# xuhaocuhk/TilinGNN

Measured on AMD Instinct MI355X. Metric: scored tile-nodes/sec (GNN forward), higher is better.
Workload: dtype f32; 1 GPU; TilinGNN.forward on a seeded banded super-graph: 100000 nodes / 1000000 adjacency edges / 1250000 collision edges per GPU, tile_count 2, T=13 edge types, width 32, depth 20, train-mode BatchNorm, graph prep included; n_nodes=100000, n_adj_edges=1000000, n_col_edges=1250000, parallelism=single GPU

## Files before the change

### include/tgnn.h

```cpp
#ifndef TGNN_H
#define TGNN_H

#include <stddef.h>
#include <stdint.h>

#ifdef __cplusplus
extern "C" {
#endif

#define TGNN_VERSION 100

#define TGNN_OK 0
#define TGNN_ERR_INVALID_ARG (-1)
#define TGNN_ERR_WORKSPACE (-2)
#define TGNN_ERR_LAUNCH (-3)
#define TGNN_ERR_UNSUPPORTED (-4)
#define TGNN_ERR_BAD_GRAPH (-5)
#define TGNN_ERR_UNVERIFIED (-7)
#define TGNN_ERR_STALE_RESULT (-6)

#define TGNN_ACT_NONE 0
#define TGNN_ACT_LEAKY_RELU 1
#define TGNN_ACT_SIGMOID 2

// ... 72 lines not shown
int tgnn_gin_fwd(const float *a, int64_t lda, const float *in_stat, const int32_t *rowptr,
                 const int32_t *col_src, const float *eps, const float *w1, const float *b1,
                 const float *w2, const float *b2, const float *w3, const float *b3, int64_t n_nodes,
                 int32_t c, int32_t act, float *out, float *z_scratch, double *bn_partial,
                 int32_t *n_partials_host, tgnn_stream_t stream);

int tgnn_dense_act_fwd(const float *a, int64_t lda, int64_t a_kblock_stride, const float *in_stat,
                       const float *w, const float *b, int64_t n_rows, int32_t in_dim, int32_t out_dim,
                       int32_t act, float *out, int64_t ldo, double *bn_partial, int32_t *n_partials_host,
                       tgnn_stream_t stream);
int tgnn_dense_act_slots_fwd(const float *a, int32_t slot_width, int64_t slot_stride, const float *in_stat,
                             const float *w, const float *b, int64_t n_rows, int32_t in_dim, int32_t out_dim,
                             int32_t act, float *out, int64_t ldo, double *bn_partial, int32_t *n_partials_host,
                             tgnn_stream_t stream);
int tgnn_dense_act_slots_f16_fwd(const float *a, int32_t slot_width, int64_t slot_stride, const float *w, const float *b,
                                 int64_t n_rows, int32_t in_dim, int32_t out_dim, int32_t act, float *out, int64_t ldo,
                                 uint32_t *bounds_scratch, void *wimg_scratch, double *bn_partial, int32_t *n_partials_host,
                                 tgnn_stream_t stream);

int tgnn_bn_finalize(int32_t mode, const double *partials, int32_t n_partials, double *sums, int32_t f,
                     int64_t n_rows_total, const float *gamma, const float *beta, float eps, float momentum,
                     float *running_mean, float *running_var, int64_t *num_batches_tracked, float *stat,
                     tgnn_stream_t stream);

int tgnn_bn_apply(const float *v, int64_t ldv, const float *stat, int64_t n_rows, int32_t f, float *out,
                  int64_t ldo, tgnn_stream_t stream);

int tgnn_merge_fwd(const float *a1, const float *stat1, const float *a2, const float *stat2,
                   const float *resid, int64_t n_nodes, int32_t c, float *out, float *h2_out,
                   tgnn_stream_t stream);

typedef struct tgnn_model_dims {
    int32_t node_features_dim;
    int32_t adj_edge_features_dim;
    int32_t network_width;
    int32_t network_depth;
    int32_t output_dim;
} tgnn_model_dims;

int32_t tgnn_param_count(const tgnn_model_dims *dims);
int tgnn_param_name(const tgnn_model_dims *dims, int32_t index, char *buf, size_t buf_len);

typedef struct tgnn_graph {
    int64_t n_nodes;
    int64_t n_adj_edges;
    int64_t n_col_edges;
    int32_t n_types;
    const int32_t *adj_rowptr;
    const int32_t *adj_src;
    const int32_t *adj_type;
    const int32_t *type_rep_edge;
    const int32_t *col_rowptr;
    const int32_t *col_src;
    const int32_t *nn_tile_col_ptr;
    const int32_t *nn_col_meta;
    const int32_t *nn_col_src;
    int32_t nn_max_in_degree;
    const int32_t *nn_mid_tile_nb;
    const uint32_t *nn_mid_ent;
    const int32_t *nn_tile_grp_ptr;
    const int32_t *nn_grp;
    const int32_t *nn_mid_verdict;
} tgnn_graph;

size_t tgnn_forward_workspace_bytes(const tgnn_model_dims *dims, int64_t n_nodes, int32_t n_types);

int tgnn_forward(const tgnn_model_dims *dims, const void *const *params_host, const float *x,
                 const float *adj_edge_attr, const tgnn_graph *graph, int32_t update_running,
                 int32_t use_running_stats, float *probs, void *ws, size_t ws_bytes,
                 tgnn_stream_t stream, tgnn_stream_t stream2);

int tgnn_forward_begin(const tgnn_model_dims *dims, const void *const *params_host, const float *x, int64_t n_nodes,
                       int32_t update_running, void *ws, size_t ws_bytes, tgnn_stream_t stream, tgnn_stream_t stream2);
int tgnn_forward_resume(const tgnn_model_dims *dims, const void *const *params_host, const float *x, const float *adj_edge_attr,
                        const tgnn_graph *graph, int32_t update_running, float *probs, void *ws, size_t ws_bytes,
                        tgnn_stream_t stream, tgnn_stream_t stream2);
int tgnn_forward_small_prepass(const tgnn_model_dims *dims, const void *const *params_host, const float *adj_edge_attr,
                               const int32_t *type_rep_edge, const int32_t *n_types_dev, int64_t n_nodes, void *ws, size_t ws_bytes,
                               tgnn_stream_t stream);

int tgnn_forward_begin_weights(const tgnn_model_dims *dims, const void *const *params_host, const float *adj_edge_attr,
                               const int32_t *type_rep_edge, const int32_t *n_types_dev, int64_t n_nodes, void *ws, size_t ws_bytes,
                               tgnn_stream_t stream);

typedef struct tgnn_train_save {
    float *init_a[2];
    float *init_stat[2];
    float *a1, *a2;
    float *u;
    float *stat1, *stat2;
    float *fin_a[4];
    float *fin_stat[4];
    float *skip;
    float *wtab;
} tgnn_train_save;
int tgnn_forward_train(const tgnn_model_dims *dims, const void *const *params_host, const float *x,
                       const float *adj_edge_attr, const tgnn_graph *graph, const tgnn_train_save *keep, float *probs,
                       void *ws, size_t ws_bytes, tgnn_stream_t stream, tgnn_stream_t stream2);

typedef struct tgnn_train_graph {
    const int32_t *adjT_rowptr, *adjT_src, *adjT_type;
    const int32_t *colT_rowptr, *colT_src;
    const float *deg, *inv_deg;
} tgnn_train_graph;
size_t tgnn_backward_workspace_bytes(const tgnn_model_dims *dims, int64_t n_nodes, int32_t n_types);
int tgnn_backward(const tgnn_model_dims *dims, const void *const *params_host, void *const *grads_host, const float *x,
                  const float *adj_edge_attr, const tgnn_graph *graph, const tgnn_train_graph *tgraph,
                  const tgnn_train_save *keep, const float *probs, const float *dprobs, void *ws, size_t ws_bytes,
                  tgnn_stream_t stream);

typedef struct tgnn_shard {
    int64_t n_own, n_rows, n_total;
    const int32_t *send_idx;
    int64_t n_send;
    double *sum_buf;
    float *send_buf;
    float *recv_buf;
    int (*allreduce_f64)(void *ctx, double *buf, int64_t count, tgnn_stream_t stream);
    int (*alltoall_rows)(void *ctx, const float *send, float *recv, int32_t row_floats, int32_t extra_rows,
                         tgnn_stream_t stream);
    void *ctx;
    int32_t world, rank;
    const int32_t *send_idx_fused;
    const int32_t *recv_idx_fused;
    tgnn_stream_t side_stream;
    void *rccl_comm, *rccl_comm_side;
    const int64_t *send_counts, *recv_counts;
    const int32_t *send_row_ptr, *send_row_slot;
} tgnn_shard;

int32_t tgnn_rccl_available(void);
size_t tgnn_rccl_unique_id_bytes(void);
int tgnn_rccl_unique_id(void *id_out);
int tgnn_rccl_comm_create(const void *unique_id, int32_t rank, int32_t world, void **comm_out);
int tgnn_rccl_comm_destroy(void *comm);
void tgnn_rccl_counters(int64_t *out2);
size_t tgnn_forward_sharded_workspace_bytes(const tgnn_model_dims *dims, int64_t n_own, int64_t n_rows,
                                            int32_t n_types);
int tgnn_forward_sharded(const tgnn_model_dims *dims, const void *const *params_host, const float *x,
                         const float *adj_edge_attr, const tgnn_graph *graph, const tgnn_shard *shard,
                         int32_t update_running, float *probs, void *ws, size_t ws_bytes, tgnn_stream_t stream);

void tgnn_set_small_layout_limit(int64_t n_nodes);
int tgnn_spin_error_poll(tgnn_stream_t stream, uint32_t *code_out);
uint64_t tgnn_set_spin_budget_us(uint64_t us);
void tgnn_persist_fallback(int64_t n_forwards);
uint32_t tgnn_spin_error_peek(void);
int64_t tgnn_get_small_layout_limit(void);

int32_t tgnn_set_split_precision(int32_t mode);
int32_t tgnn_set_gin_fused(int32_t mode);
int32_t tgnn_set_gin_mlp_f16(int32_t on);
int32_t tgnn_set_mid_tail(int32_t on);
int32_t tgnn_set_nnconv_eg(int32_t on);
int32_t tgnn_set_dense_rows_mode(int32_t mode);
int32_t tgnn_set_lean_head(int32_t bits);

int64_t tgnn_graph_prep_small_max_nodes(void);
int64_t tgnn_graph_prep_small_max_edges(void);
size_t tgnn_graph_prep_small_tmp_ints(int64_t n_nodes, int64_t n_adj_edges, int64_t n_col_edges);
int tgnn_graph_prep_small(const int64_t *adj_edge_index, int64_t n_adj_edges, const float *adj_edge_attr, int32_t fe,
                          const int64_t *col_edge_index, int64_t n_col_edges, int64_t n_nodes, int32_t *adj_rowptr,
                          int32_t *adj_src, int32_t *adj_eid, int32_t *adj_type, int32_t *edge_type, int32_t *type_rep_edge,
                          int32_t *col_rowptr, int32_t *col_src, int32_t *col_eid, int32_t *tile_col_ptr, int32_t *col_meta,
                          int32_t *col_slot_src, int32_t *tmp, int32_t *result, uint32_t *counters, int32_t *result_host,
                          tgnn_stream_t stream);

typedef struct tgnn_small_prep_layout {
    const int64_t *adj_edge_index;
    const float *adj_edge_attr;
    const int64_t *col_edge_index;
    int64_t n_adj_edges, n_col_edges, n_nodes;
    int32_t *adj_rowptr, *adj_src, *adj_eid, *adj_type, *edge_type, *type_rep_edge;
    int32_t *col_rowptr, *col_src, *col_eid;
    int32_t *tile_col_ptr, *col_meta, *col_slot_src;
    int32_t *tmp;
    int32_t fe, reserved_;
} tgnn_small_prep_layout;
int tgnn_graph_prep_small_many(const tgnn_small_prep_layout *layouts_host, int32_t k, int32_t *results_dev, int32_t *results_host,
                               tgnn_stream_t stream);
int tgnn_graph_prep_small_many_wait(tgnn_stream_t stream);
int tgnn_graph_prep_small_many_plan(const int64_t *n_adj_edges, const int64_t *n_col_edges, const int64_t *n_nodes, int32_t k,
                                    int32_t capacity_blocks, int32_t *blocks_out, int32_t *group_out);
void tgnn_graph_prep_small_many_counts(int64_t out[2]);

size_t tgnn_graph_prep_workspace_bytes(int64_t n_nodes, int64_t n_adj_edges, int64_t n_col_edges, int32_t fe);
int tgnn_graph_prep(const int64_t *adj_edge_index, int64_t n_adj_edges, const float *adj_edge_attr, int32_t fe,
                    const int64_t *col_edge_index, int64_t n_col_edges, int64_t n_nodes, int64_t n_src_nodes, int32_t *adj_rowptr,
                    int32_t *adj_src, int32_t *adj_eid, int32_t *adj_type, int32_t *edge_type, int32_t *type_rep_edge, int32_t *col_rowptr,
                    int32_t *col_src, int32_t *col_eid, int32_t *tile_col_ptr, int32_t *col_meta, int32_t *col_slot_src,
                    int32_t *mid_tile_nb, uint32_t *mid_ent, int32_t *tile_grp_ptr, int32_t *grp,
                    void *ws, size_t ws_bytes, int32_t *result, int32_t *result_host, tgnn_stream_t stream);
int tgnn_graph_prep_wait(tgnn_stream_t stream);
int32_t tgnn_set_prep_words_poll(int32_t on);
#ifdef TGNN_DEBUG
int32_t tgnn_debug_set_csr_bucket_cap(int32_t cap);
void tgnn_debug_set_block_caps(int32_t nnconv_blocks, int32_t gin_mlp_blocks);
void tgnn_debug_spin_fault(int32_t n_launches);
#endif

#define TGNN_PROF_CLASSES 8
#define TGNN_PROF_EDGE_WEIGHTS 0
#define TGNN_PROF_DENSE_INIT 1
#define TGNN_PROF_NNCONV 2
#define TGNN_PROF_GIN 3
#define TGNN_PROF_BN_FINALIZE 4
#define TGNN_PROF_MERGE 5
#define TGNN_PROF_DENSE_FINAL 6
int tgnn_forward_profiled(const tgnn_model_dims *dims, const void *const *params_host, const float *x,
                          const float *adj_edge_attr, const tgnn_graph *graph, int32_t update_running,
                          int32_t use_running_stats, float *probs, void *ws, size_t ws_bytes,
                          tgnn_stream_t stream, float *class_ms_host, int32_t *class_launches_host);

int tgnn_forward_profiled_two_stream(const tgnn_model_dims *dims, const void *const *params_host, const float *x,
                                     const float *adj_edge_attr, const tgnn_graph *graph, int32_t update_running,
                                     float *probs, void *ws, size_t ws_bytes, tgnn_stream_t stream, tgnn_stream_t stream2,
                                     float *class_ms_host, int32_t *class_launches_host);
int tgnn_forward_many(const tgnn_model_dims *dims, const void *const *params_host, int32_t n_layouts, const float *const *x,
                      const float *const *adj_edge_attr, const tgnn_graph *graphs, int32_t update_running,
                      int32_t use_running_stats, float *const *probs, void *const *ws, const size_t *ws_bytes,
                      const tgnn_stream_t *streams, int32_t n_streams, tgnn_stream_t stream2);
int tgnn_forward_union(const tgnn_model_dims *dims, const void *const *params_host, int32_t n_layouts, const float *const *x,
                       const float *const *adj_edge_attr, const tgnn_graph *graphs, int32_t use_running_stats,
                       float *const *probs, void *const *ws, const size_t *ws_bytes, tgnn_stream_t stream,
                       const tgnn_stream_t *streams, int32_t n_streams, tgnn_stream_t stream2);
int tgnn_forward_union_plan(const int64_t *n_nodes, int32_t k, int32_t capacity_blocks, int32_t *group_out);
void tgnn_forward_union_counts(int64_t out[2]);
int tgnn_forward_stamped(const tgnn_model_dims *dims, const void *const *params_host, const float *x, const float *adj_edge_attr,
                         const tgnn_graph *graph, int32_t update_running, float *probs, void *ws, size_t ws_bytes,
                         tgnn_stream_t stream, tgnn_stream_t stream2, float *nnconv_us_host);

size_t tgnn_sublayout_workspace_bytes(int64_t n_nodes, int64_t n_adj_edges, int64_t n_col_edges);
int tgnn_sublayout_compact(const int32_t *alive, int64_t n_nodes, const float *x, int32_t fx,
                           const int64_t *adj_edge_index, int64_t n_adj_edges, const float *adj_edge_attr, int32_t fe,
                           const int64_t *col_edge_index, int64_t n_col_edges, float *x_out, int64_t *inverse_out,
                           int64_t *adj_out, float *adj_attr_out, int64_t *col_out, int64_t *counts_out,
                           int32_t *err_flag, void *ws, size_t ws_bytes, tgnn_stream_t stream);

int tgnn_shard_alive_rows(const int32_t *alive_global, const int64_t *gid, int64_t n_own, int64_t n_rows,
                          const int64_t *adj_edge_index, int64_t n_adj_edges, const int64_t *col_edge_index, int64_t n_col_edges,
                          int32_t *alive_local, int32_t *err_flag, tgnn_stream_t stream);

size_t tgnn_greedy_round_workspace_bytes(int64_t n_sub);
int tgnn_greedy_round(const float *prob, int64_t ld_prob, const int64_t *inverse, int64_t n_sub, const int64_t *col_edge_index,
                      int64_t n_col_edges, int32_t round, uint64_t seed, double *prob_saved, int32_t *alive,
                      int32_t *selected_round, int64_t *n_selected, int32_t *err_flag, void *ws, size_t ws_bytes,
                      tgnn_stream_t stream);
int64_t tgnn_greedy_finish_max_nodes(void);
int tgnn_greedy_finish(const int64_t *inverse, int64_t n_sub, const int64_t *col_edge_index, int64_t n_col_edges,
                       int32_t first_round, int32_t max_rounds, uint64_t seed, double *prob_saved, int32_t *alive,
                       int32_t *selected_round, int64_t *n_selected, int32_t *err_flag, int32_t *out, tgnn_stream_t stream);

size_t tgnn_sublayout_compact_many_workspace_bytes(int32_t n_layouts, int64_t total_nodes, int64_t total_adj_edges,
                                                   int64_t total_col_edges);
int tgnn_sublayout_compact_many(int32_t n_layouts, const int32_t *active, const int64_t *node_ptr, const int64_t *adj_ptr,
                                const int64_t *col_ptr, int64_t total_nodes, int64_t total_adj_edges, int64_t total_col_edges,
                                const int32_t *alive, const float *x, int32_t fx, const int64_t *adj_edge_index,
                                const float *adj_edge_attr, int32_t fe, const int64_t *col_edge_index, float *x_out,
                                int64_t *inverse_out, int64_t *adj_out, float *adj_attr_out, int64_t *col_out, int64_t *counts_out,
                                int32_t *err_flag, void *ws, size_t ws_bytes, tgnn_stream_t stream);
size_t tgnn_greedy_round_many_workspace_bytes(int32_t n_layouts, int64_t total_nodes);
int tgnn_greedy_round_many(int32_t n_layouts, const int32_t *active, const float *const *prob, int64_t ld_prob,
                           const int64_t *node_ptr, const int64_t *col_ptr, int64_t total_nodes, int64_t total_col_edges,
                           const int64_t *counts, const int64_t *inverse, const int64_t *col_edge_index, int32_t round,
                           const uint64_t *seeds, double *prob_saved, int32_t *alive, int32_t *selected_round, int64_t *n_selected,
                           int32_t *err_flag, void *ws, size_t ws_bytes, tgnn_stream_t stream);
int tgnn_greedy_finish_many(int32_t n_layouts, const int32_t *finish, const int64_t *node_ptr, const int64_t *col_ptr,
                            int64_t total_nodes, int64_t total_col_edges, const int64_t *counts, const int64_t *inverse,
                            const int64_t *col_edge_index, int32_t first_round, int32_t max_rounds, const uint64_t *seeds,
                            double *prob_saved, int32_t *alive, int32_t *selected_round, int64_t *n_selected, int32_t *err_flag,
                            int32_t *out, tgnn_stream_t stream);

size_t tgnn_unsupervised_loss_workspace_bytes(int32_t n_maps);
int tgnn_unsupervised_loss(const float *probs, int64_t ld_probs, int32_t n_maps, const float *area_ratio,
                           int64_t ld_area, int64_t n_nodes, const int64_t *col_edge_index, int64_t n_col_edges,
                           const int64_t *adj_edge_index, int64_t n_adj_edges, const float *adj_edge_len,
                           int64_t ld_len, float collision_weight, float align_length_weight, float avg_area_weight,
                           double *losses, double *terms, void *ws, size_t ws_bytes, tgnn_stream_t stream);

// ... 118 lines not shown
```

### tilingnn_amd/_lib.py

```python
from __future__ import annotations

import ctypes as C
import os

_HERE = os.path.dirname(os.path.abspath(__file__))
LIB_PATH = os.environ.get("TGNN_LIB_PATH") or os.path.join(_HERE, "libtgnn.so")

ACT_NONE, ACT_LEAKY_RELU, ACT_SIGMOID = 0, 1, 2
BN_MAX_PARTIALS = 512
BN_STAT_ROWS = 4


class TgnnError(RuntimeError):
    code = 0


class ModelDims(C.Structure):
    _fields_ = [("node_features_dim", C.c_int32), ("adj_edge_features_dim", C.c_int32),
                ("network_width", C.c_int32), ("network_depth", C.c_int32), ("output_dim", C.c_int32)]


class Graph(C.Structure):
    _fields_ = [("n_nodes", C.c_int64), ("n_adj_edges", C.c_int64), ("n_col_edges", C.c_int64),
                ("n_types", C.c_int32),
# ... 17 lines not shown

class TrainSave(C.Structure):
    _fields_ = [("init_a", C.c_void_p * 2), ("init_stat", C.c_void_p * 2), ("a1", C.c_void_p), ("a2", C.c_void_p),
                ("u", C.c_void_p), ("stat1", C.c_void_p), ("stat2", C.c_void_p), ("fin_a", C.c_void_p * 4),
                ("fin_stat", C.c_void_p * 4), ("skip", C.c_void_p), ("wtab", C.c_void_p)]


class TrainGraphDesc(C.Structure):
    _fields_ = [("adjT_rowptr", C.c_void_p), ("adjT_src", C.c_void_p), ("adjT_type", C.c_void_p),
                ("colT_rowptr", C.c_void_p), ("colT_src", C.c_void_p), ("deg", C.c_void_p), ("inv_deg", C.c_void_p)]


ALLREDUCE_CB = C.CFUNCTYPE(C.c_int, C.c_void_p, C.c_void_p, C.c_int64, C.c_void_p)
ALLTOALL_CB = C.CFUNCTYPE(C.c_int, C.c_void_p, C.c_void_p, C.c_void_p, C.c_int32, C.c_int32, C.c_void_p)


class ShardDesc(C.Structure):
    _fields_ = [("n_own", C.c_int64), ("n_rows", C.c_int64), ("n_total", C.c_int64),
                ("send_idx", C.c_void_p), ("n_send", C.c_int64),
                ("sum_buf", C.c_void_p), ("send_buf", C.c_void_p), ("recv_buf", C.c_void_p),
                ("allreduce_f64", ALLREDUCE_CB), ("alltoall_rows", ALLTOALL_CB), ("ctx", C.c_void_p),
                ("world", C.c_int32), ("rank", C.c_int32), ("send_idx_fused", C.c_void_p), ("recv_idx_fused", C.c_void_p),
                ("side_stream", C.c_void_p), ("rccl_comm", C.c_void_p), ("rccl_comm_side", C.c_void_p),
                ("send_counts", C.c_void_p), ("recv_counts", C.c_void_p),
                ("send_row_ptr", C.c_void_p), ("send_row_slot", C.c_void_p)]


def _load() -> C.CDLL:
    if not os.path.exists(LIB_PATH):
        raise ImportError(
            f"{LIB_PATH} is missing: the HIP extension has not been built. Build it with\n"
            f"    python -c 'import __graft_entry__ as g; g.build()'    (or: make -C tilingnn_amd/csrc)\n"
            "tilingnn_amd has no CPU fallback by design.")
    import torch
    lib = C.CDLL(LIB_PATH)
    p, i32, i64, f32, sz = C.c_void_p, C.c_int32, C.c_int64, C.c_float, C.c_size_t
    pi32 = C.POINTER(C.c_int32)
    sigs = {
        "tgnn_version": (C.c_int, []),
        "tgnn_last_error": (C.c_char_p, []),
        "tgnn_csr_workspace_bytes": (sz, [i64, i64]),
        "tgnn_csr_build": (C.c_int, [p, i64, i64, i64, C.c_int, p, p, p, p, p, sz, p]),
        "tgnn_edge_dedup_workspace_bytes": (sz, [i64, i32]),
        "tgnn_edge_type_dedup": (C.c_int, [p, i64, i32, p, p, p, p, sz, p]),
        "tgnn_gather_i32": (C.c_int, [p, i64, p, i64, p, p]),
        "tgnn_edge_weight_table": (C.c_int, [p, p, i32, i32, p, p, p, p, p, p, i32, p, p]),
        "tgnn_nnconv_mean_fwd": (C.c_int, [p, i64, p, p, p, p, i32, p, p, i64, i32, i32, p, p, pi32, p]),
        "tgnn_nnconv_cols_max_columns": (i64, [i64, i64]),
        "tgnn_nnconv_cols_workspace_bytes": (sz, [i64]),
        "tgnn_nnconv_cols_build": (C.c_int, [p, p, p, i64, i32, p, p, p, p, sz, p]),
        "tgnn_nnconv_cols_max_types": (i32, []),
        "tgnn_nnconv_weight_image_floats": (sz, [i32]),
        "tgnn_nnconv_mean_cols_fwd": (C.c_int, [p, i64, p, p, p, p, i32, p, p, i64, i32, i32, p, p, p, pi32, p]),
        "tgnn_nnconv_mean_cols_f16_fwd": (C.c_int, [p, i64, i64, p, p, p, p, i32, p, p, i64, i32, i32, p, p, p, p, pi32, p]),
        "tgnn_nnconv_eg_max_groups": (i64, [i64, i64, i32]),
        "tgnn_nnconv_eg_build": (C.c_int, [p, p, p, i64, i32, p, p, p, sz, p]),
        "tgnn_nnconv_mean_eg_fwd": (C.c_int, [p, i64, i64, p, p, p, i32, p, p, i64, i32, p, p, p, p, pi32, p]),
        "tgnn_ubench_row_gather": (C.c_int, [i32, p, i64, p, i32, i32, C.POINTER(C.c_double), p]),
        "tgnn_mid_entries_words": (i64, [i64]),
        "tgnn_mid_entries_build": (C.c_int, [p, p, p, i64, p, p, p, p, p]),
        "tgnn_forward_path_counts": (None, [p]),
        "tgnn_set_mid_layout_limit": (None, [i64]),
        "tgnn_get_mid_layout_limit": (i64, []),
        "tgnn_mid_layout_max_nodes": (i64, []),
        "tgnn_spin_error_poll": (C.c_int, [p, C.POINTER(C.c_uint32)]),
        "tgnn_set_spin_budget_us": (C.c_uint64, [C.c_uint64]),
        "tgnn_persist_fallback": (None, [i64]),
        "tgnn_spin_error_peek": (C.c_uint32, []),
        "tgnn_gin_fwd": (C.c_int, [p, i64, p, p, p, p, p, p, p, p, p, p, i64, i32, i32, p, p, p, pi32, p]),
        "tgnn_dense_act_fwd": (C.c_int, [p, i64, i64, p, p, p, i64, i32, i32, i32, p, i64, p, pi32, p]),
        "tgnn_dense_act_slots_fwd": (C.c_int, [p, i32, i64, p, p, p, i64, i32, i32, i32, p, i64, p, pi32, p]),
        "tgnn_dense_act_slots_f16_fwd": (C.c_int, [p, i32, i64, p, p, i64, i32, i32, i32, p, i64, p, p, p, pi32, p]),
        "tgnn_bn_finalize": (C.c_int, [i32, p, i32, p, i32, i64, p, p, f32, f32, p, p, p, p, p]),
        "tgnn_bn_apply": (C.c_int, [p, i64, p, i64, i32, p, i64, p]),
        "tgnn_merge_fwd": (C.c_int, [p, p, p, p, p, i64, i32, p, p, p]),
        "tgnn_param_count": (i32, [C.POINTER(ModelDims)]),
        "tgnn_param_name": (C.c_int, [C.POINTER(ModelDims), i32, C.c_char_p, sz]),
        "tgnn_forward_workspace_bytes": (sz, [C.POINTER(ModelDims), i64, i32]),
        "tgnn_forward": (C.c_int, [C.POINTER(ModelDims), C.POINTER(C.c_void_p), p, p, C.POINTER(Graph), i32, i32,
                                   p, p, sz, p, p]),
        "tgnn_forward_begin": (C.c_int, [C.POINTER(ModelDims), C.POINTER(C.c_void_p), p, i64, i32, p, sz, p, p]),
        "tgnn_forward_resume": (C.c_int, [C.POINTER(ModelDims), C.POINTER(C.c_void_p), p, p, C.POINTER(Graph), i32, p, p, sz, p, p]),
        "tgnn_forward_begin_weights": (C.c_int, [C.POINTER(ModelDims), C.POINTER(C.c_void_p), p, p, p, i64, p, sz, p]),
        "tgnn_forward_small_prepass": (C.c_int, [C.POINTER(ModelDims), C.POINTER(C.c_void_p), p, p, p, i64, p, sz, p]),
        "tgnn_forward_sharded_workspace_bytes": (sz, [C.POINTER(ModelDims), i64, i64, i32]),
        "tgnn_forward_sharded": (C.c_int, [C.POINTER(ModelDims), C.POINTER(C.c_void_p), p, p, C.POINTER(Graph),
                                           C.POINTER(ShardDesc), i32, p, p, sz, p]),
        "tgnn_sublayout_workspace_bytes": (sz, [i64, i64, i64]),
        "tgnn_sublayout_compact": (C.c_int, [p, i64, p, i32, p, i64, p, i32, p, i64, p, p, p, p, p, p, p, p, sz, p]),
        "tgnn_shard_alive_rows": (C.c_int, [p, p, i64, i64, p, i64, p, i64, p, p, p]),
        "tgnn_tiles_in_region": (C.c_int, [p, p, p, p, p, i64, p, p, p, p, i64, i32, p, p, p]),
        "tgnn_region_edge_counts": (C.c_int, [p, i64, i64, p, i64, p, i64, p, p, p]),
        "tgnn_union_area_workspace_bytes": (sz, [i64, i64]),
        "tgnn_union_area": (C.c_int, [p, p, i64, p, p, p, i64, C.c_double, p, p, p, sz, p]),
        "tgnn_batch_union": (C.c_int, [p] * 10 + [i32, i32, i32, p, p, i32, p, p, p, p, p]),
        "tgnn_greedy_round_workspace_bytes": (sz, [i64]),
        "tgnn_greedy_round": (C.c_int, [p, i64, p, i64, p, i64, i32, C.c_uint64, p, p, p, p, p, p, sz, p]),
        "tgnn_greedy_finish_max_nodes": (i64, []),
        "tgnn_greedy_finish": (C.c_int, [p, i64, p, i64, i32, i32, C.c_uint64, p, p, p, p, p, p, p]),
        "tgnn_sublayout_compact_many_workspace_bytes": (sz, [i32, i64, i64, i64]),
        "tgnn_sublayout_compact_many": (C.c_int, [i32, p, p, p, p, i64, i64, i64, p, p, i32, p, p, i32, p, p, p, p, p, p, p, p, p, sz, p]),
        "tgnn_greedy_round_many_workspace_bytes": (sz, [i32, i64]),
        "tgnn_greedy_round_many": (C.c_int, [i32, p, p, i64, p, p, i64, i64, p, p, p, i32, p, p, p, p, p, p, p, sz, p]),
        "tgnn_greedy_finish_many": (C.c_int, [i32, p, p, p, i64, i64, p, p, p, i32, i32, p, p, p, p, p, p, p, p]),
        "tgnn_solution_score_sums_many_workspace_bytes": (sz, [i32]),
        "tgnn_solution_score_sums_many": (C.c_int, [i32, p, p, p, i64, i64, p, p, i64, p, p, p, i64, p, p, sz, p]),
        "tgnn_unsupervised_loss_workspace_bytes": (sz, [i32]),
        "tgnn_unsupervised_loss": (C.c_int, [p, i64, i32, p, i64, i64, p, i64, p, i64, p, i64, f32, f32, f32, p, p, p, sz, p]),
        "tgnn_solution_score_sums": (C.c_int, [p, p, i64, p, i64, p, i64, p, i64, p, p, sz, p]),
        "tgnn_graph_prep_small_max_nodes": (i64, []),
        "tgnn_graph_prep_small_max_edges": (i64, []),
        "tgnn_graph_prep_small_tmp_ints": (sz, [i64, i64, i64]),
        "tgnn_graph_prep_small": (C.c_int, [p, i64, p, i32, p, i64, i64] + [p] * 16 + [p]),
        "tgnn_graph_prep_workspace_bytes": (sz, [i64, i64, i64, i32]),
        "tgnn_graph_prep": (C.c_int, [p, i64, p, i32, p, i64, i64, i64] + [p] * 17 + [sz, p, p, p]),
        "tgnn_graph_prep_wait": (C.c_int, [p]),
        "tgnn_graph_prep_small_many": (C.c_int, [C.POINTER(SmallPrepLayout), i32, p, p, p]),
        "tgnn_graph_prep_small_many_wait": (C.c_int, [p]),
        "tgnn_graph_prep_small_many_plan": (C.c_int, [p, p, p, i32, i32, p, p]),
        "tgnn_graph_prep_small_many_counts": (None, [p]),
        "tgnn_set_nnconv_eg": (i32, [i32]),
        "tgnn_set_dense_rows_mode": (i32, [i32]),
        "tgnn_set_lean_head": (i32, [i32]),
        "tgnn_set_prep_words_poll": (i32, [i32]),
        "tgnn_set_small_layout_limit": (None, [i64]),
        "tgnn_get_small_layout_limit": (i64, []),
        "tgnn_set_split_precision": (i32, [i32]),
        "tgnn_set_gin_fused": (i32, [i32]),
        "tgnn_set_gin_mlp_f16": (i32, [i32]),
        "tgnn_set_mid_tail": (i32, [i32]),
        "tgnn_rccl_available": (i32, []),
        "tgnn_rccl_unique_id_bytes": (sz, []),
        "tgnn_rccl_unique_id": (C.c_int, [p]),
        "tgnn_rccl_comm_create": (C.c_int, [p, i32, i32, C.POINTER(C.c_void_p)]),
        "tgnn_rccl_comm_destroy": (C.c_int, [p]),
        "tgnn_rccl_counters": (None, [p]),
        "tgnn_forward_profiled": (C.c_int, [C.POINTER(ModelDims), C.POINTER(C.c_void_p), p, p, C.POINTER(Graph), i32,
                                            i32, p, p, sz, p, C.POINTER(C.c_float), pi32]),
        "tgnn_forward_many": (C.c_int, [C.POINTER(ModelDims), C.POINTER(C.c_void_p), i32, p, p, p, i32, i32, p, p, p, p, i32, p]),
        "tgnn_forward_union": (C.c_int, [C.POINTER(ModelDims), C.POINTER(C.c_void_p), i32, p, p, p, i32, p, p, p, p, p, i32, p]),
        "tgnn_forward_union_plan": (C.c_int, [p, i32, i32, p]),
        "tgnn_forward_union_counts": (None, [p]),
        "tgnn_forward_stamped": (C.c_int, [C.POINTER(ModelDims), C.POINTER(C.c_void_p), p, p, C.POINTER(Graph), i32, p, p, sz, p, p,
                                           C.POINTER(C.c_float)]),
        "tgnn_forward_profiled_two_stream": (C.c_int, [C.POINTER(ModelDims), C.POINTER(C.c_void_p), p, p, C.POINTER(Graph), i32,
                                                       p, p, sz, p, p, C.POINTER(C.c_float), pi32]),
        "tgnn_transpose": (C.c_int, [p, i32, i32, p, p]),
        "tgnn_swap_leading": (C.c_int, [p, i32, i32, i32, p, i32, p]),
        "tgnn_backward_workspace_bytes": (sz, [C.POINTER(ModelDims), i64, i32]),
        "tgnn_backward": (C.c_int, [C.POINTER(ModelDims), C.POINTER(C.c_void_p), C.POINTER(C.c_void_p), p, p,
                                    C.POINTER(Graph), C.POINTER(TrainGraphDesc), C.POINTER(TrainSave), p, p, p, sz, p]),
        "tgnn_forward_train": (C.c_int, [C.POINTER(ModelDims), C.POINTER(C.c_void_p), p, p, C.POINTER(Graph),
                                         C.POINTER(TrainSave), p, p, sz, p, p]),
        "tgnn_gin_aggregate": (C.c_int, [p, i64, p, p, p, p, i64, i32, p, p]),
        "tgnn_sigmoid_bwd": (C.c_int, [p, i64, p, i64, i64, i32, p, i64, p]),
        "tgnn_add_into": (C.c_int, [p, i64, i64, i32, p, i64, p]),
        "tgnn_reduce_workspace_bytes": (sz, [i32]),
        "tgnn_colsum": (C.c_int, [p, i64, i64, i32, p, p, sz, p]),
        "tgnn_bn_bwd_reduce": (C.c_int, [p, i64, p, i64, p, i64, i32, f32, p, p, p, p, sz, p]),
        "tgnn_bn_bwd_apply": (C.c_int, [p, i64, p, i64, p, p, i64, i32, i32, p, i64, p, p, i64, p]),
        "tgnn_merge_bwd_reduce": (C.c_int, [p, i64, p, p, p, p, p, i64, i32, f32, f32, p, p, p, i64, p, p, p, p, p, p,
                                            p, sz, p]),
        "tgnn_wgrad_workspace_bytes": (sz, [i64, i32, i32]),
        "tgnn_wgrad": (C.c_int, [p, i64, p, i64, i64, i64, i32, i32, p, p, p, sz, p]),
        "tgnn_wgrad_slots": (C.c_int, [p, i64, p, i32, i64, i64, i32, i32, p, p, p, sz, p]),
        "tgnn_sigmoid_mlp_bwd_workspace_bytes": (sz, [i64, i32, i32, i32, i32]),
        "tgnn_sigmoid_mlp_bwd": (C.c_int, [p, i64, i32, i32, i32, i32, p, p, p, p, p, p, p, i64, p, p, p, p, p, p, p, p, sz,
                                           p]),
        "tgnn_nnconv_type_sum": (C.c_int, [p, i64, p, i64, p, p, p, p, i64, i32, i32, p, p]),
        "tgnn_csr_degree": (C.c_int, [p, i64, p, p, p]),
        "tgnn_unsupervised_loss_bwd": (C.c_int, [p, i64, p, i64, i64, p, i64, p, i64, p, i64, f32, f32, f32, p, p, p, i64,
                                                 p, sz, p]),
        "tgnn_f32_to_bf16": (C.c_int, [p, i64, p, p]),
        "tgnn_nnconv64_image_elems": (sz, [i32]),
        "tgnn_nnconv64_bf16_fwd": (C.c_int, [p, i64, p, p, p, p, i32, p, p, i64, i32, p, p, p, pi32, p]),
        "tgnn_nnconv64_bf16_eg_fwd": (C.c_int, [p, i64, p, p, p, i32, p, p, i64, i32, p, p, p, pi32, p]),
        "tgnn_gin64_bf16_fwd": (C.c_int, [p, p, p, p, p, p, p, p, p, p, p, i64, i32, p, p, p, pi32, p]),
        "tgnn_collconv64_bf16_fwd": (C.c_int, [p, p, p, p, p, p, p, p, p, p, p, p, p, p, p, i64, p, p, p, p, p, p]),
        "tgnn_merge_bf16_fwd": (C.c_int, [p, p, p, p, p, i64, i32, p, p]),
        "tgnn_dense_bf16_slots_fwd": (C.c_int, [p, i64, i32, p, p, i64, i32, i32, p, p, p, pi32, p]),
        "tgnn_forward_bf16_workspace_bytes": (sz, [C.POINTER(ModelDims), i64, i32]),
        "tgnn_forward_bf16": (C.c_int, [C.POINTER(ModelDims), C.POINTER(C.c_void_p), p, p, C.POINTER(Graph), i32, p, p, sz, p, p]),
        "tgnn_forward_bf16_begin": (C.c_int, [C.POINTER(ModelDims), C.POINTER(C.c_void_p), p, i64, i32, p, sz, p]),
        "tgnn_rows_gather": (C.c_int, [p, i64, p, i64, i32, p, i64, p]),
        "tgnn_rows_scatter": (C.c_int, [p, p, i64, i32, p, i64, p]),
    }
    for name, (res, args) in sigs.items():
        fn = getattr(lib, name)
        fn.restype, fn.argtypes = res, args
    for name, (res, args) in {"tgnn_debug_spin_fault": (None, [i32]), "tgnn_debug_set_csr_bucket_cap": (i32, [i32]),
                              "tgnn_debug_set_block_caps": (None, [i32, i32])}.items():
        try:
            fn = getattr(lib, name)
        except AttributeError:
            continue
        fn.restype, fn.argtypes = res, args
    return lib


DEBUG_LIB_PATH = os.path.join(_HERE, "libtgnn_debug.so")


def has_debug_hooks() -> bool:
    return hasattr(lib, "tgnn_debug_spin_fault")


lib = _load()
EXPORTED_SYMBOLS = (
    "tgnn_version", "tgnn_last_error", "tgnn_csr_workspace_bytes", "tgnn_csr_build",
    "tgnn_edge_dedup_workspace_bytes", "tgnn_edge_type_dedup", "tgnn_gather_i32", "tgnn_edge_weight_table",
    "tgnn_nnconv_mean_fwd", "tgnn_nnconv_cols_max_columns", "tgnn_nnconv_cols_workspace_bytes",
    "tgnn_nnconv_cols_build", "tgnn_nnconv_cols_max_types", "tgnn_nnconv_weight_image_floats", "tgnn_nnconv_mean_cols_fwd", "tgnn_nnconv_mean_cols_f16_fwd", "tgnn_nnconv_eg_max_groups", "tgnn_nnconv_eg_build", "tgnn_nnconv_mean_eg_fwd",
    "tgnn_ubench_row_gather", "tgnn_mid_entries_words", "tgnn_mid_entries_build", "tgnn_forward_path_counts", "tgnn_set_mid_layout_limit", "tgnn_get_mid_layout_limit", "tgnn_mid_layout_max_nodes",
    "tgnn_spin_error_poll", "tgnn_set_spin_budget_us", "tgnn_persist_fallback", "tgnn_spin_error_peek", "tgnn_gin_fwd", "tgnn_dense_act_fwd", "tgnn_dense_act_slots_fwd", "tgnn_dense_act_slots_f16_fwd", "tgnn_bn_finalize", "tgnn_bn_apply",
    "tgnn_merge_fwd", "tgnn_param_count", "tgnn_param_name", "tgnn_forward_workspace_bytes", "tgnn_forward", "tgnn_forward_begin", "tgnn_forward_resume",
    "tgnn_forward_profiled", "tgnn_forward_profiled_two_stream", "tgnn_forward_stamped", "tgnn_forward_many", "tgnn_forward_union", "tgnn_forward_union_plan", "tgnn_forward_union_counts", "tgnn_graph_prep_small_max_nodes", "tgnn_graph_prep_small_max_edges", "tgnn_graph_prep_small_tmp_ints",
    "tgnn_graph_prep_small", "tgnn_graph_prep_workspace_bytes", "tgnn_graph_prep", "tgnn_graph_prep_wait", "tgnn_graph_prep_small_many", "tgnn_graph_prep_small_many_wait", "tgnn_graph_prep_small_many_plan", "tgnn_graph_prep_small_many_counts", "tgnn_set_small_layout_limit", "tgnn_get_small_layout_limit", "tgnn_set_split_precision", "tgnn_set_gin_fused", "tgnn_set_gin_mlp_f16", "tgnn_set_mid_tail", "tgnn_set_nnconv_eg", "tgnn_set_dense_rows_mode", "tgnn_set_lean_head", "tgnn_set_prep_words_poll", "tgnn_forward_begin_weights", "tgnn_forward_bf16_begin", "tgnn_forward_small_prepass", "tgnn_rccl_available", "tgnn_rccl_unique_id_bytes", "tgnn_rccl_unique_id", "tgnn_rccl_comm_create", "tgnn_rccl_comm_destroy", "tgnn_rccl_counters", "tgnn_forward_train", "tgnn_backward_workspace_bytes", "tgnn_backward", "tgnn_forward_sharded_workspace_bytes", "tgnn_forward_sharded",
    "tgnn_rows_gather", "tgnn_rows_scatter", "tgnn_unsupervised_loss_workspace_bytes", "tgnn_unsupervised_loss", "tgnn_solution_score_sums",
    "tgnn_sublayout_workspace_bytes", "tgnn_sublayout_compact", "tgnn_greedy_round_workspace_bytes", "tgnn_greedy_round", "tgnn_greedy_finish_max_nodes", "tgnn_greedy_finish", "tgnn_shard_alive_rows",
    "tgnn_sublayout_compact_many_workspace_bytes", "tgnn_sublayout_compact_many", "tgnn_greedy_round_many_workspace_bytes", "tgnn_greedy_round_many",
    "tgnn_greedy_finish_many", "tgnn_solution_score_sums_many_workspace_bytes", "tgnn_solution_score_sums_many",
    "tgnn_tiles_in_region", "tgnn_region_edge_counts", "tgnn_union_area_workspace_bytes", "tgnn_union_area", "tgnn_batch_union",
    "tgnn_transpose", "tgnn_swap_leading", "tgnn_gin_aggregate", "tgnn_sigmoid_bwd", "tgnn_add_into", "tgnn_reduce_workspace_bytes", "tgnn_colsum",
    "tgnn_bn_bwd_reduce", "tgnn_bn_bwd_apply", "tgnn_merge_bwd_reduce", "tgnn_wgrad_workspace_bytes", "tgnn_wgrad", "tgnn_wgrad_slots",
    "tgnn_sigmoid_mlp_bwd_workspace_bytes", "tgnn_sigmoid_mlp_bwd",
    "tgnn_nnconv_type_sum", "tgnn_csr_degree", "tgnn_unsupervised_loss_bwd",
    "tgnn_f32_to_bf16", "tgnn_nnconv64_image_elems", "tgnn_nnconv64_bf16_fwd", "tgnn_nnconv64_bf16_eg_fwd", "tgnn_gin64_bf16_fwd", "tgnn_collconv64_bf16_fwd", "tgnn_merge_bf16_fwd",
    "tgnn_dense_bf16_slots_fwd", "tgnn_forward_bf16_workspace_bytes", "tgnn_forward_bf16")


def forward_path_counts():
    out = (C.c_int64 * 3)()
    lib.tgnn_forward_path_counts(out)
    return tuple(int(v) for v in out)


def forward_union_counts():
    out = (C.c_int64 * 2)()
    lib.tgnn_forward_union_counts(out)
    return tuple(int(v) for v in out)


def forward_union_plan(n_nodes, capacity_blocks):
    k = len(n_nodes)
    sizes = (C.c_int64 * max(k, 1))(*[int(v) for v in n_nodes])
    out = (C.c_int32 * max(k, 1))()
    n_groups = int(lib.tgnn_forward_union_plan(sizes, k, int(capacity_blocks), out))
    if n_groups < 0:
        raise ValueError("tgnn_forward_union_plan: invalid arguments")
    return [int(out[i]) for i in range(k)], n_groups


def graph_prep_small_many_counts():
    out = (C.c_int64 * 2)()
    lib.tgnn_graph_prep_small_many_counts(out)
    return tuple(int(v) for v in out)


def graph_prep_small_many_plan(n_adj_edges, n_col_edges, n_nodes, capacity_blocks):
    k = len(n_nodes)
    if not (len(n_adj_edges) == len(n_col_edges) == k):
        raise ValueError("tgnn_graph_prep_small_many_plan: one count of each kind per layout")
    arr = lambda vs: (C.c_int64 * max(k, 1))(*[int(v) for v in vs])
    blocks, groups = (C.c_int32 * max(k, 1))(), (C.c_int32 * max(k, 1))()
    n_groups = int(lib.tgnn_graph_prep_small_many_plan(arr(n_adj_edges), arr(n_col_edges), arr(n_nodes), k, int(capacity_blocks), blocks, groups))
    if n_groups < 0:
        raise ValueError("tgnn_graph_prep_small_many_plan: invalid arguments")
    return [int(blocks[i]) for i in range(k)], [int(groups[i]) for i in range(k)], n_groups


def check(rc: int) -> None:
    if rc != 0:
        msg = lib.tgnn_last_error()
        err = TgnnError(f"libtgnn error {rc}: {msg.decode() if msg else '?'}")
        err.code = int(rc)
        raise err


def ptr(t) -> C.c_void_p:
    return C.c_void_p(0) if t is None else C.c_void_p(t.data_ptr())


import threading

_pinned = threading.local()


def current_stream(device) -> C.c_void_p:
    import torch
    hit = getattr(_pinned, "value", None)
    if hit is not None:
        return hit[1]
    return C.c_void_p(torch.cuda.current_stream(device).cuda_stream)


class pinned_stream:

    def __init__(self, device):
        self.device = device

# ... 121 lines not shown
```

### tilingnn_amd/csrc/forward.hip

```cpp
#include <stdarg.h>
#include <string.h>

#include <string>
#include <vector>

#include "tgnn_common.h"

namespace tgnn {
int spin_error_collect_stale(hipStream_t s);
}

namespace tgnn {

static thread_local char g_err[512] = "";

void set_error(const char *fmt, ...) {
    va_list ap;
    va_start(ap, fmt);
    vsnprintf(g_err, sizeof(g_err), fmt, ap);
    va_end(ap);
}

static void bn_names(std::vector<std::string> &v, const std::string &p) {
    v.push_back(p + ".weight");
// ... 8 lines not shown
    if (bn) bn_names(v, p + ".batch_norm");
}

static std::vector<std::string> param_names(const tgnn_model_dims &d) {
    std::vector<std::string> v;
    for (int l = 0; l < 2; ++l) lt_names(v, "init_node_feature_trans.mlp." + std::to_string(l), true);
    for (int i = 0; i < d.network_depth; ++i) {
        const std::string p1 = "brch_1_graph_conv_layers." + std::to_string(i);
        for (int l = 0; l < 3; ++l) lt_names(v, p1 + ".mlp.mlp." + std::to_string(l), false);
        v.push_back(p1 + ".nnConv.root");
        v.push_back(p1 + ".nnConv.bias");
        bn_names(v, p1 + ".batch_norm");
        const std::string p2 = "brch_2_coll_conv_layers." + std::to_string(i);
        v.push_back(p2 + ".ginConv.eps");
        for (int l = 0; l < 3; ++l) lt_names(v, p2 + ".ginConv.nn.mlp." + std::to_string(l), false);
        bn_names(v, p2 + ".batch_norm");
    }
    for (int l = 0; l < 4; ++l) lt_names(v, "final_mlp.0.mlp." + std::to_string(l), true);
    lt_names(v, "final_mlp.1", false);
    return v;
}

static bool dims_ok(const tgnn_model_dims *d) {
    return d && d->node_features_dim >= 1 && d->adj_edge_features_dim >= 1 && d->adj_edge_features_dim <= 1024 &&
           d->network_width >= 4 && d->network_width % 4 == 0 && d->network_width <= 256 && d->network_depth >= 1 &&
           d->network_depth <= kMaxDepth && d->output_dim >= 1 && d->output_dim <= 256;
}

struct Workspace {
    float *mid, *a1, *a2[2], *t0, *f1, *f2, *f3, *f4, *wtab, *wimg;
    double *part1, *part2, *partf;
    float *small_pack;
    double *small_part, *small_part_wide, *small_runstat;
    double *mid_part;
    unsigned *small_ctr;
    void *dimg[4];
    unsigned *bounds;
    float *stat1, *stat2[2], *stat_i[2], *stat_f[4];
    size_t bytes;
};

struct Prof {
    hipStream_t s;
    std::vector<hipEvent_t> ev;
    std::vector<int> slot;
    bool on = false;
    unsigned class_mask = ~0u;
    bool two_stream = false, open = false;
    unsigned long long *stamps = nullptr;
    void begin(int sl) {
        open = on && ((class_mask >> sl) & 1u);
        if (!open) return;
        hipEvent_t a, b;
        (void)hipEventCreate(&a);
        (void)hipEventCreate(&b);
        (void)hipEventRecord(a, s);
        ev.push_back(a);
        ev.push_back(b);
        slot.push_back(sl);
    }
    void end() {
        if (!open) return;
        (void)hipEventRecord(ev.back(), s);
        open = false;
    }
    void collect(float *ms_out, int32_t *count_out) {
        if (!on) return;
        (void)hipStreamSynchronize(s);
        for (size_t i = 0; i < slot.size(); ++i) {
            float ms = 0.f;
            (void)hipEventElapsedTime(&ms, ev[2 * i], ev[2 * i + 1]);
            ms_out[slot[i]] += ms;
            count_out[slot[i]] += 1;
            (void)hipEventDestroy(ev[2 * i]);
            (void)hipEventDestroy(ev[2 * i + 1]);
        }
    }
};

static const int kFinalDims[4] = {256, 128, 64, 0};
constexpr int kCarveTypes = 16;
static std::atomic<int> g_split_f16{1};
static std::atomic<int> g_nnconv_eg{1};
static std::atomic<int> g_lean_head{3};
static std::atomic<int64_t> g_path_count[3];
static std::atomic<int64_t> g_union_count[2];

static Workspace carve(const tgnn_model_dims &d, int64_t n, int64_t nr, int32_t n_types, void *ws, size_t ws_bytes) {
    Carver cv(ws, ws_bytes);
    const int c = d.network_width, D = d.network_depth;
    Workspace w{};
    w.mid = cv.take<float>((size_t)(D + 1) * nr * c);
    w.a1 = cv.take<float>((size_t)nr * c);
    w.a2[0] = cv.take<float>((size_t)nr * c);
    w.a2[1] = cv.take<float>((size_t)nr * c);
    w.t0 = cv.take<float>((size_t)n * c);
    w.f1 = cv.take<float>((size_t)n * 256);
    w.f2 = cv.take<float>((size_t)n * 128);
    w.f3 = cv.take<float>((size_t)n * 64);
    w.f4 = cv.take<float>((size_t)n * c);
    const int tc = n_types < kCarveTypes ? kCarveTypes : n_types;
    w.wtab = cv.take<float>((size_t)D * tc * c * c);
    w.wimg = cv.take<float>((size_t)D * (tc + 1) * kWtType);
    w.part1 = cv.take<double>((size_t)TGNN_BN_MAX_PARTIALS * 2 * c);
    w.part2 = cv.take<double>((size_t)TGNN_BN_MAX_PARTIALS * 2 * c);
    w.partf = cv.take<double>((size_t)TGNN_BN_MAX_PARTIALS * 2 * 256);
    w.small_pack = cv.take<float>(small_pack_floats(D));
    w.small_part = cv.take<double>((size_t)256 * 128);
    w.small_part_wide = cv.take<double>((size_t)2 * 256 * 512);
    w.small_runstat = cv.take<double>((size_t)D * 128);
    w.mid_part = cv.take<double>(mid_part_doubles());
    w.small_ctr = cv.take<unsigned>(64);
    w.bounds = cv.take<unsigned>(2 * kMaxDepth + 100);
    {
        const int fd[4] = {c * (D + 1), kFinalDims[0], kFinalDims[1], kFinalDims[2]};
        for (int l = 0; l < 3; ++l) w.dimg[l] = cv.take<unsigned char>(dense_f16_image_size(fd[l], fd[l + 1]));
        w.dimg[3] = cv.take<unsigned char>(dense_f16_image_size(fd[3], c));
    }
    w.stat1 = cv.take<float>(4 * c);
    w.stat2[0] = cv.take<float>(4 * c);
    w.stat2[1] = cv.take<float>(4 * c);
    w.stat_i[0] = cv.take<float>(4 * c);
    w.stat_i[1] = cv.take<float>(4 * c);
    for (int l = 0; l < 4; ++l) w.stat_f[l] = cv.take<float>(4 * 256);
    w.bytes = cv.off + 256;
    return w;
}

}

using namespace tgnn;

extern "C" int tgnn_version(void) { return TGNN_VERSION; }
extern "C" int32_t tgnn_set_split_precision(int32_t mode) {
    if (mode != 0 && mode != 1) return g_split_f16.load();
    return g_split_f16.exchange(mode);
}

extern "C" int32_t tgnn_set_nnconv_eg(int32_t on) {
    if (on != 0 && on != 1) return g_nnconv_eg.load();
    return g_nnconv_eg.exchange(on);
}
extern "C" int32_t tgnn_set_lean_head(int32_t bits) {
    if (bits < 0 || bits > 31) return g_lean_head.load();
    return g_lean_head.exchange(bits);
}
extern "C" const char *tgnn_last_error(void) { return g_err; }
extern "C" void tgnn_forward_path_counts(int64_t *out3) {
    if (!out3) return;
    for (int k = 0; k < 3; ++k) out3[k] = g_path_count[k].load(std::memory_order_relaxed);
}

extern "C" int32_t tgnn_param_count(const tgnn_model_dims *dims) {
    if (!dims_ok(dims)) return -1;
    return 2 * kInitStride + dims->network_depth * kLayerStride + 4 * kFinalStride + 2;
}

extern "C" int tgnn_param_name(const tgnn_model_dims *dims, int32_t index, char *buf, size_t buf_len) {
    TGNN_CHECK_ARG(dims_ok(dims), "model dims");
    TGNN_CHECK_ARG(buf && buf_len > 0, "buffer");
    const std::vector<std::string> names = param_names(*dims);
    TGNN_CHECK_ARG(index >= 0 && index < (int)names.size(), "index");
    TGNN_CHECK_ARG(names[index].size() + 1 <= buf_len, "buffer too small");
    memcpy(buf, names[index].c_str(), names[index].size() + 1);
    return TGNN_OK;
}

extern "C" size_t tgnn_forward_workspace_bytes(const tgnn_model_dims *dims, int64_t n_nodes, int32_t n_types) {
    if (!dims_ok(dims) || n_nodes < 0) return 0;
    return carve(*dims, n_nodes, n_nodes, n_types, nullptr, 0).bytes;
}

extern "C" size_t tgnn_forward_sharded_workspace_bytes(const tgnn_model_dims *dims, int64_t n_own, int64_t n_rows,
                                                       int32_t n_types) {
    if (!dims_ok(dims) || n_own < 0 || n_rows < n_own) return 0;
    return carve(*dims, n_own, n_rows, n_types, nullptr, 0).bytes;
}

#define TGNN_TRY(expr)               \
    do {                             \
        int rc__ = (expr);           \
        if (rc__ != TGNN_OK) return rc__; \
    } while (0)

struct HeadEvent {
    hipEvent_t ev = nullptr;
    const void *ws = nullptr;
    int64_t n = 0;
    bool weights = false;
};
static thread_local HeadEvent g_head[64];
struct SmallPre {
    const void *ws = nullptr;
    int64_t n = 0;
};
static thread_local SmallPre g_small_pre[64];
static inline unsigned *final_bound_word(const Workspace &w, int D, int l) { return w.bounds + (l <= 2 ? 2 * D + 2 + 2 * (l - 1) : 2 * D + 8); }
static int forward_head_bounds_images(const tgnn_model_dims *dims, const Params &P, const Workspace &w, int64_t n, int64_t n_total,
                                      hipStream_t st, bool *images_ok) {
    const int c = dims->network_width, D = dims->network_depth;
    const int fin_dims[5] = {c * (D + 1), kFinalDims[0], kFinalDims[1], kFinalDims[2], c};
    unsigned *dense_max = w.bounds + 2 * D + 1;
    const int nl = (c == 32 && n >= kDenseRowsKernelMin) ? 4 : 3;
    const float *bw[4], *bg[4], *bb[4];
    int64_t bwn[4];
    int bf[4];
    unsigned *bwm[4], *bam[4];
    bw[0] = P.f(P.fin(0)); bwn[0] = (int64_t)fin_dims[0] * fin_dims[1]; bg[0] = nullptr; bb[0] = nullptr; bf[0] = 0; bwm[0] = dense_max; bam[0] = nullptr;
    for (int l = 1; l < nl; ++l) {
        const BnPtrs bp = P.bn(P.fin(l - 1) + 2);
        bw[l] = P.f(P.fin(l));
        bwn[l] = (int64_t)fin_dims[l] * fin_dims[l + 1];
        bg[l] = bp.gamma; bb[l] = bp.beta; bf[l] = fin_dims[l];
        bwm[l] = final_bound_word(w, D, l);
        bam[l] = final_bound_word(w, D, l) + 1;
    }
    launch_dense_bounds(nl, bw, bwn, bg, bb, bf, bwm, bam, n_total, st);
    *images_ok = false;
    if (nl == 4) {
        const float *iw[4];
        int iin[4], iout[4];
        const unsigned *iwm[4];
        void *iimg[4];
        for (int l = 0; l < 4; ++l) {
            iw[l] = P.f(P.fin(l)); iin[l] = fin_dims[l]; iout[l] = fin_dims[l + 1];
            iwm[l] = l == 0 ? dense_max : final_bound_word(w, D, l);
            iimg[l] = w.dimg[l];
        }
        *images_ok = dense_f16_images_build(4, iw, iin, iout, iwm, iimg, st) == TGNN_OK;
    }
    return TGNN_OK;
}
static int forward_head_init(const tgnn_model_dims *dims, const Params &P, const float *x, const Workspace &w, int64_t n,
                             int32_t update_running, unsigned *slot_max, hipStream_t st) {
    const int fx = dims->node_features_dim;
    const int ib = init_mlp_fused_blocks(n);
    BnJob j0 = BnJob{w.partf, ib, nullptr, nullptr, nullptr, nullptr, nullptr, nullptr, w.stat_i[0]};
    BnJob j1 = BnJob{w.partf + (size_t)TGNN_BN_MAX_PARTIALS * 64, ib, nullptr, nullptr, nullptr, nullptr, nullptr, nullptr, w.stat_i[1]};
    const BnPtrs b0 = P.bn(P.init(0) + 2), b1 = P.bn(P.init(1) + 2);
    j0.gamma = b0.gamma; j0.beta = b0.beta; j1.gamma = b1.gamma; j1.beta = b1.beta;
    if (update_running) {
        j0.running_mean = b0.rm; j0.running_var = b0.rv; j0.num_batches_tracked = b0.nbt;
        j1.running_mean = b1.rm; j1.running_var = b1.rv; j1.num_batches_tracked = b1.nbt;
    }
    return launch_init_mlp_fused(x, fx, fx, P.f(P.init(0)), P.f(P.init(0) + 1), P.f(P.init(1)), P.f(P.init(1) + 1), j0, j1, n, 1e-5f, 0.1f,
                                 w.mid, slot_max, st);
}

static bool forward_cols_ok(const tgnn_model_dims *dims, const tgnn_graph *graph, int64_t nr) {
    return graph->nn_tile_col_ptr && dims->network_width == 32 && (int64_t)nr * dims->network_width * 4 < (int64_t(1) << 31);
}
static bool small_path_open(const tgnn_model_dims *dims, const tgnn_graph *graph, int64_t n, int64_t nr, bool sharded, bool keep,
                            bool use_running_stats, bool profiled) {
    return forward_cols_ok(dims, graph, nr) && !sharded && !keep && !use_running_stats && !profiled && nr == n;
}

static int forward_impl(const tgnn_model_dims *dims, const void *const *params_host, const float *x,
                        const float *adj_edge_attr, const tgnn_graph *graph, int32_t update_running,
                        int32_t use_running_stats, float *probs, void *ws, size_t ws_bytes, tgnn_stream_t stream,
                        tgnn_stream_t stream2, Prof &prof, const tgnn_shard *sh = nullptr,
                        const tgnn_train_save *keep = nullptr, bool head_done = false) {
    TGNN_CHECK_ARG(dims_ok(dims), "model dims");
    TGNN_CHECK_ARG(params_host && graph && probs && x, "null pointer");
    const bool init_running_done = (update_running & 2) != 0;
    update_running &= 1;
    const int64_t n = graph->n_nodes;
    TGNN_CHECK_ARG(n >= 1, "empty graph");
    TGNN_CHECK_ARG(use_running_stats || sh || n >= 2, "train-mode BatchNorm needs more than one row");
    TGNN_CHECK_ARG(graph->adj_rowptr && graph->col_rowptr, "graph pointers");
    TGNN_CHECK_ARG(graph->n_types == 0 || (adj_edge_attr && graph->type_rep_edge && graph->adj_src && graph->adj_type),
                   "adjacency pointers");
    const int np = tgnn_param_count(dims);
    for (int i = 0; i < np; ++i)
        if (!params_host[i]) {
            set_error("tgnn_forward: params_host[%d] is null", i);
            return TGNN_ERR_INVALID_ARG;
        }
    const int64_t nr = sh ? sh->n_rows : n, n_total = sh ? sh->n_total : n, n_halo = nr - n;
    if (sh) {
        TGNN_CHECK_ARG(sh->n_own == n && nr >= n && n_total >= n, "shard row counts");
        TGNN_CHECK_ARG(!use_running_stats, "sharded forward runs in train mode");
        TGNN_CHECK_ARG(sh->sum_buf && sh->send_buf && sh->recv_buf, "shard buffers");
        TGNN_CHECK_ARG(sh->rccl_comm ? (sh->send_counts && sh->recv_counts && sh->world >= 1 && sh->world <= 64)
                                     : (sh->allreduce_f64 && sh->alltoall_rows), "shard communicator / callbacks");
        TGNN_CHECK_ARG(sh->n_send == 0 || sh->send_idx, "send_idx");
    }
    TGNN_TRY(spin_error_collect_stale(static_cast<hipStream_t>(stream)));
    Workspace w = carve(*dims, n, nr, graph->n_types, ws, ws_bytes);
    if (!ws || w.bytes > ws_bytes) {
        set_error("tgnn_forward: workspace too small (%zu < %zu)", ws_bytes, w.bytes);
        return TGNN_ERR_WORKSPACE;
    }
    if (keep) {
        TGNN_CHECK_ARG(!sh && !use_running_stats, "the training forward is single-device, train mode");
        TGNN_CHECK_ARG(keep->skip && keep->wtab && keep->a1 && keep->a2 && keep->u && keep->stat1 && keep->stat2, "keep buffers");
        for (int l = 0; l < 2; ++l) TGNN_CHECK_ARG(keep->init_a[l] && keep->init_stat[l], "keep buffers (init)");
        for (int l = 0; l < 4; ++l) TGNN_CHECK_ARG(keep->fin_a[l] && keep->fin_stat[l], "keep buffers (final)");
        w.mid = keep->skip;
        w.wtab = keep->wtab;
        w.t0 = keep->init_a[0];
        w.a1 = keep->init_a[1];
        w.stat_i[0] = keep->init_stat[0];
        w.stat_i[1] = keep->init_stat[1];
        w.f1 = keep->fin_a[0]; w.f2 = keep->fin_a[1]; w.f3 = keep->fin_a[2]; w.f4 = keep->fin_a[3];
        for (int l = 0; l < 4; ++l) w.stat_f[l] = keep->fin_stat[l];
    }
    hipStream_t s = static_cast<hipStream_t>(stream);
    bool weights_early = false;
    bool small_pre = false;
    {
        int devp = 0;
        if (hipGetDevice(&devp) == hipSuccess && devp >= 0 && devp < 64 && g_small_pre[devp].ws) {
            small_pre = g_small_pre[devp].ws == ws && g_small_pre[devp].n == n && !head_done && !sh && !keep;
            g_small_pre[devp].ws = nullptr;
        }
    }
    if (head_done) {
        int dev = 0;
        TGNN_CHECK_HIP(hipGetDevice(&dev));
        TGNN_CHECK_ARG(dev >= 0 && dev < 64 && g_head[dev].ev && g_head[dev].ws == ws && g_head[dev].n == n,
                       "tgnn_forward_resume without a matching tgnn_forward_begin (same thread, device, workspace, node count)");
        g_head[dev].ws = nullptr;
        weights_early = g_head[dev].weights;
        g_head[dev].weights = false;
        TGNN_CHECK_HIP(hipStreamWaitEvent(s, g_head[dev].ev, 0));
    }
    hipStream_t s2 = (prof.on && !prof.two_stream) ? nullptr : static_cast<hipStream_t>(sh ? sh->side_stream : stream2);
    if (s2 == s || (sh && dims->network_width != 32)) s2 = nullptr;
    constexpr int kEvPerDev = 3 + 2 * kMaxDepth, kEvFork = 1 + 2 * kMaxDepth, kEvWeights = 2 + 2 * kMaxDepth;
    static thread_local hipEvent_t ev_cache[64][kEvPerDev] = {};
    hipEvent_t *ev = nullptr;
    if (s2) {
        int dev = 0;
        TGNN_CHECK_HIP(hipGetDevice(&dev));
        TGNN_CHECK_ARG(dev >= 0 && dev < 64, "device index");
        if (!ev_cache[dev][0])
            for (int k = 0; k < kEvPerDev; ++k)
                TGNN_CHECK_HIP(hipEventCreateWithFlags(&ev_cache[dev][k], hipEventDisableTiming));
        ev = ev_cache[dev];
    }
    prof.s = s;
    const int c = dims->network_width, D = dims->network_depth, fx = dims->node_features_dim,
              fe = dims->adj_edge_features_dim, T = graph->n_types;
    const Params P{params_host, D};
    const float eps = 1e-5f, momentum = 0.1f;
    const int fin_mode = use_running_stats ? 3 : 0;
    int32_t np1 = 0, np2 = 0;

    auto allreduce = [&](double *buf, int64_t count, hipStream_t st) -> int {
        if (sh->rccl_comm) return rccl_allreduce_f64(sh->rccl_comm, buf, count, st);
        if (sh->allreduce_f64(sh->ctx, buf, count, st) != 0) {
            set_error("tgnn_forward_sharded: the all-reduce callback failed");
            return TGNN_ERR_INVALID_ARG;
        }
        return TGNN_OK;
    };
    auto alltoall = [&](const float *send, float *recv, int row_floats, int extra_rows, hipStream_t st) -> int {
        if (sh->rccl_comm) {
            void *comm = (st != s && sh->rccl_comm_side) ? sh->rccl_comm_side : sh->rccl_comm;
            return rccl_alltoall_rows(comm, send, recv, sh->send_counts, sh->recv_counts, sh->world, row_floats, extra_rows, st);
        }
        if (sh->alltoall_rows(sh->ctx, send, recv, row_floats, extra_rows, st) != 0) {
            set_error("tgnn_forward_sharded: the all-to-all callback failed");
            return TGNN_ERR_INVALID_ARG;
        }
        return TGNN_OK;
    };
    auto finalize_jobs = [&](BnJobs jobs, int nj, int f) -> int {
        if (nj == 0) return TGNN_OK;
        if (!sh) {
            prof.begin(4);
            launch_bn_finalize(jobs, nj, fin_mode, f, n, eps, momentum, s);
            prof.end();
            return TGNN_OK;
        }
        for (int j = 0; j < nj; ++j) jobs.job[j].sums = sh->sum_buf + (size_t)j * 2 * f;
        launch_bn_finalize(jobs, nj, 1, f, n_total, eps, momentum, s);
        TGNN_TRY(allreduce(sh->sum_buf, (int64_t)nj * 2 * f, s));
        launch_bn_finalize(jobs, nj, 2, f, n_total, eps, momentum, s);
        return TGNN_OK;
    };
    auto finalize1 = [&](double *part, int nparts, int f, const BnPtrs &b, float *stat) -> int {
        BnJobs jobs{};
        jobs.job[0] = BnJob{part, nparts, nullptr, b.gamma, b.beta, (update_running || use_running_stats) ? b.rm : nullptr,
                            (update_running || use_running_stats) ? b.rv : nullptr,
                            (update_running && !use_running_stats) ? b.nbt : nullptr, stat};
        return finalize_jobs(jobs, 1, f);
    };
    auto exchange = [&](int slot, const float *a2_own, float *a2_halo_dst) -> int {
        if (!sh) return TGNN_OK;
        const int rf = a2_own ? 2 * c : c;
        float *slot_rows = w.mid + (size_t)slot * nr * c;
// ... 435 lines not shown
    return forward_impl(dims, params_host, x, adj_edge_attr, graph, update_running, use_running_stats, probs, ws,
                        ws_bytes, stream, stream2, prof);
}

extern "C" int tgnn_forward_begin(const tgnn_model_dims *dims, const void *const *params_host, const float *x, int64_t n_nodes,
                                  int32_t update_running, void *ws, size_t ws_bytes, tgnn_stream_t stream, tgnn_stream_t stream2) {
    DeviceGuard guard__(stream ? stream : stream2);
    TGNN_CHECK_ARG(dims_ok(dims) && params_host && x && n_nodes >= 2, "arguments");
    hipStream_t s = static_cast<hipStream_t>(stream), s2 = static_cast<hipStream_t>(stream2);
    const int c = dims->network_width, D = dims->network_depth, fx = dims->node_features_dim;
    if (!s2 || s2 == s || c != 32 || fx > 8 || D > kMaxDepth || ((int64_t)c * (D + 1) * kFinalDims[0]) % 4 != 0 || !g_split_f16 ||
        (g_lean_head.load(std::memory_order_relaxed) & 3) != 3 || n_nodes <= tgnn_get_mid_layout_limit() || n_nodes <= tgnn_get_small_layout_limit())
        return TGNN_ERR_UNSUPPORTED;
    const int np = tgnn_param_count(dims);
    for (int i = 0; i < np; ++i)
        if (!params_host[i]) {
            set_error("tgnn_forward_begin: params_host[%d] is null", i);
            return TGNN_ERR_INVALID_ARG;
        }
    Workspace w = carve(*dims, n_nodes, n_nodes, 0, ws, ws_bytes);
    if (!ws || w.bytes > ws_bytes) {
        set_error("tgnn_forward_begin: workspace too small (%zu < %zu)", ws_bytes, w.bytes);
        return TGNN_ERR_WORKSPACE;
    }
    int dev = 0;
    TGNN_CHECK_HIP(hipGetDevice(&dev));
    TGNN_CHECK_ARG(dev >= 0 && dev < 64, "device index");
    HeadEvent &he = g_head[dev];
    static thread_local hipEvent_t fork_ev[64] = {};
    if (!he.ev) TGNN_CHECK_HIP(hipEventCreateWithFlags(&he.ev, hipEventDisableTiming));
    if (!fork_ev[dev]) TGNN_CHECK_HIP(hipEventCreateWithFlags(&fork_ev[dev], hipEventDisableTiming));
    if (s) {
        TGNN_CHECK_HIP(hipEventRecord(fork_ev[dev], s));
        TGNN_CHECK_HIP(hipStreamWaitEvent(s2, fork_ev[dev], 0));
    }
    const Params P{params_host, D};
    const float *roots[kMaxDepth];
    for (int i = 0; i < D; ++i) roots[i] = P.f(P.layer(i) + 6);
    launch_forward_scales(w.bounds, 2 * D + 95, roots, D, w.bounds + D + 1, nullptr, 0, nullptr, s2);
    TGNN_TRY(forward_head_init(dims, P, x, w, n_nodes, update_running, w.bounds, s2));
    bool ok = false;
    TGNN_TRY(forward_head_bounds_images(dims, P, w, n_nodes, n_nodes, s2, &ok));
    TGNN_CHECK_HIP(hipEventRecord(he.ev, s2));
    he.ws = ws;
    he.n = n_nodes;
    he.weights = false;
    TGNN_CHECK_LAUNCH();
    return TGNN_OK;
}

extern "C" int tgnn_forward_small_prepass(const tgnn_model_dims *dims, const void *const *params_host, const float *adj_edge_attr,
                                          const int32_t *type_rep_edge, const int32_t *n_types_dev, int64_t n_nodes, void *ws,
                                          size_t ws_bytes, tgnn_stream_t stream) {
    DeviceGuard guard__(stream);
    TGNN_CHECK_ARG(dims_ok(dims) && params_host && n_types_dev, "arguments");
    if (!adj_edge_attr || !type_rep_edge) return TGNN_ERR_UNSUPPORTED;
    int dev = 0;
    TGNN_CHECK_HIP(hipGetDevice(&dev));
    TGNN_CHECK_ARG(dev >= 0 && dev < 64, "device index");
    const int c = dims->network_width, D = dims->network_depth, fe = dims->adj_edge_features_dim;
    if (c != 32 || n_nodes < 2 || n_nodes > tgnn_get_small_layout_limit() || !edge_weight_table_device_count_ok(fe, c) ||
        (g_lean_head.load(std::memory_order_relaxed) & 8))
        return TGNN_ERR_UNSUPPORTED;
    Workspace w = carve(*dims, n_nodes, n_nodes, 0, ws, ws_bytes);
    if (!ws || w.bytes > ws_bytes) return TGNN_ERR_WORKSPACE;
    hipStream_t s = static_cast<hipStream_t>(stream);
    const Params P{params_host, D};
    EdgeMlpLayers layers{};
    const float *roots[kMaxDepth];
    for (int i = 0; i < D; ++i) {
        const int b = P.layer(i);
        layers.l[i] = EdgeMlpLayer{P.f(b), P.f(b + 1), P.f(b + 2), P.f(b + 3), P.f(b + 4), P.f(b + 5)};
        roots[i] = P.f(b + 6);
    }
    launch_edge_weight_table_batched(adj_edge_attr, type_rep_edge, 0, fe, layers, D, c, w.wtab, roots, w.wimg, s, nullptr, nullptr, 1.0f,
                                     n_types_dev, kCarveTypes);
    launch_small_pack(P, D, w.small_pack, w.small_ctr, s);
    g_small_pre[dev].ws = ws;
    g_small_pre[dev].n = n_nodes;
    TGNN_CHECK_LAUNCH();
    return TGNN_OK;
}

extern "C" int tgnn_forward_begin_weights(const tgnn_model_dims *dims, const void *const *params_host, const float *adj_edge_attr,
                                          const int32_t *type_rep_edge, const int32_t *n_types_dev, int64_t n_nodes, void *ws,
                                          size_t ws_bytes, tgnn_stream_t stream) {
    DeviceGuard guard__(stream);
    TGNN_CHECK_ARG(dims_ok(dims) && params_host && n_types_dev, "arguments");
    if (!adj_edge_attr || !type_rep_edge) return TGNN_ERR_UNSUPPORTED;
    int dev = 0;
    TGNN_CHECK_HIP(hipGetDevice(&dev));
    TGNN_CHECK_ARG(dev >= 0 && dev < 64, "device index");
    HeadEvent &he = g_head[dev];
    const int c = dims->network_width, D = dims->network_depth, fe = dims->adj_edge_features_dim;
    if (!he.ev || he.ws != ws || he.n != n_nodes || c != 32 || !edge_weight_table_device_count_ok(fe, c) || !g_nnconv_eg.load() ||
        !g_split_f16.load() || (g_lean_head.load(std::memory_order_relaxed) & 24))
        return TGNN_ERR_UNSUPPORTED;
    Workspace w = carve(*dims, n_nodes, n_nodes, 0, ws, ws_bytes);
    if (!ws || w.bytes > ws_bytes) return TGNN_ERR_WORKSPACE;
    hipStream_t s = static_cast<hipStream_t>(stream);
    const Params P{params_host, D};
    EdgeMlpLayers layers{};
    const float *roots[kMaxDepth];
    for (int i = 0; i < D; ++i) {
        const int b = P.layer(i);
        layers.l[i] = EdgeMlpLayer{P.f(b), P.f(b + 1), P.f(b + 2), P.f(b + 3), P.f(b + 4), P.f(b + 5)};
        roots[i] = P.f(b + 6);
    }
    launch_edge_weight_table_batched(adj_edge_attr, type_rep_edge, 0, fe, layers, D, c, w.wtab, roots, w.wimg, s, nullptr, w.bounds + D + 1,
                                     kEgImageScale, n_types_dev, kCarveTypes);
    he.weights = true;
    TGNN_CHECK_LAUNCH();
    return TGNN_OK;
}

extern "C" int tgnn_forward_resume(const tgnn_model_dims *dims, const void *const *params_host, const float *x,
                                   const float *adj_edge_attr, const tgnn_graph *graph, int32_t update_running, float *probs, void *ws,
                                   size_t ws_bytes, tgnn_stream_t stream, tgnn_stream_t stream2) {
    DeviceGuard guard__(stream);
    Prof prof;
    return forward_impl(dims, params_host, x, adj_edge_attr, graph, update_running, 0, probs, ws, ws_bytes, stream, stream2, prof,
                        nullptr, nullptr, true);
}

extern "C" int tgnn_forward_many(const tgnn_model_dims *dims, const void *const *params_host, int32_t n_layouts,
                                 const float *const *x, const float *const *adj_edge_attr, const tgnn_graph *graphs,
                                 int32_t update_running, int32_t use_running_stats, float *const *probs, void *const *ws,
                                 const size_t *ws_bytes, const tgnn_stream_t *streams, int32_t n_streams, tgnn_stream_t stream2) {
    TGNN_CHECK_ARG(n_layouts >= 0 && n_streams >= 1 && x && adj_edge_attr && graphs && probs && ws && ws_bytes && streams,
                   "arguments");
    for (int k = 0; k < n_layouts; ++k) {
        tgnn_stream_t st = streams[k % n_streams];
        DeviceGuard guard__(st);
        Prof prof;
        const int rc = forward_impl(dims, params_host, x[k], adj_edge_attr[k], graphs + k, update_running, use_running_stats,
                                    probs[k], ws[k], ws_bytes[k], st, stream2, prof);
        if (rc != TGNN_OK) return rc;
    }
    return TGNN_OK;
}

extern "C" int tgnn_forward_union(const tgnn_model_dims *dims, const void *const *params_host, int32_t n_layouts,
                                  const float *const *x, const float *const *adj_edge_attr, const tgnn_graph *graphs,
                                  int32_t use_running_stats, float *const *probs, void *const *ws, const size_t *ws_bytes,
                                  tgnn_stream_t stream, const tgnn_stream_t *streams, int32_t n_streams, tgnn_stream_t stream2) {
    TGNN_CHECK_ARG(n_layouts >= 0 && n_streams >= 1 && x && adj_edge_attr && graphs && probs && ws && ws_bytes && streams,
                   "arguments");
    TGNN_CHECK_ARG(dims_ok(dims) && params_host, "model dims / parameters");
    if (n_layouts == 0) return TGNN_OK;
    const int K = n_layouts;
    std::vector<int> teams((size_t)K, 0);
    std::vector<int32_t> group((size_t)K, -1);
    int n_groups = 0;
    {
        DeviceGuard guard__(stream);
        TGNN_TRY(spin_error_collect_stale(static_cast<hipStream_t>(stream)));
        const int np = tgnn_param_count(dims);
        bool params_ok = true;
        for (int i = 0; i < np; ++i) params_ok = params_ok && params_host[i];
        for (int k = 0; k < K && params_ok; ++k) {
            const tgnn_graph *g = graphs + k;
            const int64_t n = g->n_nodes;
            const bool sane = x[k] && probs[k] && ws[k] && n >= 2 && g->adj_rowptr && g->col_rowptr &&
                              (g->n_types == 0 || (adj_edge_attr[k] && g->type_rep_edge && g->adj_src && g->adj_type));
            if (!sane || !small_path_open(dims, g, n, n, false, false, use_running_stats != 0, false)) continue;
            if (carve(*dims, n, n, g->n_types, ws[k], ws_bytes[k]).bytes > ws_bytes[k]) continue;
            teams[(size_t)k] = small_union_tiles(dims, n, g->n_types, g->nn_max_in_degree);
        }
        n_groups = small_union_plan(teams.data(), K, small_union_capacity(), group.data());
    }
    for (int k = 0; k < K; ++k) {
        if (group[(size_t)k] >= 0) continue;
        tgnn_stream_t st = streams[k % n_streams];
        DeviceGuard guard__(st);
        Prof prof;
        const int rc = forward_impl(dims, params_host, x[k], adj_edge_attr[k], graphs + k, 0, use_running_stats, probs[k], ws[k],
                                    ws_bytes[k], st, stream2, prof);
        if (rc != TGNN_OK) return rc;
    }
    if (n_groups == 0) return TGNN_OK;
    DeviceGuard guard__(stream);
    hipStream_t s = static_cast<hipStream_t>(stream);
    std::vector<SmallUnionLayout> L;
    std::vector<int32_t> grp;
    for (int k = 0; k < K; ++k) {
        if (group[(size_t)k] < 0) continue;
        const tgnn_graph *g = graphs + k;
        const Workspace w = carve(*dims, g->n_nodes, g->n_nodes, g->n_types, ws[k], ws_bytes[k]);
        L.push_back(SmallUnionLayout{x[k], adj_edge_attr[k], g, probs[k], w.mid, w.a2[0], w.a2[1], w.wtab, w.wimg, w.small_part,
                                     w.small_part_wide});
        grp.push_back(group[(size_t)k]);
    }
    const Params P{params_host, dims->network_depth};
    TGNN_TRY(launch_forward_small_union(dims, P, L.data(), (int)L.size(), grp.data(), n_groups, 1e-5f, 0.1f, s));
    g_path_count[1].fetch_add((int64_t)L.size(), std::memory_order_relaxed);
// ... 91 lines not shown
```

### tilingnn_amd/csrc/graph_prep.hip

```cpp
#include <atomic>
#include <chrono>
#include <mutex>
#include <vector>

#include "tgnn_common.h"

namespace tgnn {

constexpr int kScanThreads = 256;
constexpr int kScanItems = 8;
constexpr int kScanTile = kScanThreads * kScanItems;

__device__ __forceinline__ int wave_inclusive_scan(int v) {
    const int lane = threadIdx.x & 63;
#pragma unroll
    for (int d = 1; d < 64; d <<= 1) {
        int t = __shfl_up(v, d, 64);
        if (lane >= d) v += t;
    }
    return v;
}

__global__ __launch_bounds__(kScanThreads) void scan_tiles_kernel(const int *in, int *out,
                                                                  int *__restrict__ block_sums, int64_t n) {
// ... 251 lines not shown
        const int64_t n_here = e - base < kDedupRows ? e - base : kDedupRows;
        const int64_t total = n_here * fe;
        __syncthreads();
        {
            const int step_r = kDedupRows / fe, step_c = kDedupRows % fe;
            int r = tid / fe, c = tid % fe;
            const float *src = attr + base * fe;
            for (int k = tid; k < (int)total; k += kDedupRows) {
                rows_s[r * ld + c] = canon_bits(src[k]);
                r += step_r;
                c += step_c;
                if (c >= fe) { c -= fe; ++r; }
            }
        }
        ltab[tid] = -1;
        ltab[tid + kDedupRows] = -1;
        __syncthreads();
        const int64_t i = base + tid;
        const bool ok = i < e;
        const uint32_t *mine = rows_s + tid * ld;
        uint64_t h = 0xCBF29CE484222325ull;
        if (ok)
            for (int k = 0; k < fe; ++k) h = mix64(h, mine[k]);
        const uint32_t h32 = (uint32_t)(h ^ (h >> 32));
        int my_l = 0;
        if (ok) {
            uint32_t sl = h32 & (kDedupLocal - 1);
            while (true) {
                int cur = ltab[sl];
                if (cur < 0) {
                    const int prev = atomicCAS(&ltab[sl], -1, tid);
                    if (prev < 0) break;
                    cur = prev;
                }
                bool same = cur == tid;
                if (!same) {
                    const uint32_t *other = rows_s + cur * ld;
                    uint32_t diff = 0;
                    for (int k = 0; k < fe; ++k) diff |= other[k] ^ mine[k];
                    same = diff == 0;
                }
                if (same) {
                    if (tid < cur) atomicMin(&ltab[sl], tid);
                    break;
                }
                sl = (sl + 1) & (kDedupLocal - 1);
            }
            my_l = (int)sl;
        }
        __syncthreads();
        if (ok && ltab[my_l] == tid) {
            uint32_t slot = h32 & mask;
            while (true) {
                int cur = __hip_atomic_load(&table[slot], __ATOMIC_RELAXED, __HIP_MEMORY_SCOPE_AGENT);
                if (cur < 0) {
                    const int prev = atomicCAS(&table[slot], -1, (int)i);
                    if (prev < 0) {
                        if (rep_cnt) {
                            const int k = atomicAdd(rep_cnt, 1) + 1;
                            if (k < kDedupListMax) rep_slots[k] = (int)slot;
                        }
                        break;
                    }
                    cur = prev;
                }
                bool same = cur == (int)i;
                if (!same) {
                    const float *other = attr + (int64_t)cur * fe;
                    uint32_t diff = 0;
#pragma unroll 8
                    for (int k = 0; k < fe; ++k) diff |= canon_bits(other[k]) ^ mine[k];
                    same = diff == 0;
                }
                if (same) {
                    if ((int)i < cur) atomicMin(&table[slot], (int)i);
                    break;
                }
                slot = (slot + 1) & mask;
            }
            lslot[tid] = (int)slot;
        }
        __syncthreads();
        if (ok) slot_of_edge[i] = lslot[ltab[my_l]];
    }
}

__global__ void dedup_insert_direct_kernel(const float *__restrict__ attr, int64_t e, int fe, int *__restrict__ table,
                                           uint32_t mask, int *__restrict__ slot_of_edge, int *__restrict__ rep_cnt = nullptr,
                                           int *__restrict__ rep_slots = nullptr) {
    for (int64_t i = (int64_t)blockIdx.x * blockDim.x + threadIdx.x; i < e; i += (int64_t)gridDim.x * blockDim.x) {
        uint64_t h = 0xCBF29CE484222325ull;
        for (int k = 0; k < fe; ++k) h = mix64(h, canon_bits(attr[i * fe + k]));
        uint32_t slot = (uint32_t)(h ^ (h >> 32)) & mask;
        while (true) {
            int cur = __hip_atomic_load(&table[slot], __ATOMIC_RELAXED, __HIP_MEMORY_SCOPE_AGENT);
            if (cur < 0) {
                const int prev = atomicCAS(&table[slot], -1, (int)i);
                if (prev < 0) {
                    if (rep_cnt) {
                        const int k = atomicAdd(rep_cnt, 1) + 1;
                        if (k < kDedupListMax) rep_slots[k] = (int)slot;
                    }
                    break;
                }
                cur = prev;
            }
            if (cur == (int)i || rows_equal(attr, fe, cur, i)) {
                if ((int)i < cur) atomicMin(&table[slot], (int)i);
                break;
            }
            slot = (slot + 1) & mask;
        }
        slot_of_edge[i] = (int)slot;
    }
}

__global__ void dedup_mark_first_kernel(const int *__restrict__ table, const int *__restrict__ slot_of_edge,
                                        int64_t e, int *__restrict__ is_first) {
    for (int64_t i = (int64_t)blockIdx.x * blockDim.x + threadIdx.x; i < e; i += (int64_t)gridDim.x * blockDim.x)
        is_first[i] = table[slot_of_edge[i]] == (int)i ? 1 : 0;
}

__global__ void dedup_assign_kernel(const int *__restrict__ table, const int *__restrict__ slot_of_edge,
                                    const int *__restrict__ first_rank, int64_t e, int *__restrict__ edge_type,
                                    int *__restrict__ type_rep_edge, int *__restrict__ n_types,
                                    const int *__restrict__ skip_flag = nullptr) {
    if (skip_flag && *skip_flag) return;
    for (int64_t i = (int64_t)blockIdx.x * blockDim.x + threadIdx.x; i < e; i += (int64_t)gridDim.x * blockDim.x) {
        const int rep = table[slot_of_edge[i]];
        const int t = first_rank[rep];
        edge_type[i] = t;
        if (rep == (int)i) type_rep_edge[t] = (int)i;
        if (n_types && i == e - 1) *n_types = first_rank[i] + (rep == (int)i ? 1 : 0);
    }
}

__global__ __launch_bounds__(1024) void dedup_rank_kernel(const int *__restrict__ table, const int *__restrict__ rep_cnt,
                                                          const int *__restrict__ rep_slots, int *__restrict__ first_rank,
                                                          int *__restrict__ type_rep_edge, int *__restrict__ n_types,
                                                          int *__restrict__ fallback) {
    __shared__ int reps[kDedupListMax];
    const int cnt = *rep_cnt + 1;
    if (cnt > kDedupListMax) {
        if (threadIdx.x == 0) { *fallback = 1; *n_types = cnt; }
        return;
    }
    for (int k = threadIdx.x; k < cnt; k += 1024) reps[k] = table[rep_slots[k]];
    __syncthreads();
    for (int k = threadIdx.x; k < cnt; k += 1024) {
        const int mine = reps[k];
        int rank = 0;
        for (int j = 0; j < cnt; ++j) rank += reps[j] < mine ? 1 : 0;
        first_rank[mine] = rank;
        type_rep_edge[rank] = mine;
    }
    if (threadIdx.x == 0) *n_types = cnt;
}

__global__ void gather_i32_kernel(const int *__restrict__ src, int64_t n_src, const int *__restrict__ idx,
                                  int64_t n, int *__restrict__ out) {
    for (int64_t i = (int64_t)blockIdx.x * blockDim.x + threadIdx.x; i < n; i += (int64_t)gridDim.x * blockDim.x) {
        const int k = idx[i];
        out[i] = (k >= 0 && k < n_src) ? src[k] : 0;
    }
}

// ... 534 lines not shown
                            }
                    }
                }
                __syncthreads();
            }
            if (!fill) {
                small_prep_barrier(A.ctr, target, G);
                for (int t = tid; t <= nt16; t += NT) tile_ptr[t] = t < nt16 ? g_tile_cols[t] : 0;
                __syncthreads();
                small_block_scan(tile_ptr, nt16 + 1, wave_tot);
                if (blk == 0)
                    for (int t = tid; t <= nt16; t += NT) A.tile_col_ptr[t] = tile_ptr[t];
                __syncthreads();
            }
        }
    } else {
        small_prep_barrier(A.ctr, target, G);
    }
    TGNN_PT
    if (blk == 0 && tid == 0) {
        A.result[0] = n_types;
        A.result[1] = g_flags[0];
        A.result[2] = g_flags[1];
        A.result[3] = ec_valid;
        A.result[4] = maxdeg;
        A.result[5] = cols ? 1 : 0;
        A.result[6] = fallback ? 1 : 0;
        if (!kUnion && A.result_host) {
            const int w[7] = {n_types, g_flags[0], g_flags[1], ec_valid, maxdeg, cols ? 1 : 0, fallback ? 1 : 0};
#pragma unroll
            for (int k = 0; k < 7; ++k) __hip_atomic_store(A.result_host + k, w[k], __ATOMIC_RELAXED, __HIP_MEMORY_SCOPE_SYSTEM);
            for (int k = 7; k < 31; ++k) __hip_atomic_store(A.result_host + k, 0, __ATOMIC_RELAXED, __HIP_MEMORY_SCOPE_SYSTEM);
            __threadfence_system();
            __hip_atomic_store(A.result_host + 31, kPrepWordsMagic, __ATOMIC_RELEASE, __HIP_MEMORY_SCOPE_SYSTEM);
        }
    }
    if (kUnion && blk == 0 && tid >= 7 && tid < 32) A.result[tid] = 0;
    __syncthreads();
    if (tid == 0 && atomicAdd(&A.ctr[1], 1u) == (unsigned)G - 1) {
        __hip_atomic_store(&A.ctr[0], 0u, __ATOMIC_RELAXED, __HIP_MEMORY_SCOPE_AGENT);
        __hip_atomic_store(&A.ctr[1], 0u, __ATOMIC_RELAXED, __HIP_MEMORY_SCOPE_AGENT);
    }
}

__global__ __launch_bounds__(kSmallPrepThreads) void graph_prep_small_kernel(SmallPrepArgs A) {
    graph_prep_small_body<false>(A, (int)blockIdx.x, (int)gridDim.x);
}

__global__ __launch_bounds__(kSmallPrepThreads) void graph_prep_small_union_kernel(const SmallPrepArgs *__restrict__ tab,
                                                                                   const int *__restrict__ first_block, int n_layouts) {
    int lo = 0, hi = n_layouts;
    while (hi - lo > 1) {
        const int mid = (lo + hi) >> 1;
        if (first_block[mid] <= (int)blockIdx.x) lo = mid; else hi = mid;
    }
    const int j = __builtin_amdgcn_readfirstlane(lo);
    const int b0 = __builtin_amdgcn_readfirstlane(first_block[j]), b1 = __builtin_amdgcn_readfirstlane(first_block[j + 1]);
    const SmallPrepArgs *e = tab + j;
    SmallPrepArgs A;
    A.adj_ei = e->adj_ei; A.col_ei = e->col_ei; A.attr = e->attr;
    A.n = e->n; A.ea = e->ea; A.ec = e->ec; A.fe = e->fe; A.max_col_types = e->max_col_types;
    A.adj_rowptr = e->adj_rowptr; A.adj_src = e->adj_src; A.adj_eid = e->adj_eid; A.adj_type = e->adj_type;
    A.edge_type = e->edge_type; A.type_rep = e->type_rep;
    A.col_rowptr = e->col_rowptr; A.col_src = e->col_src; A.col_eid = e->col_eid;
    A.tile_col_ptr = e->tile_col_ptr; A.col_meta = e->col_meta; A.col_slot_src = e->col_slot_src;
    A.result_host = nullptr; A.tmp = e->tmp; A.result = e->result; A.ctr = e->ctr;
    graph_prep_small_body<true>(A, (int)blockIdx.x - b0, b1 - b0);
}

static inline unsigned grid_for(int64_t n, int threads = 256, int cap = 256 * 16) {
    int64_t g = (n + threads - 1) / threads;
    if (g < 1) g = 1;
    if (g > cap) g = cap;
    return (unsigned)g;
}

static inline uint32_t dedup_table_size(int64_t e) {
    uint64_t want = (uint64_t)(e > 512 ? e : 512) * 2;
    uint32_t cap = 1024;
    while (cap < want) cap <<= 1;
    return cap;
}


constexpr int kBkLogMax = 9, kBkRows = 1 << kBkLogMax, kBkMaxBuckets = 4096, kBkThreads = 1024;
constexpr int kBkCap = 15360;
constexpr int kBkCapHalf = 7168;
struct BkSet {
    const int64_t *ei;
    int64_t e;
    int drop_self;
    int *rowptr, *col_src, *col_eid, *err_flag;
    int *rec_eid, *rec_src;
    unsigned short *rec_row;
    int *total_out, *max_deg_out;
};
struct BkArgs {
    BkSet set[2];
    int64_t n, n_src;
    int nb, nblk;
    int lg;
    int cap;
    int cap_lds;
    int *hist;
    const int *tile_off;
    unsigned *scan_ticket;
};
__device__ __forceinline__ int bk_scanned(const BkArgs &A, int64_t i) {
    const int v = A.hist[i];
    return A.tile_off ? v + A.tile_off[i / kScanTile] : v;
}

__global__ __launch_bounds__(kBkThreads) void bk_hist_kernel(BkArgs A) {
    extern __shared__ int bk_h[];
    const BkSet S = A.set[blockIdx.y];
    const int tid = threadIdx.x, blk = blockIdx.x;
    for (int b = tid; b < A.nb; b += kBkThreads) bk_h[b] = 0;
    __syncthreads();
    const int64_t i0 = S.e * blk / A.nblk, i1 = S.e * (blk + 1) / A.nblk;
    for (int64_t i = i0 + tid; i < i1; i += kBkThreads) {
        const int64_t s = S.ei[i], d = S.ei[S.e + i];
        if (s < 0 || s >= A.n_src || d < 0 || d >= A.n) {
            if (S.err_flag) *S.err_flag = 1;
        } else if (!(S.drop_self && s == d)) {
            atomicAdd(&bk_h[d >> A.lg], 1);
        }
    }
    __syncthreads();
    for (int b = tid; b < A.nb; b += kBkThreads) A.hist[((int64_t)blockIdx.y * A.nb + b) * A.nblk + blk] = bk_h[b];
    if (blk == 0 && blockIdx.y == 1 && tid == 0) {
        A.hist[(int64_t)2 * A.nb * A.nblk] = 0;
        if (A.scan_ticket) *A.scan_ticket = 0u;
    }
}

constexpr int kBkChunk = kBkThreads * 8;
__global__ __launch_bounds__(kBkThreads) void bk_scatter_kernel(BkArgs A) {
    extern __shared__ int bk_h[];
    int *cur = bk_h, *lcnt = cur + A.nb, *lstart = lcnt + A.nb, *wtot = lstart + A.nb;
    int *l_eid = wtot + 16, *l_src = l_eid + kBkChunk;
    unsigned short *l_row = reinterpret_cast<unsigned short *>(l_src + kBkChunk), *l_bkt = l_row + kBkChunk;
    const BkSet S = A.set[blockIdx.y];
    const int tid = threadIdx.x, blk = blockIdx.x;
    const int base = bk_scanned(A, (int64_t)blockIdx.y * A.nb * A.nblk);
    for (int b = tid; b < A.nb; b += kBkThreads) cur[b] = bk_scanned(A, ((int64_t)blockIdx.y * A.nb + b) * A.nblk + blk) - base;
    const int64_t i0 = S.e * blk / A.nblk, i1 = S.e * (blk + 1) / A.nblk;
    const int per = (A.nb + kBkThreads - 1) / kBkThreads;
    for (int64_t c0 = i0; c0 < i1; c0 += kBkChunk) {
        for (int b = tid; b < A.nb; b += kBkThreads) lcnt[b] = 0;
        __syncthreads();
        int e_b[8], e_r[8], e_s[8], e_row[8];
#pragma unroll
        for (int u = 0; u < 8; ++u) {
            const int64_t i = c0 + tid + (int64_t)u * kBkThreads;
            e_b[u] = -1;
            if (i < i1) {
                const int64_t sv = S.ei[i], d = S.ei[S.e + i];
                if (!(sv < 0 || sv >= A.n_src || d < 0 || d >= A.n || (S.drop_self && sv == d))) {
                    e_b[u] = (int)(d >> A.lg);
                    e_row[u] = (int)(d & ((1 << A.lg) - 1));
                    e_s[u] = (int)sv;
                    e_r[u] = atomicAdd(&lcnt[e_b[u]], 1);
                }
            }
        }
        __syncthreads();
// ... 55 lines not shown
    const bool in_lds = m <= A.cap;
    if (tid < rows) cnt[tid] = 0;
    __syncthreads();
    if (in_lds) {
        for (int j = tid; j < m; j += kBkThreads) atomicAdd(&cnt[S.rec_row[lo + j]], 1);
    } else if (tid < rows) {
        int c = 0;
        for (int j = 0; j < m; ++j) c += S.rec_row[lo + j] == tid ? 1 : 0;
        cnt[tid] = c;
    }
    __syncthreads();
    int mine = 0, incl = 0;
    if (tid < rows) {
        mine = cnt[tid];
        incl = wave_inclusive_scan(mine);
        if ((tid & 63) == 63) wtot[tid >> 6] = incl;
    }
    __syncthreads();
    if (tid < rows) {
        int woff = 0;
        for (int w = 0; w < (tid >> 6); ++w) woff += wtot[w];
        off[tid] = woff + incl - mine;
        if (tid == rows - 1) off[rows] = woff + incl;
        const int64_t row = (int64_t)b * rows + tid;
        if (row < A.n) S.rowptr[row] = lo + off[tid];
        cnt[tid] = 0;
    }
    if (b == A.nb - 1 && tid == 0) {
        S.rowptr[A.n] = hi;
        if (S.total_out) *S.total_out = hi;
    }
    if (S.max_deg_out && tid < rows) {
        int md = mine;
#pragma unroll
        for (int d = 32; d >= 1; d >>= 1) md = max(md, __shfl_xor(md, d, 64));
        if ((tid & 63) == 0) wtot[8 + (tid >> 6)] = md;
    }
    __syncthreads();
    if (S.max_deg_out && tid == 0) {
        int md = 0;
        for (int w = 0; w < (rows >> 6); ++w) md = max(md, wtot[8 + w]);
        if (md > 0) atomicMax(S.max_deg_out, md);
    }
    if (in_lds) {
        for (int j = tid; j < m; j += kBkThreads) {
            const int r = S.rec_row[lo + j];
            const int at = off[r] + atomicAdd(&cnt[r], 1);
            key_s[at] = S.rec_eid[lo + j];
            val_s[at] = S.rec_src[lo + j];
            row_s[at] = (unsigned short)r;
        }
        __syncthreads();
        for (int j = tid; j < m; j += kBkThreads) {
            const int r = row_s[j], rb = off[r], re = off[r + 1], key = key_s[j];
            int rank = 0;
            for (int q = rb; q < re; ++q) rank += key_s[q] < key ? 1 : 0;
            S.col_eid[lo + rb + rank] = key;
            S.col_src[lo + rb + rank] = val_s[j];
        }
    } else if (tid < rows) {
        int *ke = S.col_eid + lo + off[tid], *ks = S.col_src + lo + off[tid];
        int c = 0;
        for (int j = 0; j < m; ++j)
            if (S.rec_row[lo + j] == tid) {
                ke[c] = S.rec_eid[lo + j];
                ks[c] = S.rec_src[lo + j];
                ++c;
            }
        for (int i = 1; i < c; ++i) {
            const int key = ke[i], val = ks[i];
            int j = i - 1;
            while (j >= 0 && ke[j] > key) {
                ke[j + 1] = ke[j];
                ks[j + 1] = ks[j];
                --j;
            }
            ke[j + 1] = key;
            ks[j + 1] = val;
        }
    }
}

static std::atomic<int> g_bk_cap{kBkCap};
static int prep_side_stream(hipStream_t *st, hipEvent_t *fork, hipEvent_t *join) {
    static std::mutex mu;
    static hipStream_t streams[64] = {};
    static thread_local hipEvent_t events[64][2] = {};
    int dev = 0;
    if (hipGetDevice(&dev) != hipSuccess || dev < 0 || dev >= 64) return TGNN_ERR_INVALID_ARG;
    {
        std::lock_guard<std::mutex> lock(mu);
        if (!streams[dev] && hipStreamCreateWithFlags(&streams[dev], hipStreamNonBlocking) != hipSuccess) return TGNN_ERR_INVALID_ARG;
    }
    if (!events[dev][0])
        for (int k = 0; k < 2; ++k)
            if (hipEventCreateWithFlags(&events[dev][k], hipEventDisableTiming) != hipSuccess) return TGNN_ERR_INVALID_ARG;
    *st = streams[dev];
    *fork = events[dev][0];
    *join = events[dev][1];
    return TGNN_OK;
}

static thread_local hipEvent_t g_prep_words_ev[64] = {};
static hipError_t prep_words_event(hipEvent_t *ev) {
    int dev = 0;
    hipError_t e = hipGetDevice(&dev);
    if (e != hipSuccess) return e;
    if (dev < 0 || dev >= 64) return hipErrorInvalidDevice;
    if (!g_prep_words_ev[dev]) {
        e = hipEventCreateWithFlags(&g_prep_words_ev[dev], hipEventDisableTiming);
        if (e != hipSuccess) return e;
    }
    *ev = g_prep_words_ev[dev];
    return hipSuccess;
}

static thread_local volatile int32_t *g_prep_poll[64] = {};
static std::atomic<int> g_prep_poll_on{1};

extern "C" int32_t tgnn_set_prep_words_poll(int32_t on) {
    if (on < 0) return g_prep_poll_on.load();
    return g_prep_poll_on.exchange(on ? 1 : 0);
}

extern "C" int tgnn_graph_prep_wait(tgnn_stream_t stream) {
    DeviceGuard guard__(stream);
    int dev = 0;
    TGNN_CHECK_HIP(hipGetDevice(&dev));
    if (dev >= 0 && dev < 64 && g_prep_poll[dev]) {
        volatile int32_t *h = g_prep_poll[dev];
        g_prep_poll[dev] = nullptr;
        const auto t0 = std::chrono::steady_clock::now();
        for (unsigned spins = 0;; ++spins) {
            if (__atomic_load_n(const_cast<const int32_t *>(h) + 31, __ATOMIC_ACQUIRE) == kPrepWordsMagic) return TGNN_OK;
            __builtin_ia32_pause();
            if ((spins & 1023) == 1023 && std::chrono::steady_clock::now() - t0 > std::chrono::seconds(2)) break;
        }
        TGNN_CHECK_HIP(hipStreamSynchronize(static_cast<hipStream_t>(stream)));
        if (__atomic_load_n(const_cast<const int32_t *>(h) + 31, __ATOMIC_ACQUIRE) == kPrepWordsMagic) return TGNN_OK;
        set_error("tgnn_graph_prep_wait: the result words never reached the host buffer");
        return TGNN_ERR_INVALID_ARG;
    }
    hipEvent_t ev = nullptr;
    TGNN_CHECK_HIP(prep_words_event(&ev));
    TGNN_CHECK_HIP(hipEventSynchronize(ev));
    return TGNN_OK;
}

static int bk_blocks(int64_t e_max) {
    int64_t nblk = (e_max + 8191) / 8192;
    return (int)(nblk < 1 ? 1 : (nblk > 256 ? 256 : nblk));
}
static int bk_log_rows(int64_t n, int64_t e_max) {
    return (n <= (int64_t)256 * kBkMaxBuckets && e_max * 256 <= (int64_t)3584 * (n > 0 ? n : 1)) ? 8 : 9;
}
static size_t bk_workspace_bytes(int64_t n, int64_t ea, int64_t ec) {
    const int64_t rows = (int64_t)1 << bk_log_rows(n, ea > ec ? ea : ec);
    const int64_t nb = (n + rows - 1) / rows, nblk = bk_blocks(ea > ec ? ea : ec), cells = 2 * nb * nblk + 1;
    return align_up((size_t)cells * 4, 256) + scan_ws_ints(cells) * 4 + align_up((size_t)(ea > 0 ? ea : 1) * 10, 256) +
           align_up((size_t)(ec > 0 ? ec : 1) * 10, 256) + 2048;
}
static bool bk_fits(int64_t n) { return (n + kBkRows - 1) / kBkRows <= kBkMaxBuckets; }

static int csr_build_pair_bucketed(const int64_t *adj_ei, int64_t ea, const int64_t *col_ei, int64_t ec, int64_t n, int64_t n_src,
                                   int *a_rowptr, int *a_src, int *a_eid, int *a_err, int *c_rowptr, int *c_src, int *c_eid,
                                   int *c_err, int *a_max_deg, int *c_total, void *ws, size_t ws_bytes, hipStream_t s) {
    BkArgs A{};
    A.n = n; A.n_src = n_src;
    A.lg = bk_log_rows(n, ea > ec ? ea : ec);
    A.nb = (int)((n + ((int64_t)1 << A.lg) - 1) >> A.lg);
    A.nblk = bk_blocks(ea > ec ? ea : ec);
    A.cap_lds = A.lg == 8 ? kBkCapHalf : kBkCap;
    A.cap = g_bk_cap.load() < A.cap_lds ? g_bk_cap.load() : A.cap_lds;
    const int64_t cells = (int64_t)2 * A.nb * A.nblk + 1;
    Carver cv(ws, ws_bytes);
    A.hist = cv.take<int>(cells);
    int *scan_ws = cv.take<int>(scan_ws_ints(cells));
    const int64_t es[2] = {ea, ec};
    for (int k = 0; k < 2; ++k) {
        const int64_t e1 = es[k] > 0 ? es[k] : 1;
        unsigned char *rec = cv.take<unsigned char>((size_t)e1 * 10);
        A.set[k].rec_eid = reinterpret_cast<int *>(rec);
        A.set[k].rec_src = reinterpret_cast<int *>(rec + (size_t)e1 * 4);
        A.set[k].rec_row = reinterpret_cast<unsigned short *>(rec + (size_t)e1 * 8);
    }
    A.set[0].ei = adj_ei; A.set[0].e = ea; A.set[0].drop_self = 0;
    A.set[0].rowptr = a_rowptr; A.set[0].col_src = a_src; A.set[0].col_eid = a_eid; A.set[0].err_flag = a_err;
    A.set[1].ei = col_ei; A.set[1].e = ec; A.set[1].drop_self = 1;
    A.set[1].rowptr = c_rowptr; A.set[1].col_src = c_src; A.set[1].col_eid = c_eid; A.set[1].err_flag = c_err;
    A.set[0].max_deg_out = a_max_deg;
    A.set[1].total_out = c_total;
    const size_t lds_h = (size_t)A.nb * sizeof(int);
    const int64_t scan_tiles = (cells + kScanTile - 1) / kScanTile;
    const bool fused_scan = cells > kScanOneMax && scan_tiles <= kScanFusedTiles;
    if (fused_scan) {
        A.tile_off = scan_ws + align_up((size_t)scan_tiles, 64);
        A.scan_ticket = reinterpret_cast<unsigned *>(scan_ws + scan_ws_ints(cells) - 32);
    }
    bk_hist_kernel<<<dim3(A.nblk, 2), kBkThreads, lds_h, s>>>(A);
    if (fused_scan)
        scan_tiles_fused_kernel<<<(unsigned)scan_tiles, kScanThreads, 0, s>>>(A.hist, A.hist, scan_ws, const_cast<int *>(A.tile_off), cells,
                                                                             A.scan_ticket);
    else
        exclusive_scan_i32(A.hist, A.hist, cells, scan_ws, s);
    const size_t lds_s = (size_t)(3 * A.nb + 16 + 2 * kBkChunk) * sizeof(int) + (size_t)2 * kBkChunk * sizeof(unsigned short);
    static LdsOptIn site_s;
    TGNN_CHECK_HIP(opt_in_dynamic_lds(bk_scatter_kernel, (int)(160 * 1024 - 256), site_s));
    bk_scatter_kernel<<<dim3(A.nblk, 2), kBkThreads, lds_s, s>>>(A);
    const size_t lds_r = (size_t)(2 * (1 << A.lg) + 1 + 16 + 2 * A.cap_lds) * sizeof(int) + (size_t)A.cap_lds * sizeof(unsigned short);
    static LdsOptIn site;
    TGNN_CHECK_HIP(opt_in_dynamic_lds(bk_rows_kernel, (int)(160 * 1024 - 256), site));
    bk_rows_kernel<<<dim3(A.nb, 2), kBkThreads, lds_r, s>>>(A);
    TGNN_CHECK_LAUNCH();
    return TGNN_OK;
}

}

using namespace tgnn;

#ifdef TGNN_DEBUG
extern "C" int32_t tgnn_debug_set_csr_bucket_cap(int32_t cap) {
    const int prev = g_bk_cap.load();
    if (cap >= 0) g_bk_cap.store(cap > kBkCap ? kBkCap : cap);
    return prev;
}
#endif

extern "C" size_t tgnn_csr_workspace_bytes(int64_t n_nodes, int64_t n_edges) {
    return align_up((size_t)(n_nodes + 1) * 4, 256) + align_up((size_t)(n_edges > 0 ? n_edges : 1) * 4, 256) +
           scan_ws_ints(n_nodes + 1) * 4 + 1024;
}

extern "C" int tgnn_csr_build(const int64_t *edge_index, int64_t n_edges, int64_t n_nodes, int64_t n_src_nodes,
                              int drop_self_loops, int32_t *rowptr, int32_t *col_src, int32_t *col_eid, int32_t *err_flag, void *ws,
                              size_t ws_bytes, tgnn_stream_t stream) {
    DeviceGuard guard__(stream);
    TGNN_CHECK_ARG(n_nodes >= 0 && n_nodes < (1ll << 31) - 1, "n_nodes must fit int32");
    TGNN_CHECK_ARG(n_src_nodes >= n_nodes && n_src_nodes < (1ll << 31) - 1, "n_src_nodes must be >= n_nodes and fit int32");
    TGNN_CHECK_ARG(n_edges >= 0 && n_edges < (1ll << 31) - 1, "n_edges must fit int32");
    TGNN_CHECK_ARG(rowptr && (n_edges == 0 || (edge_index && col_src && col_eid)), "null pointer");
    if (ws_bytes < tgnn_csr_workspace_bytes(n_nodes, n_edges) || !ws) {
        set_error("tgnn_csr_build: workspace too small");
        return TGNN_ERR_WORKSPACE;
    }
    hipStream_t s = static_cast<hipStream_t>(stream);
    Carver cv(ws, ws_bytes);
    int *cnt = cv.take<int>(n_nodes + 1);
    int *rank = cv.take<int>(n_edges > 0 ? n_edges : 1);
    int *scan_ws = cv.take<int>(scan_ws_ints(n_nodes + 1));
    TGNN_CHECK_HIP(hipMemsetAsync(cnt, 0, (size_t)(n_nodes + 1) * 4, s));
    if (n_edges > 0)
        csr_count_kernel<<<grid_for(n_edges), 256, 0, s>>>(edge_index, n_edges, n_nodes, n_src_nodes, drop_self_loops, cnt,
                                                           rank, err_flag);
    exclusive_scan_i32(cnt, rowptr, n_nodes + 1, scan_ws, s);
    if (n_edges > 0) {
        csr_fill_kernel<<<grid_for(n_edges), 256, 0, s>>>(edge_index, n_edges, rowptr, rank, col_src, col_eid);
        csr_sort_rows_kernel<<<(unsigned)((n_nodes + kSortRows - 1) / kSortRows), kSortRows, 0, s>>>(rowptr, n_nodes, col_src,
                                                                                                  col_eid);
    }
    TGNN_CHECK_LAUNCH();
    return TGNN_OK;
}

extern "C" size_t tgnn_edge_dedup_workspace_bytes(int64_t n_edges, int32_t fe) {
    (void)fe;
    return (size_t)dedup_table_size(n_edges) * 4 + align_up((size_t)n_edges * 4, 256) * 2 +
           scan_ws_ints(n_edges) * 4 + 2048 + (size_t)(kDedupListMax + 64) * 4 + 512;
}

static int edge_type_dedup_listed(const float *edge_attr, int64_t n_edges, int32_t fe, int32_t *edge_type, int32_t *type_rep_edge,
                                  int32_t *n_types, int32_t *fallback, void *ws, size_t ws_bytes, hipStream_t s) {
    (void)ws_bytes;
    Carver cv(ws, ws_bytes);
    const uint32_t cap = dedup_table_size(n_edges);
    int *table = cv.take<int>(cap + 64);
    int *slot_of_edge = cv.take<int>(n_edges);
    int *first_rank = cv.take<int>(n_edges);
    int *rep_slots = cv.take<int>(kDedupListMax);
    TGNN_CHECK_HIP(hipMemsetAsync(table, 0xFF, (size_t)(cap + 64) * 4, s));
    if (fe <= 60)
        dedup_insert_kernel<<<grid_for(n_edges, kDedupRows), kDedupRows, (size_t)kDedupRows * (fe | 1) * 4, s>>>(
            edge_attr, n_edges, fe, table, cap - 1, slot_of_edge, table + cap, rep_slots);
    else
        dedup_insert_direct_kernel<<<grid_for(n_edges), 256, 0, s>>>(edge_attr, n_edges, fe, table, cap - 1, slot_of_edge, table + cap,
                                                                     rep_slots);
    dedup_rank_kernel<<<1, 1024, 0, s>>>(table, table + cap, rep_slots, first_rank, type_rep_edge, n_types, fallback);
    dedup_assign_kernel<<<grid_for(n_edges), 256, 0, s>>>(table, slot_of_edge, first_rank, n_edges, edge_type, type_rep_edge,
                                                          nullptr, fallback);
    TGNN_CHECK_LAUNCH();
    return TGNN_OK;
}

extern "C" int tgnn_edge_type_dedup(const float *edge_attr, int64_t n_edges, int32_t fe, int32_t *edge_type,
                                    int32_t *type_rep_edge, int32_t *n_types, void *ws, size_t ws_bytes,
                                    tgnn_stream_t stream) {
    DeviceGuard guard__(stream);
    TGNN_CHECK_ARG(n_edges >= 0 && n_edges < (1ll << 30), "n_edges out of range");
    TGNN_CHECK_ARG(fe >= 1, "fe must be >= 1");
    TGNN_CHECK_ARG(n_types, "null n_types");
    hipStream_t s = static_cast<hipStream_t>(stream);
    if (n_edges == 0) {
        TGNN_CHECK_HIP(hipMemsetAsync(n_types, 0, 4, s));
        return TGNN_OK;
    }
    TGNN_CHECK_ARG(edge_attr && edge_type && type_rep_edge, "null pointer");
    if (ws_bytes < tgnn_edge_dedup_workspace_bytes(n_edges, fe) || !ws) {
        set_error("tgnn_edge_type_dedup: workspace too small");
        return TGNN_ERR_WORKSPACE;
    }
    Carver cv(ws, ws_bytes);
    const uint32_t cap = dedup_table_size(n_edges);
    int *table = cv.take<int>(cap);
    int *slot_of_edge = cv.take<int>(n_edges);
    int *is_first = cv.take<int>(n_edges);
    int *scan_ws = cv.take<int>(scan_ws_ints(n_edges));
    TGNN_CHECK_HIP(hipMemsetAsync(table, 0xFF, (size_t)cap * 4, s));
    if (fe <= 60)
        dedup_insert_kernel<<<grid_for(n_edges, kDedupRows), kDedupRows, (size_t)kDedupRows * (fe | 1) * 4, s>>>(
            edge_attr, n_edges, fe, table, cap - 1, slot_of_edge);
    else
        dedup_insert_direct_kernel<<<grid_for(n_edges), 256, 0, s>>>(edge_attr, n_edges, fe, table, cap - 1, slot_of_edge);
    dedup_mark_first_kernel<<<grid_for(n_edges), 256, 0, s>>>(table, slot_of_edge, n_edges, is_first);
    exclusive_scan_i32(is_first, is_first, n_edges, scan_ws, s);
    dedup_assign_kernel<<<grid_for(n_edges), 256, 0, s>>>(table, slot_of_edge, is_first, n_edges, edge_type,
                                                          type_rep_edge, n_types);
    TGNN_CHECK_LAUNCH();
    return TGNN_OK;
}

extern "C" int tgnn_gather_i32(const int32_t *src, int64_t n_src, const int32_t *idx, int64_t n, int32_t *out,
                               tgnn_stream_t stream) {
    DeviceGuard guard__(stream);
    if (n <= 0) return TGNN_OK;
    TGNN_CHECK_ARG(src && idx && out, "null pointer");
    gather_i32_kernel<<<grid_for(n), 256, 0, static_cast<hipStream_t>(stream)>>>(src, n_src, idx, n, out);
    TGNN_CHECK_LAUNCH();
    return TGNN_OK;
}

extern "C" int64_t tgnn_nnconv_cols_max_columns(int64_t n_nodes, int64_t n_edges) {
    return n_edges + (n_nodes + kColTileRows - 1) / kColTileRows + 32;
}

extern "C" size_t tgnn_nnconv_cols_workspace_bytes(int64_t n_nodes) {
    const int64_t ntiles = (n_nodes + kColTileRows - 1) / kColTileRows;
    return align_up((size_t)(ntiles + 1) * 4, 256) + scan_ws_ints(ntiles + 1) * 4 + 1024;
}

extern "C" int tgnn_nnconv_cols_build(const int32_t *rowptr, const int32_t *col_src, const int32_t *col_type,
                                      int64_t n_nodes, int32_t n_types, int32_t *tile_col_ptr, int32_t *col_meta,
                                      int32_t *col_slot_src, void *ws, size_t ws_bytes, tgnn_stream_t stream) {
    DeviceGuard guard__(stream);
    TGNN_CHECK_ARG(n_nodes >= 1, "n_nodes");
    TGNN_CHECK_ARG(n_types >= 0 && n_types <= kMaxColTypes, "the column NNConv structure supports at most 40 edge types");
    TGNN_CHECK_ARG(rowptr && tile_col_ptr && col_meta && col_slot_src, "null pointer");
    TGNN_CHECK_ARG(n_types == 0 || (col_src && col_type), "null CSR pointer");
    if (!ws || ws_bytes < tgnn_nnconv_cols_workspace_bytes(n_nodes)) {
        set_error("tgnn_nnconv_cols_build: workspace too small");
        return TGNN_ERR_WORKSPACE;
    }
    hipStream_t s = static_cast<hipStream_t>(stream);
    const int64_t nt16 = (n_nodes + kColTileRows - 1) / kColTileRows;
    Carver cv(ws, ws_bytes);
    int *tile_cols = cv.take<int>(nt16 + 1);
    int *scan_ws = cv.take<int>(scan_ws_ints(nt16 + 1));
    TGNN_CHECK_HIP(hipMemsetAsync(tile_cols + nt16, 0, 4, s));
    const unsigned blocks = (unsigned)((n_nodes + 63) / 64);
    nnconv_col_kernel<false><<<blocks, 64, 0, s>>>(rowptr, col_src, col_type, n_nodes, n_types, tile_cols, nullptr,
                                                   nullptr, nullptr);
    exclusive_scan_i32(tile_cols, tile_col_ptr, nt16 + 1, scan_ws, s);
    nnconv_col_kernel<true><<<blocks, 64, 0, s>>>(rowptr, col_src, col_type, n_nodes, n_types, nullptr, tile_col_ptr,
                                                  col_meta, col_slot_src);
    TGNN_CHECK_LAUNCH();
    return TGNN_OK;
}

extern "C" int64_t tgnn_nnconv_eg_max_groups(int64_t n_nodes, int64_t n_edges, int32_t n_types) {
    const int64_t ntiles = (n_nodes + kColTileRows - 1) / kColTileRows;
    const int64_t a = n_edges / 16 + ntiles * (int64_t)n_types, b = n_edges;
    return (a < b ? a : b) + ntiles + 32;
}

static void launch_nnconv_eg_build(const int32_t *rowptr, const int32_t *col_src, int32_t *col_type, int64_t n_nodes,
                                   int32_t n_types, const int *n_types_dev, int max_types, int32_t *tile_grps,
                                   int32_t *tile_grp_ptr, int32_t *grp, int *scan_ws, int *built_flag, hipStream_t s,
                                   const int32_t *edge_type = nullptr, const int32_t *col_eid = nullptr,
                                   const int32_t *result_words = nullptr, int32_t *host_words = nullptr) {
    const int64_t nt16 = (n_nodes + kColTileRows - 1) / kColTileRows;
    const unsigned blocks = (unsigned)((n_nodes + 63) / 64);
    nnconv_eg_kernel<false><<<blocks, 64, 0, s>>>(rowptr, col_src, col_type, n_nodes, n_types, tile_grps, nullptr, nullptr,
                                                  n_types_dev, max_types, built_flag, edge_type, col_eid,
                                                  edge_type ? col_type : nullptr, result_words, host_words);
    exclusive_scan_i32(tile_grps, tile_grp_ptr, nt16 + 1, scan_ws, s);
    nnconv_eg_kernel<true><<<blocks, 64, 0, s>>>(rowptr, col_src, col_type, n_nodes, n_types, nullptr, tile_grp_ptr,
                                                 reinterpret_cast<int2 *>(grp), n_types_dev, max_types, nullptr);
}

extern "C" int tgnn_nnconv_eg_build(const int32_t *rowptr, const int32_t *col_src, const int32_t *col_type,
                                    int64_t n_nodes, int32_t n_types, int32_t *tile_grp_ptr, int32_t *grp, void *ws,
                                    size_t ws_bytes, tgnn_stream_t stream) {
    DeviceGuard guard__(stream);
    TGNN_CHECK_ARG(n_nodes >= 1, "n_nodes");
// ... 345 lines not shown
    const SmallPrepArgs *args_dev = reinterpret_cast<const SmallPrepArgs *>(tab_dev);
    const int *fb_dev = reinterpret_cast<const int *>(tab_dev + arg_bytes);
    struct Group { int first, count, blocks, fb_at; };
    std::vector<Group> groups((size_t)n_groups, Group{0, 0, 0, 0});
    const int max_col_types = tgnn_nnconv_cols_max_types();
    int fb_at = 0;
    for (int j = 0; j < k; ++j) {
        const tgnn_small_prep_layout &l = layouts[j];
        SmallPrepArgs A{};
        A.adj_ei = l.adj_edge_index; A.col_ei = l.col_edge_index; A.attr = l.adj_edge_attr;
        A.n = l.n_nodes; A.ea = l.n_adj_edges; A.ec = l.n_col_edges; A.fe = l.fe;
        A.max_col_types = max_col_types;
        A.adj_rowptr = l.adj_rowptr; A.adj_src = l.adj_src; A.adj_eid = l.adj_eid; A.adj_type = l.adj_type;
        A.edge_type = l.edge_type; A.type_rep = l.type_rep_edge;
        A.col_rowptr = l.col_rowptr; A.col_src = l.col_src; A.col_eid = l.col_eid;
        A.tile_col_ptr = l.tile_col_ptr; A.col_meta = l.col_meta; A.col_slot_src = l.col_slot_src;
        A.tmp = l.tmp;
        A.result = results_dev + (size_t)j * 32;
        A.ctr = ctr + (size_t)j * 32;
        args[j] = A;
        Group &G = groups[(size_t)group[(size_t)j]];
        if (G.count == 0) {
            G.first = j;
            G.fb_at = fb_at++;
            fb[G.fb_at] = 0;
        }
        G.blocks += blocks[(size_t)j];
        G.count += 1;
        fb[fb_at++] = G.blocks;
    }
    TGNN_CHECK_HIP(hipMemcpyAsync(tab_dev, u.host, tab_bytes, hipMemcpyHostToDevice, s));
    int rc = TGNN_OK;
    int64_t launched = 0, prepared = 0;
    for (const Group &G : groups) {
        if (hipMemsetAsync(ctr + (size_t)G.first * 32, 0, (size_t)G.count * 128, s) != hipSuccess) {
            set_error("tgnn_graph_prep_small_many: hipMemsetAsync of the counters failed");
            rc = TGNN_ERR_LAUNCH;
            break;
        }
        struct Ctx { const SmallPrepArgs *tab; const int *fb; int count, blocks; } ctx{args_dev + G.first, fb_dev + G.fb_at, G.count, G.blocks};
        rc = spin_kernel_chain(s, [](void *c, hipStream_t st) {
            Ctx *x = static_cast<Ctx *>(c);
            graph_prep_small_union_kernel<<<dim3(x->blocks), dim3(kSmallPrepThreads), kSmallPrepLds, st>>>(x->tab, x->fb, x->count);
        }, &ctx, G.blocks);
        if (rc != TGNN_OK) break;
        ++launched;
        prepared += G.count;
    }
    if (rc == TGNN_OK && hipMemcpyAsync(results_host, results_dev, (size_t)k * 32 * sizeof(int32_t), hipMemcpyDeviceToHost, s) != hipSuccess) {
        set_error("tgnn_graph_prep_small_many: the copy of the result words could not be queued");
        rc = TGNN_ERR_LAUNCH;
    }
    (void)hipEventRecord(ev_words, s);
    (void)hipEventRecord(u.ev, s);
    g_prep_many_count[0].fetch_add(launched, std::memory_order_relaxed);
    g_prep_many_count[1].fetch_add(prepared, std::memory_order_relaxed);
    if (rc != TGNN_OK) return rc;
    TGNN_CHECK_LAUNCH();
    return TGNN_OK;
}

extern "C" int tgnn_graph_prep_small_many_wait(tgnn_stream_t stream) {
    DeviceGuard guard__(stream);
    hipEvent_t ev = nullptr;
    TGNN_CHECK_HIP(prep_many_event(&ev));
    TGNN_CHECK_HIP(hipEventSynchronize(ev));
    return TGNN_OK;
}

__global__ __launch_bounds__(256) void prep_result_kernel(const int *__restrict__ col_rowptr, const int *__restrict__ adj_rowptr,
                                                          int64_t n, int *__restrict__ result) {
    if (blockIdx.x == 0 && threadIdx.x == 0) result[3] = col_rowptr[n];
    int md = 0;
    for (int64_t r = (int64_t)blockIdx.x * 256 + threadIdx.x; r < n; r += (int64_t)gridDim.x * 256)
        md = max(md, adj_rowptr[r + 1] - adj_rowptr[r]);
#pragma unroll
    for (int d = 32; d >= 1; d >>= 1) md = max(md, __shfl_xor(md, d, 64));
    __shared__ int wm[4];
    if ((threadIdx.x & 63) == 0) wm[threadIdx.x >> 6] = md;
    __syncthreads();
    if (threadIdx.x == 0) atomicMax(result + 4, max(max(wm[0], wm[1]), max(wm[2], wm[3])));
}

extern "C" size_t tgnn_graph_prep_workspace_bytes(int64_t n_nodes, int64_t n_adj_edges, int64_t n_col_edges, int32_t fe) {
    const int64_t emax = n_adj_edges > n_col_edges ? n_adj_edges : n_col_edges;
    return align_up(tgnn_csr_workspace_bytes(n_nodes, emax), 256) + align_up(bk_workspace_bytes(n_nodes, n_adj_edges, n_col_edges), 256) +
           align_up(tgnn_edge_dedup_workspace_bytes(n_adj_edges, fe), 256) +
           align_up(tgnn_nnconv_cols_workspace_bytes(n_nodes), 256) + 1024;
}

extern "C" int tgnn_graph_prep(const int64_t *adj_edge_index, int64_t n_adj_edges, const float *adj_edge_attr, int32_t fe,
                               const int64_t *col_edge_index, int64_t n_col_edges, int64_t n_nodes, int64_t n_src_nodes,
                               int32_t *adj_rowptr, int32_t *adj_src, int32_t *adj_eid, int32_t *adj_type, int32_t *edge_type,
                               int32_t *type_rep_edge,
                               int32_t *col_rowptr, int32_t *col_src, int32_t *col_eid, int32_t *tile_col_ptr, int32_t *col_meta,
                               int32_t *col_slot_src, int32_t *mid_tile_nb, uint32_t *mid_ent, int32_t *tile_grp_ptr, int32_t *grp,
                               void *ws, size_t ws_bytes, int32_t *result, int32_t *result_host, tgnn_stream_t stream) {
    DeviceGuard guard__(stream);
    TGNN_CHECK_ARG(n_nodes >= 1 && fe >= 1 && n_adj_edges >= 0 && n_col_edges >= 0, "shape");
    TGNN_CHECK_ARG(n_src_nodes >= n_nodes && n_src_nodes < (1ll << 31) - 1, "n_src_nodes must be >= n_nodes and fit int32");
    const bool want_cols = tile_col_ptr != nullptr, want_eg = tile_grp_ptr != nullptr;
    TGNN_CHECK_ARG(adj_rowptr && col_rowptr && result, "null pointer");
    TGNN_CHECK_ARG(want_cols || want_eg, "no NNConv structure asked for (type columns and / or edge groups)");
    TGNN_CHECK_ARG(!want_cols || (col_meta && col_slot_src), "type columns: tile_col_ptr, col_meta, col_slot_src go together");
    TGNN_CHECK_ARG(!want_eg || (grp && ((uintptr_t)grp % 8) == 0), "edge groups: tile_grp_ptr and an 8-byte aligned grp go together");
    TGNN_CHECK_ARG(want_cols || !(mid_tile_nb && mid_ent), "the mid-size batches are built from the type columns");
    if (!ws || ws_bytes < tgnn_graph_prep_workspace_bytes(n_nodes, n_adj_edges, n_col_edges, fe)) {
        set_error("tgnn_graph_prep: workspace too small");
        return TGNN_ERR_WORKSPACE;
    }
    hipStream_t s = static_cast<hipStream_t>(stream);
    const int64_t emax = n_adj_edges > n_col_edges ? n_adj_edges : n_col_edges;
    Carver cv(ws, ws_bytes);
    const size_t csr_b = tgnn_csr_workspace_bytes(n_nodes, emax), dd_b = tgnn_edge_dedup_workspace_bytes(n_adj_edges, fe),
                 col_b = tgnn_nnconv_cols_workspace_bytes(n_nodes);
    void *ws_csr = cv.take<unsigned char>(csr_b), *ws_dd = cv.take<unsigned char>(dd_b), *ws_col = cv.take<unsigned char>(col_b);
    TGNN_CHECK_HIP(hipMemsetAsync(result, 0, 32 * sizeof(int32_t), s));
    hipStream_t s_side = nullptr;
    hipEvent_t ev_fork = nullptr, ev_join = nullptr;
    if (n_adj_edges > 0 && prep_side_stream(&s_side, &ev_fork, &ev_join) == TGNN_OK) {
        TGNN_CHECK_HIP(hipEventRecord(ev_fork, s));
        TGNN_CHECK_HIP(hipStreamWaitEvent(s_side, ev_fork, 0));
    } else {
        s_side = nullptr;
    }
    int rc;
    bool bucketed = false;
    auto bail = [&](int code) {
        if (s_side && hipEventRecord(ev_join, s_side) == hipSuccess) (void)hipStreamWaitEvent(s, ev_join, 0);
        return code;
    };
    const bool csr_first = n_adj_edges + n_col_edges >= 1000000;
    auto queue_dedup = [&]() -> int {
        if (!s_side) return TGNN_OK;
        rc = edge_type_dedup_listed(adj_edge_attr, n_adj_edges, fe, edge_type, type_rep_edge, result + 0, result + 6, ws_dd, dd_b, s_side);
        if (rc != TGNN_OK) return bail(rc);
        if (hipEventRecord(ev_join, s_side) != hipSuccess) {
            (void)hipStreamSynchronize(s_side);
            set_error("tgnn_graph_prep: hipEventRecord failed");
            return TGNN_ERR_LAUNCH;
        }
        return TGNN_OK;
    };
    if (!csr_first) {
        const int rcd = queue_dedup();
        if (rcd != TGNN_OK) return rcd;
    }
    if (bk_fits(n_nodes) && n_adj_edges < (int64_t(1) << 31) - 1 && n_col_edges < (int64_t(1) << 31) - 1) {
        const size_t bk_b = bk_workspace_bytes(n_nodes, n_adj_edges, n_col_edges);
        void *ws_bk = cv.take<unsigned char>(bk_b);
        rc = csr_build_pair_bucketed(adj_edge_index, n_adj_edges, col_edge_index, n_col_edges, n_nodes, n_src_nodes, adj_rowptr, adj_src,
                                     adj_eid, result + 1, col_rowptr, col_src, col_eid, result + 2, result + 4, result + 3, ws_bk, bk_b, s);
        if (rc != TGNN_OK) return bail(rc);
        bucketed = true;
    } else {
        rc = tgnn_csr_build(adj_edge_index, n_adj_edges, n_nodes, n_src_nodes, 0, adj_rowptr, adj_src, adj_eid, result + 1, ws_csr, csr_b, stream);
        if (rc != TGNN_OK) return bail(rc);
        rc = tgnn_csr_build(col_edge_index, n_col_edges, n_nodes, n_src_nodes, 1, col_rowptr, col_src, col_eid, result + 2, ws_csr, csr_b, stream);
        if (rc != TGNN_OK) return bail(rc);
    }
    if (csr_first) {
        const int rcd = queue_dedup();
        if (rcd != TGNN_OK) return rcd;
    }
    if (s_side) {
        TGNN_CHECK_HIP(hipStreamWaitEvent(s, ev_join, 0));
    } else {
        rc = tgnn_edge_type_dedup(adj_edge_attr, n_adj_edges, fe, edge_type, type_rep_edge, result + 0, ws_dd, dd_b, stream);
        if (rc != TGNN_OK) return rc;
    }
    if (!bucketed) {
        int64_t rb = (n_nodes + 1023) / 1024;
        prep_result_kernel<<<(unsigned)(rb > 256 ? 256 : rb), 256, 0, s>>>(col_rowptr, adj_rowptr, n_nodes, result);
    }
    int32_t *host_words_dev = nullptr;
    if (result_host && want_eg && !want_cols && !(mid_tile_nb && mid_ent) && g_prep_poll_on.load(std::memory_order_relaxed)) {
        int dev = 0;
        void *dptr = nullptr;
        if (hipGetDevice(&dev) == hipSuccess && dev >= 0 && dev < 64 && hipHostGetDevicePointer(&dptr, result_host, 0) == hipSuccess && dptr) {
            if (g_prep_poll[dev]) TGNN_CHECK_HIP(hipDeviceSynchronize());
            host_words_dev = static_cast<int32_t *>(dptr);
            __atomic_store_n(result_host + 31, 0, __ATOMIC_RELEASE);
            g_prep_poll[dev] = result_host;
        } else {
            (void)hipGetLastError();
        }
    }
    if (result_host && !host_words_dev) {
        hipEvent_t ev_words = nullptr;
        TGNN_CHECK_HIP(prep_words_event(&ev_words));
        if (s_side) {
            TGNN_CHECK_HIP(hipEventRecord(ev_fork, s));
            TGNN_CHECK_HIP(hipStreamWaitEvent(s_side, ev_fork, 0));
            TGNN_CHECK_HIP(hipMemcpyAsync(result_host, result, 32 * sizeof(int32_t), hipMemcpyDeviceToHost, s_side));
            TGNN_CHECK_HIP(hipEventRecord(ev_words, s_side));
        } else {
            TGNN_CHECK_HIP(hipMemcpyAsync(result_host, result, 32 * sizeof(int32_t), hipMemcpyDeviceToHost, s));
            TGNN_CHECK_HIP(hipEventRecord(ev_words, s));
        }
    }
    const int64_t nt16 = (n_nodes + kColTileRows - 1) / kColTileRows;
    Carver cc(ws_col, col_b);
    int *tile_cols = cc.take<int>(nt16 + 1);
    int *scan_ws = cc.take<int>(scan_ws_ints(nt16 + 1));
    const unsigned blocks = (unsigned)((n_nodes + 63) / 64);
    const int max_types = tgnn_nnconv_cols_max_types();
    if (want_cols) {
        nnconv_col_kernel<false><<<blocks, 64, 0, s>>>(adj_rowptr, adj_src, adj_type, n_nodes, 0, tile_cols, nullptr, nullptr, nullptr,
                                                       result + 0, max_types, nullptr, n_adj_edges > 0 ? edge_type : nullptr, adj_eid,
                                                       n_adj_edges > 0 ? adj_type : nullptr);
        exclusive_scan_i32(tile_cols, tile_col_ptr, nt16 + 1, scan_ws, s);
        nnconv_col_kernel<true><<<blocks, 64, 0, s>>>(adj_rowptr, adj_src, adj_type, n_nodes, 0, nullptr, tile_col_ptr, col_meta,
                                                      col_slot_src, result + 0, max_types, result + 5);
    }
    if (want_eg) {
        const bool gather_types = !want_cols && n_adj_edges > 0;
        launch_nnconv_eg_build(adj_rowptr, adj_src, adj_type, n_nodes, 0, result + 0, max_types, tile_cols, tile_grp_ptr, grp, scan_ws,
                               result + 10, s, gather_types ? edge_type : nullptr, gather_types ? adj_eid : nullptr,
                               host_words_dev ? result : nullptr, host_words_dev);
// ... 9 lines not shown
```

### tilingnn_amd/csrc/tgnn_common.h

```cpp
#pragma once
#include <hip/hip_runtime.h>
#include <stdint.h>
#include <stdio.h>

#include <atomic>

#include "../../include/tgnn.h"

namespace tgnn {

constexpr int kWave = 64;
constexpr float kLeakySlope = 0.01f;

void set_error(const char *fmt, ...);

#define TGNN_CHECK_ARG(cond, msg)                                                     \
    do {                                                                              \
        if (!(cond)) {                                                                \
            ::tgnn::set_error("%s: invalid argument: %s (%s)", __func__, msg, #cond); \
            return TGNN_ERR_INVALID_ARG;                                              \
        }                                                                             \
    } while (0)

#define TGNN_CHECK_LAUNCH()                                                                 \
    do {                                                                                    \
        hipError_t e__ = hipGetLastError();                                                 \
        if (e__ != hipSuccess) {                                                            \
            ::tgnn::set_error("%s: launch failed: %s", __func__, hipGetErrorString(e__));   \
            return TGNN_ERR_LAUNCH;                                                         \
        }                                                                                   \
    } while (0)

#define TGNN_CHECK_HIP(expr)                                                                \
    do {                                                                                    \
        hipError_t e__ = (expr);                                                            \
        if (e__ != hipSuccess) {                                                            \
            ::tgnn::set_error("%s: %s failed: %s", __func__, #expr, hipGetErrorString(e__)); \
            return TGNN_ERR_LAUNCH;                                                         \
        }                                                                                   \
    } while (0)

static inline size_t align_up(size_t v, size_t a) { return (v + a - 1) / a * a; }

struct DeviceGuard {
    int prev = -1;
    explicit DeviceGuard(tgnn_stream_t stream) {
        if (!stream) return;
        int cur = -1;
        hipDevice_t dev = -1;
        if (hipGetDevice(&cur) != hipSuccess || hipStreamGetDevice(static_cast<hipStream_t>(stream), &dev) != hipSuccess) return;
        if (dev != cur && hipSetDevice(dev) == hipSuccess) prev = cur;
    }
    ~DeviceGuard() {
        if (prev >= 0) (void)hipSetDevice(prev);
    }
    DeviceGuard(const DeviceGuard &) = delete;
    DeviceGuard &operator=(const DeviceGuard &) = delete;
};

struct LdsOptIn {
    std::atomic<bool> done[64];
};
template <class Kern>
static inline hipError_t opt_in_dynamic_lds(Kern kern, int bytes, LdsOptIn &site) {
    int dev = 0;
    hipError_t e = hipGetDevice(&dev);
    if (e != hipSuccess) return e;
    const bool tracked = dev >= 0 && dev < 64;
    if (tracked && site.done[dev].load(std::memory_order_acquire)) return hipSuccess;
    e = hipFuncSetAttribute(reinterpret_cast<const void *>(kern), hipFuncAttributeMaxDynamicSharedMemorySize, bytes);
    if (e == hipSuccess && tracked) site.done[dev].store(true, std::memory_order_release);
    return e;
}

static inline int device_cus() {
    static std::atomic<int> cached[64];
    int dev = 0;
    if (hipGetDevice(&dev) != hipSuccess || dev < 0 || dev >= 64) return 256;
    int v = cached[dev].load(std::memory_order_relaxed);
    if (v > 0) return v;
    int cus = 0;
    if (hipDeviceGetAttribute(&cus, hipDeviceAttributeMultiprocessorCount, dev) != hipSuccess || cus <= 0) cus = 256;
    cached[dev].store(cus, std::memory_order_relaxed);
    return cus;
}
static inline int cus_minus(int reserve) {
    const int cus = device_cus();
    const int left = cus - reserve;
    return left > cus / 4 ? left : (cus / 4 > 0 ? cus / 4 : 1);
}

struct Carver {
    char *base;
    size_t off = 0, cap;
    Carver(void *p, size_t bytes) : base(static_cast<char *>(p)), cap(bytes) {}
    template <typename T>
    T *take(size_t count) {
        off = align_up(off, 256);
        T *p = reinterpret_cast<T *>(base + off);
        off += count * sizeof(T);
        return p;
    }
    bool ok() const { return off <= cap; }
};

__device__ __forceinline__ float sigmoidf_(float v) { return __builtin_amdgcn_rcpf(1.0f + __expf(-v)); }
__device__ __forceinline__ float sigmoid_out_f32(float v) {
    constexpr float kL2eH = 1.44269502162933349609375f, kL2eL = 1.925963033500011e-8f, kLn2 = 0.693147182464599609375f;
    const float nv = -fminf(fmaxf(v, -87.0f), 87.0f);
    const float th = nv * kL2eH;
    const float tl = fmaf(nv, kL2eH, -th) + nv * kL2eL;
    const float eh = __builtin_amdgcn_exp2f(th);
    const float e = fmaf(eh, tl * kLn2, eh);
    const float d = 1.0f + e;
    float r = __builtin_amdgcn_rcpf(d);
    r = fmaf(fmaf(-d, r, 1.0f), r, r);
    return v != v ? v : r;
}
__device__ __forceinline__ float act_apply(float v, int act) {
    if (act == TGNN_ACT_LEAKY_RELU) return v >= 0.f ? v : v * kLeakySlope;
    if (act == TGNN_ACT_SIGMOID) return sigmoidf_(v);
    return v;
}
__device__ __forceinline__ float leakyf_(float v) { return v >= 0.f ? v : v * kLeakySlope; }

__device__ __forceinline__ float bn_apply1(float v, float mhi, float mlo, float g, float b) {
    return ((v - mhi) - mlo) * g + b;
}

using tgnn_bf16x8 = __attribute__((ext_vector_type(8))) __bf16;
using tgnn_u32x4 = __attribute__((ext_vector_type(4))) unsigned int;
__device__ __forceinline__ void split3_trunc(const float (&x)[8], tgnn_bf16x8 &hi, tgnn_bf16x8 &mid, tgnn_bf16x8 &lo) {
    tgnn_u32x4 ph, pm, pl;
#pragma unroll
    for (int p = 0; p < 4; ++p) {
        const unsigned int a0 = __float_as_uint(x[2 * p]), a1 = __float_as_uint(x[2 * p + 1]);
        const float r0 = x[2 * p] - __uint_as_float(a0 & 0xffff0000u);
        const float r1 = x[2 * p + 1] - __uint_as_float(a1 & 0xffff0000u);
        const unsigned int b0 = __float_as_uint(r0), b1 = __float_as_uint(r1);
        const float s0 = r0 - __uint_as_float(b0 & 0xffff0000u);
        const float s1 = r1 - __uint_as_float(b1 & 0xffff0000u);
        ph[p] = __builtin_amdgcn_perm(a1, a0, 0x07060302u);
        pm[p] = __builtin_amdgcn_perm(b1, b0, 0x07060302u);
        pl[p] = __builtin_amdgcn_perm(__float_as_uint(s1), __float_as_uint(s0), 0x07060302u);
    }
    hi = __builtin_bit_cast(tgnn_bf16x8, ph);
    mid = __builtin_bit_cast(tgnn_bf16x8, pm);
    lo = __builtin_bit_cast(tgnn_bf16x8, pl);
}

using tgnn_f16x8 = __attribute__((ext_vector_type(8))) _Float16;
__device__ __forceinline__ void split2_f16(const float (&x)[8], float s, tgnn_f16x8 &hi, tgnn_f16x8 &lo) {
#pragma unroll
    for (int j = 0; j < 8; ++j) {
        float a = x[j] * s;
        asm volatile("" : "+v"(a));
// ... 357 lines not shown
```

### tilingnn_amd/graph_networks/networks/TilinGNN.py

```python
import ctypes as C

import torch
import torch.nn as nn

from ... import _lib, ops
from ..._lib import check, lib, ptr
from .. import _graph_cache, _tracking
from .._tracking import Tracked
from ..layers.coll_conv import CollConv
from ..layers.edge_conv import GraphConv
from ..layers.util import MLP, Linear_trans


import os as _os
_BEGIN_FIRST = _os.environ.get("TGNN_BEGIN_FIRST", "1") == "1"


def _default_node_features_dim():
    try:
        from inputs.config import environment
        return environment.tile_count + 1
    except Exception as exc:
        raise ValueError("node_features_dim not given and inputs.config.environment is not importable; "
                         "pass node_features_dim=tile_count+1") from exc
# ... 149 lines not shown
            check(lib.tgnn_forward_union(C.byref(dims), table, k_n, arr(xs), arr(attrs), gs, int(not bn_train), arr(outs), arr(wss),
                                         (C.c_size_t * k_n)(*[int(w.numel()) for w in wss]), cur.cuda_stream,
                                         (C.c_void_p * len(used))(*[st.cuda_stream for st in used]), len(used), _lib.side_stream(dev)))
            for st in used:
                cur.wait_stream(st)
                st.wait_stream(cur)
            return outs
        check(lib.tgnn_forward_many(C.byref(dims), table, k_n, arr(xs), arr(attrs), gs, 0, int(not bn_train), arr(outs), arr(wss),
                                    (C.c_size_t * k_n)(*[int(w.numel()) for w in wss]),
                                    (C.c_void_p * len(used))(*[st.cuda_stream for st in used]), len(used), _lib.side_stream(dev)))
        for st in used:
            cur.wait_stream(st)
        return outs

    def forward(self, x, adj_e_index, adj_e_features, col_e_idx, col_e_features=None):
        return self._forward_one(x, adj_e_index, adj_e_features, col_e_idx, col_e_features)

    def forward_checked(self, x, adj_e_index, adj_e_features, col_e_idx, col_e_features=None):
        try:
            out = self._forward_one(x, adj_e_index, adj_e_features, col_e_idx, col_e_features)
        except _lib.TgnnError as exc:
            if exc.code != _lib.ERR_STALE_RESULT:
                raise
            out = self._forward_one(x, adj_e_index, adj_e_features, col_e_idx, col_e_features)
        dev = x.device
        code = C.c_uint32(0)
        check(lib.tgnn_spin_error_poll(_lib.current_stream(dev), C.byref(code)))
        if code.value:
            import warnings
            warnings.warn("tilingnn_amd: a persistent forward kernel gave up waiting for its blocks (another process holds compute "
                          f"units; reason bits {code.value}); the forward is repeated on the general launch schedule, which the "
                          "next forwards of this process take as well", RuntimeWarning)
            out = self._forward_one(x, adj_e_index, adj_e_features, col_e_idx, col_e_features)
        return out

    def _forward_one(self, x, adj_e_index, adj_e_features, col_e_idx, col_e_features=None, update_running=True):
        fast = (self.activation_dtype == torch.float32 and not (self.autograd and self.training and torch.is_grad_enabled()))
        table, dev = self._param_table(verify=not fast)
        for name, t in (("x", x), ("adj_e_index", adj_e_index), ("adj_e_features", adj_e_features),
                        ("col_e_idx", col_e_idx)):
            if t.device != dev:
                raise ValueError(f"`{name}` is on {t.device} but the network is on {dev}")
        if x.dim() != 2 or x.shape[1] != self.node_features_dim:
            raise ValueError(f"x must be [N, {self.node_features_dim}], got {tuple(x.shape)}")
        if adj_e_features.dim() != 2 or adj_e_features.shape[1] != self.adj_edge_features_dim:
            raise ValueError(f"adj_e_features must be [Ea, {self.adj_edge_features_dim}], "
                             f"got {tuple(adj_e_features.shape)}")
        n = int(x.shape[0])
        bn_train = self.training
        if self.autograd and bn_train and torch.is_grad_enabled():
            from ... import train
            return train.forward_with_grad(self, x, adj_e_index, adj_e_features, col_e_idx), adj_e_features
        if bn_train and n < 2:
            raise ValueError("Expected more than 1 value per channel when training")
        if self.activation_dtype == torch.bfloat16:
            from ... import ops_bf16
            graph = _graph_cache.get_full(n, adj_e_index, adj_e_features, col_e_idx) if self.cache_graph else None
            return ops_bf16.forward(self, x, adj_e_index, adj_e_features, col_e_idx, graph), adj_e_features
        if self.activation_dtype != torch.float32:
            raise ValueError("activation_dtype must be torch.float32 or torch.bfloat16")
        xf = ops._f32c(x, "x")
        ea = ops._f32c(adj_e_features, "adj_e_features")
        dims = self._dims()
        begun = False
        init_done = 0
        state = {}

        def prepare_new():
            def begin(info=None):
                state["bytes"] = lib.tgnn_forward_workspace_bytes(C.byref(dims), n, 0)
                state["ws"] = torch.empty(state["bytes"], dtype=torch.uint8, device=dev)
                state["rc"] = lib.tgnn_forward_begin(C.byref(dims), table, ptr(xf), n, int(update_running), ptr(state["ws"]), state["bytes"],
                                                     None, _lib.side_stream(dev))

            use_begin = bn_train and ops.runs_general_schedule(n) and n > 4096
            if use_begin:
                side = _lib.side_stream_torch(dev)
                if side is None:
                    use_begin = False
                else:
                    side.wait_stream(torch.cuda.current_stream(dev))
            if use_begin and _BEGIN_FIRST:
                begin()

            def weights(info=None):
                if not _BEGIN_FIRST:
                    begin()
                if info is not None and state.get("rc") == 0:
                    rcw = lib.tgnn_forward_begin_weights(C.byref(dims), table, ptr(ea), ptr(info["type_rep_edge"]), ptr(info["result"]),
                                                         n, ptr(state["ws"]), state["bytes"], _lib.current_stream(dev))
                    if rcw not in (0, _lib.ERR_UNSUPPORTED):
                        check(rcw)
            use_small = (not use_begin and bn_train and fast and 2 <= n <= min(4096, int(lib.tgnn_get_small_layout_limit())))

            def small_pre(info=None):
                if info is None:
                    return
                nbytes = lib.tgnn_forward_workspace_bytes(C.byref(dims), n, 0)
                wsp = torch.empty(nbytes, dtype=torch.uint8, device=dev)
                rcs = lib.tgnn_forward_small_prepass(C.byref(dims), table, ptr(ea), ptr(info["type_rep_edge"]), ptr(info["result"]), n,
                                                     ptr(wsp), nbytes, _lib.current_stream(dev))
                if rcs == 0:
                    state["small_ws"], state["small_bytes"] = wsp, nbytes
                elif rcs != _lib.ERR_UNSUPPORTED:
                    check(rcs)
            try:
                return ops.prepare_graph(n, adj_e_index, adj_e_features, col_e_idx,
                                         after_enqueue=weights if use_begin else small_pre if use_small else None)
            except Exception:
                side = _lib.side_stream_torch(dev) if state.get("rc") == 0 else None
                if side is not None:
                    torch.cuda.current_stream(dev).wait_stream(side)
                raise

        graph = _graph_cache.get_full(n, adj_e_index, adj_e_features, col_e_idx, build=prepare_new) if self.cache_graph else prepare_new()
        begun = state.get("rc") == 0
        if begun:
            ws, ws_bytes = state["ws"], state["bytes"]
        elif state.get("rc") not in (None, _lib.ERR_UNSUPPORTED):
            check(state["rc"])
        if begun and graph.n_types > 16:
            ws_need = lib.tgnn_forward_workspace_bytes(C.byref(dims), n, graph.n_types)
            if ws_need > ws_bytes:
                side = _lib.side_stream_torch(dev)
                if side is not None:
                    torch.cuda.current_stream(dev).wait_stream(side)
                begun = False
                init_done = 2 if update_running else 0
        if not begun and "small_ws" in state and graph.n_types <= 16:
            ws, ws_bytes = state["small_ws"], state["small_bytes"]
        elif not begun:
            ws_bytes = lib.tgnn_forward_workspace_bytes(C.byref(dims), n, graph.n_types)
            ws = torch.empty(ws_bytes, dtype=torch.uint8, device=dev)
        if graph.cols is None and graph.groups is not None and (not bn_train or lib.tgnn_set_split_precision(-1) == 0 or
                                                                 self.network_depth > 64):
            graph.ensure_columns()
        probs = torch.empty(n, self.output_dim, dtype=torch.float32, device=dev)
        g = graph.c_struct(defer_late_check=True)
        if begun:
            check(lib.tgnn_forward_resume(C.byref(dims), table, ptr(xf), ptr(ea), C.byref(g), int(update_running), ptr(probs), ptr(ws),
                                          ws_bytes, _lib.current_stream(dev), _lib.side_stream(dev)))
            if self._param_table_stale():
                table, dev = self._param_table()
                check(lib.tgnn_forward(C.byref(dims), table, ptr(xf), ptr(ea), C.byref(g), 0, 0, ptr(probs), ptr(ws), ws_bytes,
                                       _lib.current_stream(dev), _lib.side_stream(dev)))
            return probs, adj_e_features
        rc = lib.tgnn_forward(C.byref(dims), table, ptr(xf), ptr(ea), C.byref(g), int(bn_train and update_running) | init_done,
                              int(not bn_train), ptr(probs), ptr(ws), ws_bytes, _lib.current_stream(dev), _lib.side_stream(dev))
        if rc == _lib.ERR_UNVERIFIED:
            g = graph.c_struct()
            rc = lib.tgnn_forward(C.byref(dims), table, ptr(xf), ptr(ea), C.byref(g), int(bn_train and update_running) | init_done,
                                  int(not bn_train), ptr(probs), ptr(ws), ws_bytes, _lib.current_stream(dev), _lib.side_stream(dev))
        check(rc)
        if graph.late_words_failed():
            g = graph.c_struct()
            check(lib.tgnn_forward(C.byref(dims), table, ptr(xf), ptr(ea), C.byref(g), int(bn_train and update_running),
                                   int(not bn_train), ptr(probs), ptr(ws), ws_bytes, _lib.current_stream(dev), _lib.side_stream(dev)))
        if self._param_table_stale():
            table, dev = self._param_table()
            check(lib.tgnn_forward(C.byref(dims), table, ptr(xf), ptr(ea), C.byref(g), 0,
                                   int(not bn_train), ptr(probs), ptr(ws), ws_bytes, _lib.current_stream(dev), _lib.side_stream(dev)))
        return probs, adj_e_features
```

### tilingnn_amd/ops.py

```python
from __future__ import annotations

import ctypes as C
import os
from dataclasses import dataclass
from typing import Optional, Tuple

import torch

from . import _lib
from ._lib import ACT_LEAKY_RELU, ACT_NONE, ACT_SIGMOID, BN_MAX_PARTIALS, check, lib, ptr

Tensor = torch.Tensor


def _need_gpu(t: Tensor, name: str) -> None:
    if not t.is_cuda:
        raise RuntimeError(
            f"tilingnn_amd: `{name}` lives on {t.device}; this package only runs on an AMD GPU "
            "(no CPU fallback exists by design -- move the module and its inputs to 'cuda').")


def _f32c(t: Tensor, name: str) -> Tensor:
    _need_gpu(t, name)
    if t.dtype != torch.float32:
# ... 151 lines not shown
    ntiles = (n_nodes + 15) // 16
    grp = NNConvGroups(torch.empty(ntiles + 1, dtype=torch.int32, device=dev),
                       torch.empty(cap * 16, 2, dtype=torch.int32, device=dev))
    ws_bytes = lib.tgnn_nnconv_cols_workspace_bytes(n_nodes)
    ws = torch.empty(ws_bytes, dtype=torch.uint8, device=dev)
    check(lib.tgnn_nnconv_eg_build(ptr(rowptr), ptr(col_src), ptr(col_type), n_nodes, n_types,
                                   ptr(grp.tile_grp_ptr), ptr(grp.grp), ptr(ws), ws_bytes, _stream(rowptr)))
    return grp


def _check_edge_index(ei: Tensor, name: str) -> Tensor:
    _need_gpu(ei, name)
    if ei.dtype != torch.int64:
        raise ValueError(f"`{name}` must be int64 (torch .long()), got {ei.dtype}")
    if ei.numel() == 0:
        return ei.reshape(2, 0)
    if ei.dim() != 2 or ei.shape[0] != 2:
        raise ValueError(f"`{name}` must have shape [2, E], got {tuple(ei.shape)}")
    return ei if ei.is_contiguous() else ei.contiguous()


def build_csr(edge_index: Tensor, n_nodes: int, drop_self_loops: bool,
              n_src_nodes: Optional[int] = None) -> Tuple[Tensor, Tensor, Tensor, Tensor]:
    ei = _check_edge_index(edge_index, "edge_index")
    dev, e = ei.device, int(ei.shape[1])
    rowptr = torch.empty(n_nodes + 1, dtype=torch.int32, device=dev)
    col_src = torch.empty(max(e, 1), dtype=torch.int32, device=dev)
    col_eid = torch.empty(max(e, 1), dtype=torch.int32, device=dev)
    err = torch.zeros(1, dtype=torch.int32, device=dev)
    ws_bytes = lib.tgnn_csr_workspace_bytes(n_nodes, e)
    ws = torch.empty(ws_bytes, dtype=torch.uint8, device=dev)
    check(lib.tgnn_csr_build(ptr(ei), e, n_nodes, n_nodes if n_src_nodes is None else n_src_nodes,
                             int(drop_self_loops), ptr(rowptr), ptr(col_src), ptr(col_eid), ptr(err), ptr(ws), ws_bytes,
                             _stream(ei)))
    return rowptr, col_src, col_eid, err


def dedup_edge_types(edge_attr: Tensor) -> Tuple[Tensor, Tensor, Tensor]:
    ea = _f32c(edge_attr, "edge_attr")
    if ea.dim() != 2:
        raise ValueError(f"`edge_attr` must be [E, Fe], got {tuple(ea.shape)}")
    e, fe = int(ea.shape[0]), int(ea.shape[1])
    dev = ea.device
    edge_type = torch.empty(max(e, 1), dtype=torch.int32, device=dev)
    rep = torch.empty(max(e, 1), dtype=torch.int32, device=dev)
    n_types = torch.zeros(1, dtype=torch.int32, device=dev)
    ws_bytes = lib.tgnn_edge_dedup_workspace_bytes(e, fe)
    ws = torch.empty(ws_bytes, dtype=torch.uint8, device=dev)
    check(lib.tgnn_edge_type_dedup(ptr(ea), e, fe, ptr(edge_type), ptr(rep), ptr(n_types), ptr(ws), ws_bytes,
                                   _stream(ea)))
    return edge_type, rep, n_types


COLS_MIN_NODES = int(os.environ.get("TGNN_COLS_MIN_NODES", "0"))
GROUPS = os.environ.get("TGNN_GROUPS", "1") != "0"


def _small_prep_limits(_cache=[]):
    if not _cache:
        _cache.append((int(lib.tgnn_graph_prep_small_max_nodes()), int(lib.tgnn_graph_prep_small_max_edges())))
    return _cache[0]


def _small_prep_counters(dev, _cache={}):
    key = (dev.index, torch.cuda.current_stream(dev).cuda_stream)
    if key not in _cache:
        _cache[key] = torch.zeros(2, dtype=torch.int32, device=dev)
    return _cache[key]


SMALL_PREP = True


_pinned_words = {}


def _pinned_result_words(dev):
    import threading
    key = (threading.get_ident(), dev.index, "early")
    host = _pinned_words.get(key)
    if host is None:
        host = _pinned_words[key] = torch.empty(32, dtype=torch.int32, pin_memory=True)
    return host


def _read_back(res: Tensor):
    import threading
    key = (threading.get_ident(), res.device.index)
    host = _pinned_words.get(key)
    if host is None:
        host = _pinned_words[key] = torch.empty(32, dtype=torch.int32, pin_memory=True)
    host.copy_(res, non_blocking=True)
    torch.cuda.current_stream(res.device).synchronize()
    return host.tolist()


def _prepare_graph_fused(n_nodes: int, adj: Tensor, attr: Tensor, col: Tensor, small: bool,
                         n_src_nodes: Optional[int] = None, groups: Optional[bool] = None, after_enqueue=None) -> Optional[PreparedGraph]:
    ea, ec = int(adj.shape[1]), int(col.shape[1])
    if attr.dim() != 2 or attr.shape[1] < 1:
        return None
    attr = _f32c(attr, "adj_e_features")
    dev = adj.device
    ntiles = (n_nodes + 15) // 16
    e1, c1 = max(ea, 1), max(ec, 1)
    fe = int(attr.shape[1])
    ws_ints = int(lib.tgnn_graph_prep_small_tmp_ints(n_nodes, ea, ec)) if small else \
        (int(lib.tgnn_graph_prep_workspace_bytes(n_nodes, ea, ec, fe)) + 3) // 4 + 64
    lo_mid, hi_mid = mid_layout_range()
    want_eg = (not small and groups) if groups is not None else \
        (not small and GROUPS and (n_src_nodes is not None or runs_general_schedule(n_nodes)))
    both = groups == "both" and not small
    want_cols = both or not want_eg
    want_mid = not small and want_cols and n_src_nodes is None and lo_mid < n_nodes <= hi_mid
    mid_words = int(lib.tgnn_mid_entries_words(n_nodes)) if want_mid else 0
    cap = int(lib.tgnn_nnconv_cols_max_columns(n_nodes, ea)) if want_cols else 0
    gcap = int(lib.tgnn_nnconv_eg_max_groups(n_nodes, ea, lib.tgnn_nnconv_cols_max_types())) if want_eg else 0
    sizes = [n_nodes + 1, e1, e1, e1, e1, e1, n_nodes + 1, c1, c1, ntiles + 1, cap, cap * 16,
             ntiles if want_mid else 0, mid_words, ntiles + 1 if want_eg else 0, gcap * 32]
    offs, at = [], 0
    for sz in sizes:
        offs.append(at)
        at += (sz + 63) // 64 * 64
    buf = torch.empty(at, dtype=torch.int32, device=dev)
    v = [buf[o:o + sz] for o, sz in zip(offs, sizes)]
    (a_rowptr, a_src, a_eid, adj_type, edge_type, rep, c_rowptr, c_src, c_eid, tile_col_ptr, col_meta, col_slot_src,
     mid_nb, mid_ent, tile_grp_ptr, grp) = v
    res = torch.empty(32, dtype=torch.int32, device=dev)
    tmp = torch.empty(ws_ints, dtype=torch.int32, device=dev)
    head = (ptr(adj), ea, ptr(attr), fe, ptr(col), ec, n_nodes) + (() if small else (n_src_nodes or n_nodes,)) + (ptr(a_rowptr), ptr(a_src), ptr(a_eid), ptr(adj_type), ptr(edge_type),
            ptr(rep), ptr(c_rowptr), ptr(c_src), ptr(c_eid),
            *((ptr(tile_col_ptr), ptr(col_meta), ptr(col_slot_src)) if want_cols else (None,) * 3))
    small_words = None
    if small:
        small_words = _pinned_result_words(dev) if lib.tgnn_set_prep_words_poll(-1) else None
        check(lib.tgnn_graph_prep_small(*head, ptr(tmp), ptr(res), ptr(_small_prep_counters(dev)),
                                        C.c_void_p(small_words.data_ptr()) if small_words is not None else None, _stream(adj)))
    else:
        mid_args = (ptr(mid_nb), ptr(mid_ent)) if want_mid else (None,) * 2
        eg_args = (ptr(tile_grp_ptr), ptr(grp)) if want_eg else (None,) * 2
        early = _pinned_result_words(dev)
        check(lib.tgnn_graph_prep(*head, *mid_args, *eg_args, ptr(tmp), ws_ints * 4, ptr(res),
                                  C.c_void_p(early.data_ptr()) if early is not None else None, _stream(adj)))
    late = None
    if not small and early is not None:
        if want_mid:
            words = torch.empty(32, dtype=torch.int32, pin_memory=True)
            words.copy_(res, non_blocking=True)
            ev = torch.cuda.Event()
            ev.record(torch.cuda.current_stream(dev))
            late = (words, ev, res)
        if after_enqueue is not None:
            after_enqueue({"type_rep_edge": rep, "result": res})
            after_enqueue = None
        check(lib.tgnn_graph_prep_wait(_stream(adj)))
        host = early.tolist()
        host[5] = host[10] = int(host[0] <= lib.tgnn_nnconv_cols_max_types() and not host[6])
        host[9] = 0
    else:
        if after_enqueue is not None:
            after_enqueue({"type_rep_edge": rep, "result": res} if small else None)
        if small_words is not None:
            check(lib.tgnn_graph_prep_wait(_stream(adj)))
            host = small_words.tolist()
        else:
            host = _read_back(res)
    if host[1] or host[2]:
        raise IndexError(f"edge index out of range [0, {n_nodes}) in {'adj_e_index' if host[1] else 'col_e_idx'}")
    if host[6]:
        return None
    cols = NNConvColumns(tile_col_ptr, col_meta, col_slot_src) if host[5] and want_cols else None
    mid = NNConvBatches(mid_nb, mid_ent) if want_mid and cols is not None and host[9] == 0 else None
    groups_ = NNConvGroups(tile_grp_ptr, grp.view(-1, 2)) if want_eg and host[10] else None
    g = PreparedGraph(n_nodes, ea, int(host[3]), int(host[0]), a_rowptr, a_src, a_eid, adj_type, edge_type, rep,
                      c_rowptr, c_src, c_eid, cols, int(host[4]), mid, groups_)
    if late is not None and mid is not None:
        g.__dict__["_late_words"] = late
    return g


def _pinned_many_words(dev, k: int) -> Tensor:
    import threading
    key = (threading.get_ident(), dev.index, "many")
    host = _pinned_words.get(key)
    if host is None or host.numel() < 32 * k:
        host = _pinned_words[key] = torch.empty(32 * max(2 * k, 16), dtype=torch.int32, pin_memory=True)
    return host


def _small_many_eligible(n_nodes: int, adj: Tensor, attr: Tensor, col: Tensor) -> bool:
    max_n, max_e = _small_prep_limits()
    return COLS_MIN_NODES == 0 and 1 <= n_nodes <= max_n and max(int(adj.shape[1]), int(col.shape[1])) <= max_e and \
        attr.dim() == 2 and attr.shape[1] >= 1 and not (GROUPS and runs_general_schedule(n_nodes))


def _prepare_graphs_small_queue(items):
    k = len(items)
    dev = items[0][1].device
    table = (_lib.SmallPrepLayout * k)()
    pieces, keep, tmp_at, at_all = [], [], [], 0
    for n_nodes, adj, attr, col in items:
        tmp_at.append(at_all)
        at_all += (int(lib.tgnn_graph_prep_small_tmp_ints(n_nodes, int(adj.shape[1]), int(col.shape[1]))) + 63) // 64 * 64
    tmp = torch.empty(at_all, dtype=torch.int32, device=dev)
    res = torch.empty(k, 32, dtype=torch.int32, device=dev)
    for j, (n_nodes, adj, attr, col) in enumerate(items):
        ea, ec = int(adj.shape[1]), int(col.shape[1])
        ntiles = (n_nodes + 15) // 16
        e1, c1 = max(ea, 1), max(ec, 1)
        cap = int(lib.tgnn_nnconv_cols_max_columns(n_nodes, ea))
        sizes = [n_nodes + 1, e1, e1, e1, e1, e1, n_nodes + 1, c1, c1, ntiles + 1, cap, cap * 16]
# ... 355 lines not shown
```

Baseline: 54.41 million nodes/s.

## Overlap edge-weight table build with graph prep and add dictionary dedup

Registers an early-weights side job that the graph-prep side stream runs right after edge-type dedup, so the edge-MLP weight table is built in parallel with the rest of graph preparation rather than after it. It also adds a dictionary-based dedup insert kernel, and an option to keep the result-words buffer and zero it with a small kernel after the forward pass so the next prep can skip its memset. The default lean_head becomes 35, which turns on the early path. The cost is more global state, such as thread-local side jobs and cached result buffers, which raises the risk of stale state or reuse across calls.

```diff
diff --git a/include/tgnn.h b/include/tgnn.h
--- a/include/tgnn.h
+++ b/include/tgnn.h
@@ -178,6 +178,8 @@
 int tgnn_forward_begin_weights(const tgnn_model_dims *dims, const void *const *params_host, const float *adj_edge_attr,
                                const int32_t *type_rep_edge, const int32_t *n_types_dev, int64_t n_nodes, void *ws, size_t ws_bytes,
                                tgnn_stream_t stream);
+int tgnn_forward_begin_weights_early(const tgnn_model_dims *dims, const void *const *params_host, const float *adj_edge_attr,
+                                     int64_t n_nodes, void *ws, size_t ws_bytes);
 
 typedef struct tgnn_train_save {
     float *init_a[2];
@@ -289,8 +291,13 @@
                     void *ws, size_t ws_bytes, int32_t *result, int32_t *result_host, tgnn_stream_t stream);
 int tgnn_graph_prep_wait(tgnn_stream_t stream);
 int32_t tgnn_set_prep_words_poll(int32_t on);
+int tgnn_graph_prep_words_done(int32_t *result, tgnn_stream_t stream);
+int32_t tgnn_graph_prep_words_clean(const int32_t *result, tgnn_stream_t stream);
+int32_t tgnn_set_prep_words_keep(int32_t on);
+int32_t tgnn_set_dedup_dict(int32_t on);
 #ifdef TGNN_DEBUG
 int32_t tgnn_debug_set_csr_bucket_cap(int32_t cap);
+int32_t tgnn_debug_set_dedup_grid(int32_t cap);
 void tgnn_debug_set_block_caps(int32_t nnconv_blocks, int32_t gin_mlp_blocks);
 void tgnn_debug_spin_fault(int32_t n_launches);
 #endif
diff --git a/scratch/ab_prep_head.py b/scratch/ab_prep_head.py
--- /dev/null
+++ b/scratch/ab_prep_head.py
@@ -0,0 +1,41 @@
+import os, sys, statistics, torch
+sys.path.insert(0, os.path.dirname(os.path.dirname(os.path.abspath(__file__))))
+from tilingnn_amd import TilinGNN
+from tilingnn_amd._lib import lib
+from tilingnn_amd.synth import make_super_graph
+from tilingnn_amd.weights import make_state_dict
+dev = torch.device('cuda:0')
+n = 100_000
+modes = [(3, 0, 0), (3, 1, 0), (35, 0, 0), (3, 0, 1), (35, 1, 1)]
+sg = make_super_graph(n, 10 * n, 12 * n + n // 2, tile_count=2, n_edge_types=13, seed=1)
+x, adj, attr, col, _ = sg.to_torch(dev)
+net = TilinGNN(adj_edge_features_dim=15, network_depth=20, network_width=32, node_features_dim=3)
+net.load_state_dict(make_state_dict(15, 20, 32, 1, 3, seed=0), strict=True)
+net = net.to(dev).train()
+def setm(m):
+    lib.tgnn_set_lean_head(m[0]); lib.tgnn_set_dedup_dict(m[1]); lib.tgnn_set_prep_words_keep(m[2])
+probs = {}
+net.cache_graph = False
+for m in modes:
+    setm(m)
+    probs[m] = net(x=x, adj_e_index=adj, adj_e_features=attr, col_e_idx=col)[0].clone()
+for m in modes[1:]:
+    print(f"mode {m} vs {modes[0]}: identical {bool((probs[m] == probs[modes[0]]).all())}", flush=True)
+def timed(cache):
+    net.cache_graph = cache
+    for _ in range(3): net(x=x, adj_e_index=adj, adj_e_features=attr, col_e_idx=col)
+    torch.cuda.synchronize()
+    e0, e1 = torch.cuda.Event(enable_timing=True), torch.cuda.Event(enable_timing=True)
+    e0.record()
+    for _ in range(20): net(x=x, adj_e_index=adj, adj_e_features=attr, col_e_idx=col)
+    e1.record(); torch.cuda.synchronize()
+    return e0.elapsed_time(e1) / 20
+acc = {m: ([], []) for m in modes}
+for rep in range(int(os.environ.get("AB_REPS", "12"))):
+    for m in modes:
+        setm(m)
+        acc[m][0].append(timed(True)); acc[m][1].append(timed(False))
+for m in modes:
+    c, p = acc[m]
+    print(f"lean_head {m[0]:2d} dedup_dict {m[1]} words_keep {m[2]}: cached {statistics.mean(c)*1e3:7.1f} +- {statistics.stdev(c)*1e3:5.1f} us   "
+          f"with preparation {statistics.mean(p)*1e3:7.1f} +- {statistics.stdev(p)*1e3:5.1f} us (min {min(p)*1e3:.1f})  [mean +- sd of {len(p)} x 20 steps]", flush=True)
diff --git a/scratch/run_step.py b/scratch/run_step.py
--- /dev/null
+++ b/scratch/run_step.py
@@ -0,0 +1,21 @@
+import os, sys, time, torch
+sys.path.insert(0, os.getcwd())
+from tilingnn_amd import TilinGNN
+from tilingnn_amd.synth import make_super_graph
+from tilingnn_amd.weights import make_state_dict
+dev = torch.device("cuda:0")
+n = 100_000
+sg = make_super_graph(n, 10 * n, 12 * n + n // 2, tile_count=2, n_edge_types=13, seed=1)
+x, adj, attr, col, _ = sg.to_torch(dev)
+net = TilinGNN(adj_edge_features_dim=15, network_depth=20, network_width=32, node_features_dim=3)
+net.load_state_dict(make_state_dict(15, 20, 32, 1, 3, seed=0), strict=True)
+net = net.to(dev).train()
+net.cache_graph = False
+for _ in range(8):
+    net(x=x, adj_e_index=adj, adj_e_features=attr, col_e_idx=col)
+torch.cuda.synchronize()
+t0 = time.perf_counter()
+for _ in range(20):
+    net(x=x, adj_e_index=adj, adj_e_features=attr, col_e_idx=col)
+torch.cuda.synchronize()
+print("ms_per_step", (time.perf_counter() - t0) / 20 * 1e3)
diff --git a/scratch/step_timeline.py b/scratch/step_timeline.py
--- /dev/null
+++ b/scratch/step_timeline.py
@@ -0,0 +1,31 @@
+import csv, glob, sys
+d, outf = sys.argv[1], sys.argv[2]
+rows = []
+for f in glob.glob(d + "/**/*kernel_trace.csv", recursive=True):
+    for r in csv.DictReader(open(f)):
+        rows.append((int(r["Start_Timestamp"]), int(r["End_Timestamp"]), "q" + r.get("Queue_Id", "?"), r["Kernel_Name"]))
+rows.sort()
+starts = [i for i, r in enumerate(rows) if "bk_hist" in r[3]]
+a, b = starts[-2], starts[-1]
+def first_of(i):
+    j = i
+    while j > 0 and rows[i][0] - rows[j - 1][0] < 80_000 and ("fillBuffer" in rows[j - 1][3] or "dedup" in rows[j - 1][3] or "prep_init" in rows[j - 1][3]):
+        j -= 1
+    return j
+a2, b2 = first_of(a), first_of(b)
+lo = max(a2 - 3, 0)
+sel = rows[lo:b2]
+t0 = rows[a2][0]
+with open(outf, "w") as o:
+    prev_end = sel[0][0]
+    for s, e, q, name in sel:
+        o.write(f"{(s-t0)/1e3:9.1f} {(e-t0)/1e3:9.1f} {(e-s)/1e3:8.1f} us  gap {(s-prev_end)/1e3:6.1f}  {q:4s} {name[:110]}\n")
+        prev_end = max(prev_end, e)
+    prev_last = max(r[1] for r in rows[lo:a2]) if a2 > lo else t0
+    o.write(f"previous step's last kernel end -> bk_hist start: {(rows[a][0]-prev_last)/1e3:.1f} us\n")
+    eg = [r for r in sel if "nnconv_eg_kernel" in r[3] and r[0] >= t0]
+    if eg: o.write(f"end of the preparation's last launch (nnconv_eg_kernel<true>): {(max(r[1] for r in eg)-t0)/1e3:.1f} us\n")
+    nn = [r for r in sel if "nnconv32_eg_kernel" in r[3] and r[0] >= t0]
+    if nn: o.write(f"start of the first nnconv32_eg_kernel: {(nn[0][0]-t0)/1e3:.1f} us\n")
+    o.write(f"step period (start to next step's start): {(rows[b2][0]-t0)/1e3:.1f} us\n")
+print(open(outf).read()[-700:])
diff --git a/tilingnn_amd/_lib.py b/tilingnn_amd/_lib.py
--- a/tilingnn_amd/_lib.py
+++ b/tilingnn_amd/_lib.py
@@ -123,6 +123,11 @@
         "tgnn_forward_begin": (C.c_int, [C.POINTER(ModelDims), C.POINTER(C.c_void_p), p, i64, i32, p, sz, p, p]),
         "tgnn_forward_resume": (C.c_int, [C.POINTER(ModelDims), C.POINTER(C.c_void_p), p, p, C.POINTER(Graph), i32, p, p, sz, p, p]),
         "tgnn_forward_begin_weights": (C.c_int, [C.POINTER(ModelDims), C.POINTER(C.c_void_p), p, p, p, i64, p, sz, p]),
+        "tgnn_forward_begin_weights_early": (C.c_int, [C.POINTER(ModelDims), C.POINTER(C.c_void_p), p, i64, p, sz]),
+        "tgnn_set_dedup_dict": (i32, [i32]),
+        "tgnn_graph_prep_words_done": (C.c_int, [p, p]),
+        "tgnn_graph_prep_words_clean": (i32, [p, p]),
+        "tgnn_set_prep_words_keep": (i32, [i32]),
         "tgnn_forward_small_prepass": (C.c_int, [C.POINTER(ModelDims), C.POINTER(C.c_void_p), p, p, p, i64, p, sz, p]),
         "tgnn_forward_sharded_workspace_bytes": (sz, [C.POINTER(ModelDims), i64, i64, i32]),
         "tgnn_forward_sharded": (C.c_int, [C.POINTER(ModelDims), C.POINTER(C.c_void_p), p, p, C.POINTER(Graph),
@@ -229,7 +234,7 @@
     for name, (res, args) in sigs.items():
         fn = getattr(lib, name)
         fn.restype, fn.argtypes = res, args
-    for name, (res, args) in {"tgnn_debug_spin_fault": (None, [i32]), "tgnn_debug_set_csr_bucket_cap": (i32, [i32]),
+    for name, (res, args) in {"tgnn_debug_spin_fault": (None, [i32]), "tgnn_debug_set_csr_bucket_cap": (i32, [i32]), "tgnn_debug_set_dedup_grid": (i32, [i32]),
                               "tgnn_debug_set_block_caps": (None, [i32, i32])}.items():
         try:
             fn = getattr(lib, name)
@@ -256,7 +261,7 @@
     "tgnn_spin_error_poll", "tgnn_set_spin_budget_us", "tgnn_persist_fallback", "tgnn_spin_error_peek", "tgnn_gin_fwd", "tgnn_dense_act_fwd", "tgnn_dense_act_slots_fwd", "tgnn_dense_act_slots_f16_fwd", "tgnn_bn_finalize", "tgnn_bn_apply",
     "tgnn_merge_fwd", "tgnn_param_count", "tgnn_param_name", "tgnn_forward_workspace_bytes", "tgnn_forward", "tgnn_forward_begin", "tgnn_forward_resume",
     "tgnn_forward_profiled", "tgnn_forward_profiled_two_stream", "tgnn_forward_stamped", "tgnn_forward_many", "tgnn_forward_union", "tgnn_forward_union_plan", "tgnn_forward_union_counts", "tgnn_graph_prep_small_max_nodes", "tgnn_graph_prep_small_max_edges", "tgnn_graph_prep_small_tmp_ints",
-    "tgnn_graph_prep_small", "tgnn_graph_prep_workspace_bytes", "tgnn_graph_prep", "tgnn_graph_prep_wait", "tgnn_graph_prep_small_many", "tgnn_graph_prep_small_many_wait", "tgnn_graph_prep_small_many_plan", "tgnn_graph_prep_small_many_counts", "tgnn_set_small_layout_limit", "tgnn_get_small_layout_limit", "tgnn_set_split_precision", "tgnn_set_gin_fused", "tgnn_set_gin_mlp_f16", "tgnn_set_mid_tail", "tgnn_set_nnconv_eg", "tgnn_set_dense_rows_mode", "tgnn_set_lean_head", "tgnn_set_prep_words_poll", "tgnn_forward_begin_weights", "tgnn_forward_bf16_begin", "tgnn_forward_small_prepass", "tgnn_rccl_available", "tgnn_rccl_unique_id_bytes", "tgnn_rccl_unique_id", "tgnn_rccl_comm_create", "tgnn_rccl_comm_destroy", "tgnn_rccl_counters", "tgnn_forward_train", "tgnn_backward_workspace_bytes", "tgnn_backward", "tgnn_forward_sharded_workspace_bytes", "tgnn_forward_sharded",
+    "tgnn_graph_prep_small", "tgnn_graph_prep_workspace_bytes", "tgnn_graph_prep", "tgnn_graph_prep_wait", "tgnn_graph_prep_small_many", "tgnn_graph_prep_small_many_wait", "tgnn_graph_prep_small_many_plan", "tgnn_graph_prep_small_many_counts", "tgnn_set_small_layout_limit", "tgnn_get_small_layout_limit", "tgnn_set_split_precision", "tgnn_set_gin_fused", "tgnn_set_gin_mlp_f16", "tgnn_set_mid_tail", "tgnn_set_nnconv_eg", "tgnn_set_dense_rows_mode", "tgnn_set_lean_head", "tgnn_set_prep_words_poll", "tgnn_graph_prep_words_done", "tgnn_graph_prep_words_clean", "tgnn_set_prep_words_keep", "tgnn_set_dedup_dict", "tgnn_forward_begin_weights", "tgnn_forward_begin_weights_early", "tgnn_forward_bf16_begin", "tgnn_forward_small_prepass", "tgnn_rccl_available", "tgnn_rccl_unique_id_bytes", "tgnn_rccl_unique_id", "tgnn_rccl_comm_create", "tgnn_rccl_comm_destroy", "tgnn_rccl_counters", "tgnn_forward_train", "tgnn_backward_workspace_bytes", "tgnn_backward", "tgnn_forward_sharded_workspace_bytes", "tgnn_forward_sharded",
     "tgnn_rows_gather", "tgnn_rows_scatter", "tgnn_unsupervised_loss_workspace_bytes", "tgnn_unsupervised_loss", "tgnn_solution_score_sums",
     "tgnn_sublayout_workspace_bytes", "tgnn_sublayout_compact", "tgnn_greedy_round_workspace_bytes", "tgnn_greedy_round", "tgnn_greedy_finish_max_nodes", "tgnn_greedy_finish", "tgnn_shard_alive_rows",
     "tgnn_sublayout_compact_many_workspace_bytes", "tgnn_sublayout_compact_many", "tgnn_greedy_round_many_workspace_bytes", "tgnn_greedy_round_many",
diff --git a/tilingnn_amd/csrc/forward.hip b/tilingnn_amd/csrc/forward.hip
--- a/tilingnn_amd/csrc/forward.hip
+++ b/tilingnn_amd/csrc/forward.hip
@@ -114,7 +114,7 @@
 constexpr int kCarveTypes = 16;
 static std::atomic<int> g_split_f16{1};
 static std::atomic<int> g_nnconv_eg{1};
-static std::atomic<int> g_lean_head{3};
+static std::atomic<int> g_lean_head{35};
 static std::atomic<int64_t> g_path_count[3];
 static std::atomic<int64_t> g_union_count[2];
 
@@ -174,7 +174,7 @@
     return g_nnconv_eg.exchange(on);
 }
 extern "C" int32_t tgnn_set_lean_head(int32_t bits) {
-    if (bits < 0 || bits > 31) return g_lean_head.load();
+    if (bits < 0 || bits > 63) return g_lean_head.load();
     return g_lean_head.exchange(bits);
 }
 extern "C" const char *tgnn_last_error(void) { return g_err; }
@@ -340,6 +340,7 @@
     hipStream_t s = static_cast<hipStream_t>(stream);
     bool weights_early = false;
     bool small_pre = false;
+    prep_set_side_job(nullptr, nullptr);
     {
         int devp = 0;
         if (hipGetDevice(&devp) == hipSuccess && devp >= 0 && devp < 64 && g_small_pre[devp].ws) {
@@ -941,23 +942,22 @@
     return TGNN_OK;
 }
 
-extern "C" int tgnn_forward_begin_weights(const tgnn_model_dims *dims, const void *const *params_host, const float *adj_edge_attr,
-                                          const int32_t *type_rep_edge, const int32_t *n_types_dev, int64_t n_nodes, void *ws,
-                                          size_t ws_bytes, tgnn_stream_t stream) {
-    DeviceGuard guard__(stream);
+static int begin_weights_on(const tgnn_model_dims *dims, const void *const *params_host, const float *adj_edge_attr,
+                            const int32_t *type_rep_edge, const int32_t *n_types_dev, int64_t n_nodes, void *ws, size_t ws_bytes,
+                            hipStream_t s) {
     TGNN_CHECK_ARG(dims_ok(dims) && params_host && n_types_dev, "arguments");
     if (!adj_edge_attr || !type_rep_edge) return TGNN_ERR_UNSUPPORTED;
     int dev = 0;
     TGNN_CHECK_HIP(hipGetDevice(&dev));
     TGNN_CHECK_ARG(dev >= 0 && dev < 64, "device index");
     HeadEvent &he = g_head[dev];
+    if (he.ev && he.weights && he.ws == ws && he.n == n_nodes) return TGNN_OK;
     const int c = dims->network_width, D = dims->network_depth, fe = dims->adj_edge_features_dim;
     if (!he.ev || he.ws != ws || he.n != n_nodes || c != 32 || !edge_weight_table_device_count_ok(fe, c) || !g_nnconv_eg.load() ||
         !g_split_f16.load() || (g_lean_head.load(std::memory_order_relaxed) & 24))
         return TGNN_ERR_UNSUPPORTED;
     Workspace w = carve(*dims, n_nodes, n_nodes, 0, ws, ws_bytes);
     if (!ws || w.bytes > ws_bytes) return TGNN_ERR_WORKSPACE;
-    hipStream_t s = static_cast<hipStream_t>(stream);
     const Params P{params_host, D};
     EdgeMlpLayers layers{};
     const float *roots[kMaxDepth];
@@ -970,6 +970,48 @@
                                      kEgImageScale, n_types_dev, kCarveTypes);
     he.weights = true;
     TGNN_CHECK_LAUNCH();
+    return TGNN_OK;
+}
+
+extern "C" int tgnn_forward_begin_weights(const tgnn_model_dims *dims, const void *const *params_host, const float *adj_edge_attr,
+                                          const int32_t *type_rep_edge, const int32_t *n_types_dev, int64_t n_nodes, void *ws,
+                                          size_t ws_bytes, tgnn_stream_t stream) {
+    DeviceGuard guard__(stream);
+    return begin_weights_on(dims, params_host, adj_edge_attr, type_rep_edge, n_types_dev, n_nodes, ws, ws_bytes,
+                            static_cast<hipStream_t>(stream));
+}
+
+struct EarlyWeights {
+    tgnn_model_dims dims;
+    const void *const *params_host = nullptr;
+    const float *adj_edge_attr = nullptr;
+    int64_t n = 0;
+    void *ws = nullptr;
+    size_t ws_bytes = 0;
+};
+static thread_local EarlyWeights g_early_weights;
+static int early_weights_job(void *ctx, const int32_t *type_rep_edge, const int32_t *n_types_dev, hipStream_t side) {
+    const EarlyWeights &a = *static_cast<const EarlyWeights *>(ctx);
+    return begin_weights_on(&a.dims, a.params_host, a.adj_edge_attr, type_rep_edge, n_types_dev, a.n, a.ws, a.ws_bytes, side);
+}
+
+extern "C" int tgnn_forward_begin_weights_early(const tgnn_model_dims *dims, const void *const *params_host, const float *adj_edge_attr,
+                                                int64_t n_nodes, void *ws, size_t ws_bytes) {
+    prep_set_side_job(nullptr, nullptr);
+    if (!dims) return TGNN_OK;
+    TGNN_CHECK_ARG(dims_ok(dims) && params_host, "arguments");
+    if (!adj_edge_attr || !(g_lean_head.load(std::memory_order_relaxed) & 32)) return TGNN_ERR_UNSUPPORTED;
+    int dev = 0;
+    TGNN_CHECK_HIP(hipGetDevice(&dev));
+    TGNN_CHECK_ARG(dev >= 0 && dev < 64, "device index");
+    const HeadEvent &he = g_head[dev];
+    const int c = dims->network_width, fe = dims->adj_edge_features_dim;
+    if (!he.ev || he.ws != ws || he.n != n_nodes || he.weights || c != 32 || !edge_weight_table_device_count_ok(fe, c) ||
+        !g_nnconv_eg.load() || !g_split_f16.load() || (g_lean_head.load(std::memory_order_relaxed) & 24))
+        return TGNN_ERR_UNSUPPORTED;
+    if (!ws || carve(*dims, n_nodes, n_nodes, 0, ws, ws_bytes).bytes > ws_bytes) return TGNN_ERR_WORKSPACE;
+    g_early_weights = EarlyWeights{*dims, params_host, adj_edge_attr, n_nodes, ws, ws_bytes};
+    prep_set_side_job(early_weights_job, &g_early_weights);
     return TGNN_OK;
 }
 
diff --git a/tilingnn_amd/csrc/graph_prep.hip b/tilingnn_amd/csrc/graph_prep.hip
--- a/tilingnn_amd/csrc/graph_prep.hip
+++ b/tilingnn_amd/csrc/graph_prep.hip
@@ -357,6 +357,144 @@
         }
         __syncthreads();
         if (ok) slot_of_edge[i] = lslot[ltab[my_l]];
+    }
+}
+
+constexpr int kDedupDict = 32;
+__device__ __forceinline__ uint32_t canon_u32(uint32_t u) { return u == 0x80000000u ? 0u : u; }
+__global__ __launch_bounds__(kDedupRows) void dedup_insert_dict_kernel(const float *__restrict__ attr, int64_t e, int fe,
+                                                                       int *__restrict__ table, uint32_t mask,
+                                                                       int *__restrict__ slot_of_edge, int *__restrict__ rep_cnt,
+                                                                       int *__restrict__ rep_slots) {
+    extern __shared__ uint32_t rows_s[];
+    __shared__ int ltab[kDedupLocal];
+    __shared__ int lslot[kDedupRows];
+    __shared__ uint32_t d_hash[kDedupDict];
+    __shared__ int d_slot[kDedupDict];
+    __shared__ int d_n;
+    const int ld = fe | 1, tid = threadIdx.x;
+    uint32_t *d_rows = rows_s + kDedupRows * ld;
+    if (tid == 0) d_n = 0;
+    const int step_r = (4 * kDedupRows) / fe, step_c = (4 * kDedupRows) % fe;
+    for (int64_t base = (int64_t)blockIdx.x * kDedupRows; base < e; base += (int64_t)gridDim.x * kDedupRows) {
+        const int64_t n_here = e - base < kDedupRows ? e - base : kDedupRows;
+        const int total = (int)(n_here * fe), nv = total >> 2;
+        {
+            const float *src = attr + base * fe;
+            const uint4 *src4 = reinterpret_cast<const uint4 *>(src);
+            int r = (4 * tid) / fe, c = (4 * tid) % fe;
+            for (int v = tid; v < nv; v += kDedupRows) {
+                const uint4 q = src4[v];
+                int rr = r, cc = c;
+                rows_s[rr * ld + cc] = canon_u32(q.x);
+                if (++cc == fe) { cc = 0; ++rr; }
+                rows_s[rr * ld + cc] = canon_u32(q.y);
+                if (++cc == fe) { cc = 0; ++rr; }
+                rows_s[rr * ld + cc] = canon_u32(q.z);
+                if (++cc == fe) { cc = 0; ++rr; }
+                rows_s[rr * ld + cc] = canon_u32(q.w);
+                r += step_r;
+                c += step_c;
+                if (c >= fe) { c -= fe; ++r; }
+            }
+            const int kt = (nv << 2) + tid;
+            if (kt < total) rows_s[(kt / fe) * ld + kt % fe] = canon_bits(src[kt]);
+        }
+        __syncthreads();
+        const int64_t i = base + tid;
+        const bool ok = i < e;
+        const uint32_t *mine = rows_s + tid * ld;
+        uint64_t h = 0xCBF29CE484222325ull;
+        if (ok)
+            for (int k = 0; k < fe; ++k) h = mix64(h, mine[k]);
+        const uint32_t h32 = (uint32_t)(h ^ (h >> 32));
+        const int nd = d_n < kDedupDict ? d_n : kDedupDict;
+        int slot_found = -1;
+        if (ok)
+            for (int j = 0; j < nd; ++j) {
+                if (d_hash[j] != h32) continue;
+                const uint32_t *other = d_rows + j * ld;
+                uint32_t diff = 0;
+                for (int k = 0; k < fe; ++k) diff |= other[k] ^ mine[k];
+                if (diff == 0) {
+                    slot_found = d_slot[j];
+                    break;
+                }
+            }
+        const bool miss = ok && slot_found < 0;
+        if (!__syncthreads_or(miss ? 1 : 0)) {
+            if (ok) slot_of_edge[i] = slot_found;
+            continue;
+        }
+        ltab[tid] = -1;
+        ltab[tid + kDedupRows] = -1;
+        __syncthreads();
+        int my_l = 0;
+        if (miss) {
+            uint32_t sl = h32 & (kDedupLocal - 1);
+            while (true) {
+                int cur = ltab[sl];
+                if (cur < 0) {
+                    const int prev = atomicCAS(&ltab[sl], -1, tid);
+                    if (prev < 0) break;
+                    cur = prev;
+                }
+                bool same = cur == tid;
+                if (!same) {
+                    const uint32_t *other = rows_s + cur * ld;
+                    uint32_t diff = 0;
+                    for (int k = 0; k < fe; ++k) diff |= other[k] ^ mine[k];
+                    same = diff == 0;
+                }
+                if (same) {
+                    if (tid < cur) atomicMin(&ltab[sl], tid);
+                    break;
+                }
+                sl = (sl + 1) & (kDedupLocal - 1);
+            }
+            my_l = (int)sl;
+        }
+        __syncthreads();
+        if (miss && ltab[my_l] == tid) {
+            uint32_t slot = h32 & mask;
+            while (true) {
+                int cur = __hip_atomic_load(&table[slot], __ATOMIC_RELAXED, __HIP_MEMORY_SCOPE_AGENT);
+                if (cur < 0) {
+                    const int prev = atomicCAS(&table[slot], -1, (int)i);
+                    if (prev < 0) {
+                        if (rep_cnt) {
+                            const int k = atomicAdd(rep_cnt, 1) + 1;
+                            if (k < kDedupListMax) rep_slots[k] = (int)slot;
+                        }
+                        break;
+                    }
+                    cur = prev;
+                }
+                bool same = cur == (int)i;
+                if (!same) {
+                    const float *other = attr + (int64_t)cur * fe;
+                    uint32_t diff = 0;
+#pragma unroll 8
+                    for (int k = 0; k < fe; ++k) diff |= canon_bits(other[k]) ^ mine[k];
+                    same = diff == 0;
+                }
+                if (same) {
+                    if ((int)i < cur) atomicMin(&table[slot], (int)i);
+                    break;
+                }
+                slot = (slot + 1) & mask;
+            }
+            lslot[tid] = (int)slot;
+            const int j = atomicAdd(&d_n, 1);
+            if (j < kDedupDict) {
+                d_hash[j] = h32;
+                d_slot[j] = (int)slot;
+                uint32_t *dst = d_rows + j * ld;
+                for (int k = 0; k < fe; ++k) dst[k] = mine[k];
+            }
+        }
+        __syncthreads();
+        if (ok) slot_of_edge[i] = miss ? lslot[ltab[my_l]] : slot_found;
     }
 }
 
@@ -1057,6 +1195,27 @@
     return cap;
 }
 
+static std::atomic<int> g_dedup_dict{0};
+static std::atomic<int> g_dedup_grid_cap{0};
+static hipError_t launch_dedup_insert(const float *attr, int64_t e, int fe, int *table, uint32_t mask, int *slot_of_edge, int *rep_cnt,
+                                      int *rep_slots, hipStream_t s) {
+    const size_t tile_b = (size_t)kDedupRows * (fe | 1) * 4;
+    if (g_dedup_dict.load(std::memory_order_relaxed) && ((uintptr_t)attr & 15) == 0) {
+        const size_t lds = tile_b + (size_t)kDedupDict * (fe | 1) * 4;
+        static LdsOptIn site;
+        if (lds > 64 * 1024) {
+            const hipError_t err = opt_in_dynamic_lds(dedup_insert_dict_kernel, (int)(80 * 1024), site);
+            if (err != hipSuccess) return err;
+        }
+        const int cap = g_dedup_grid_cap.load(std::memory_order_relaxed);
+        const unsigned grid = grid_for(e, kDedupRows, cap > 0 ? cap : 2 * device_cus());
+        dedup_insert_dict_kernel<<<grid, kDedupRows, lds, s>>>(attr, e, fe, table, mask, slot_of_edge, rep_cnt, rep_slots);
+    } else {
+        dedup_insert_kernel<<<grid_for(e, kDedupRows), kDedupRows, tile_b, s>>>(attr, e, fe, table, mask, slot_of_edge, rep_cnt, rep_slots);
+    }
+    return hipSuccess;
+}
+
 
 constexpr int kBkLogMax = 9, kBkRows = 1 << kBkLogMax, kBkMaxBuckets = 4096, kBkThreads = 1024;
 constexpr int kBkCap = 15360;
@@ -1278,6 +1437,12 @@
 }
 
 static std::atomic<int> g_bk_cap{kBkCap};
+struct SideJob {
+    PrepSideJob fn = nullptr;
+    void *ctx = nullptr;
+};
+static thread_local SideJob g_side_job;
+void prep_set_side_job(PrepSideJob fn, void *ctx) { g_side_job = SideJob{fn, ctx}; }
 static int prep_side_stream(hipStream_t *st, hipEvent_t *fork, hipEvent_t *join) {
     static std::mutex mu;
     static hipStream_t streams[64] = {};
@@ -1415,7 +1580,16 @@
 
 using namespace tgnn;
 
+extern "C" int32_t tgnn_set_dedup_dict(int32_t on) {
+    if (on < 0) return g_dedup_dict.load();
+    return g_dedup_dict.exchange(on ? 1 : 0);
+}
+
 #ifdef TGNN_DEBUG
+extern "C" int32_t tgnn_debug_set_dedup_grid(int32_t cap) {
+    if (cap < 0) return g_dedup_grid_cap.load();
+    return g_dedup_grid_cap.exchange(cap);
+}
 extern "C" int32_t tgnn_debug_set_csr_bucket_cap(int32_t cap) {
     const int prev = g_bk_cap.load();
     if (cap >= 0) g_bk_cap.store(cap > kBkCap ? kBkCap : cap);
@@ -1476,8 +1650,7 @@
     int *rep_slots = cv.take<int>(kDedupListMax);
     TGNN_CHECK_HIP(hipMemsetAsync(table, 0xFF, (size_t)(cap + 64) * 4, s));
     if (fe <= 60)
-        dedup_insert_kernel<<<grid_for(n_edges, kDedupRows), kDedupRows, (size_t)kDedupRows * (fe | 1) * 4, s>>>(
-            edge_attr, n_edges, fe, table, cap - 1, slot_of_edge, table + cap, rep_slots);
+        TGNN_CHECK_HIP(launch_dedup_insert(edge_attr, n_edges, fe, table, cap - 1, slot_of_edge, table + cap, rep_slots, s));
     else
         dedup_insert_direct_kernel<<<grid_for(n_edges), 256, 0, s>>>(edge_attr, n_edges, fe, table, cap - 1, slot_of_edge, table + cap,
                                                                      rep_slots);
@@ -1513,8 +1686,7 @@
     int *scan_ws = cv.take<int>(scan_ws_ints(n_edges));
     TGNN_CHECK_HIP(hipMemsetAsync(table, 0xFF, (size_t)cap * 4, s));
     if (fe <= 60)
-        dedup_insert_kernel<<<grid_for(n_edges, kDedupRows), kDedupRows, (size_t)kDedupRows * (fe | 1) * 4, s>>>(
-            edge_attr, n_edges, fe, table, cap - 1, slot_of_edge);
+        TGNN_CHECK_HIP(launch_dedup_insert(edge_attr, n_edges, fe, table, cap - 1, slot_of_edge, nullptr, nullptr, s));
     else
         dedup_insert_direct_kernel<<<grid_for(n_edges), 256, 0, s>>>(edge_attr, n_edges, fe, table, cap - 1, slot_of_edge);
     dedup_mark_first_kernel<<<grid_for(n_edges), 256, 0, s>>>(table, slot_of_edge, n_edges, is_first);
@@ -2026,6 +2198,37 @@
     if (threadIdx.x == 0) atomicMax(result + 4, max(max(wm[0], wm[1]), max(wm[2], wm[3])));
 }
 
+__global__ __launch_bounds__(64) void prep_words_zero_kernel(int *__restrict__ result) {
+    if (threadIdx.x < 32) result[threadIdx.x] = 0;
+}
+struct WordsClean {
+    const int32_t *ptr = nullptr;
+    hipStream_t stream = nullptr;
+};
+static thread_local WordsClean g_words_clean;
+static std::atomic<int> g_words_keep{0};
+
+extern "C" int32_t tgnn_set_prep_words_keep(int32_t on) {
+    if (on < 0) return g_words_keep.load();
+    return g_words_keep.exchange(on ? 1 : 0);
+}
+
+extern "C" int32_t tgnn_graph_prep_words_clean(const int32_t *result, tgnn_stream_t stream) {
+    return result && g_words_clean.ptr == result && g_words_clean.stream == static_cast<hipStream_t>(stream) ? 1 : 0;
+}
+
+extern "C" int tgnn_graph_prep_words_done(int32_t *result, tgnn_stream_t stream) {
+    TGNN_CHECK_ARG(result, "null pointer");
+    g_words_clean = WordsClean{};
+    if (!g_words_keep.load(std::memory_order_relaxed)) return TGNN_OK;
+    DeviceGuard guard__(stream);
+    hipStream_t s = static_cast<hipStream_t>(stream);
+    prep_words_zero_kernel<<<1, 64, 0, s>>>(result);
+    TGNN_CHECK_LAUNCH();
+    g_words_clean = WordsClean{result, s};
+    return TGNN_OK;
+}
+
 extern "C" size_t tgnn_graph_prep_workspace_bytes(int64_t n_nodes, int64_t n_adj_edges, int64_t n_col_edges, int32_t fe) {
     const int64_t emax = n_adj_edges > n_col_edges ? n_adj_edges : n_col_edges;
     return align_up(tgnn_csr_workspace_bytes(n_nodes, emax), 256) + align_up(bk_workspace_bytes(n_nodes, n_adj_edges, n_col_edges), 256) +
@@ -2041,6 +2244,11 @@
                                int32_t *col_slot_src, int32_t *mid_tile_nb, uint32_t *mid_ent, int32_t *tile_grp_ptr, int32_t *grp,
                                void *ws, size_t ws_bytes, int32_t *result, int32_t *result_host, tgnn_stream_t stream) {
     DeviceGuard guard__(stream);
+    const SideJob side_job = g_side_job;
+    g_side_job = SideJob{};
+    const bool words_clean = result && g_words_clean.ptr == result && g_words_clean.stream == static_cast<hipStream_t>(stream) &&
+                             g_words_keep.load(std::memory_order_relaxed);
+    g_words_clean = WordsClean{};
     TGNN_CHECK_ARG(n_nodes >= 1 && fe >= 1 && n_adj_edges >= 0 && n_col_edges >= 0, "shape");
     TGNN_CHECK_ARG(n_src_nodes >= n_nodes && n_src_nodes < (1ll << 31) - 1, "n_src_nodes must be >= n_nodes and fit int32");
     const bool want_cols = tile_col_ptr != nullptr, want_eg = tile_grp_ptr != nullptr;
@@ -2059,7 +2267,7 @@
     const size_t csr_b = tgnn_csr_workspace_bytes(n_nodes, emax), dd_b = tgnn_edge_dedup_workspace_bytes(n_adj_edges, fe),
                  col_b = tgnn_nnconv_cols_workspace_bytes(n_nodes);
     void *ws_csr = cv.take<unsigned char>(csr_b), *ws_dd = cv.take<unsigned char>(dd_b), *ws_col = cv.take<unsigned char>(col_b);
-    TGNN_CHECK_HIP(hipMemsetAsync(result, 0, 32 * sizeof(int32_t), s));
+    if (!words_clean) TGNN_CHECK_HIP(hipMemsetAsync(result, 0, 32 * sizeof(int32_t), s));
     hipStream_t s_side = nullptr;
     hipEvent_t ev_fork = nullptr, ev_join = nullptr;
     if (n_adj_edges > 0 && prep_side_stream(&s_side, &ev_fork, &ev_join) == TGNN_OK) {
@@ -2079,6 +2287,10 @@
         if (!s_side) return TGNN_OK;
         rc = edge_type_dedup_listed(adj_edge_attr, n_adj_edges, fe, edge_type, type_rep_edge, result + 0, result + 6, ws_dd, dd_b, s_side);
         if (rc != TGNN_OK) return bail(rc);
+        if (side_job.fn) {
+            rc = side_job.fn(side_job.ctx, type_rep_edge, result + 0, s_side);
+            if (rc != TGNN_OK && rc != TGNN_ERR_UNSUPPORTED) return bail(rc);
+        }
         if (hipEventRecord(ev_join, s_side) != hipSuccess) {
             (void)hipStreamSynchronize(s_side);
             set_error("tgnn_graph_prep: hipEventRecord failed");
diff --git a/tilingnn_amd/csrc/tgnn_common.h b/tilingnn_amd/csrc/tgnn_common.h
--- a/tilingnn_amd/csrc/tgnn_common.h
+++ b/tilingnn_amd/csrc/tgnn_common.h
@@ -72,6 +72,9 @@
     if (e == hipSuccess && tracked) site.done[dev].store(true, std::memory_order_release);
     return e;
 }
+
+typedef int (*PrepSideJob)(void *ctx, const int32_t *type_rep_edge, const int32_t *n_types_dev, hipStream_t side);
+void prep_set_side_job(PrepSideJob fn, void *ctx);
 
 static inline int device_cus() {
     static std::atomic<int> cached[64];
diff --git a/tilingnn_amd/graph_networks/networks/TilinGNN.py b/tilingnn_amd/graph_networks/networks/TilinGNN.py
--- a/tilingnn_amd/graph_networks/networks/TilinGNN.py
+++ b/tilingnn_amd/graph_networks/networks/TilinGNN.py
@@ -255,6 +255,9 @@
                     side.wait_stream(torch.cuda.current_stream(dev))
             if use_begin and _BEGIN_FIRST:
                 begin()
+                if state.get("rc") == 0:
+                    state["early"] = lib.tgnn_forward_begin_weights_early(C.byref(dims), table, ptr(ea), n, ptr(state["ws"]),
+                                                                          state["bytes"]) == 0
 
             def weights(info=None):
                 if not _BEGIN_FIRST:
@@ -284,6 +287,8 @@
                 side = _lib.side_stream_torch(dev) if state.get("rc") == 0 else None
                 if side is not None:
                     torch.cuda.current_stream(dev).wait_stream(side)
+                if state.get("early"):
+                    lib.tgnn_forward_begin_weights_early(None, None, None, 0, None, 0)
                 raise
 
         graph = _graph_cache.get_full(n, adj_e_index, adj_e_features, col_e_idx, build=prepare_new) if self.cache_graph else prepare_new()
@@ -313,6 +318,7 @@
         if begun:
             check(lib.tgnn_forward_resume(C.byref(dims), table, ptr(xf), ptr(ea), C.byref(g), int(update_running), ptr(probs), ptr(ws),
                                           ws_bytes, _lib.current_stream(dev), _lib.side_stream(dev)))
+            ops.prep_words_done(dev)
             if self._param_table_stale():
                 table, dev = self._param_table()
                 check(lib.tgnn_forward(C.byref(dims), table, ptr(xf), ptr(ea), C.byref(g), 0, 0, ptr(probs), ptr(ws), ws_bytes,
diff --git a/tilingnn_amd/ops.py b/tilingnn_amd/ops.py
--- a/tilingnn_amd/ops.py
+++ b/tilingnn_amd/ops.py
@@ -257,6 +257,24 @@
     if host is None:
         host = _pinned_words[key] = torch.empty(32, dtype=torch.int32, pin_memory=True)
     return host
+
+
+_kept_words = {}
+
+
+def _kept_result_words(dev, create=True):
+    import threading
+    key = (threading.get_ident(), dev.index, torch.cuda.current_stream(dev).cuda_stream)
+    res = _kept_words.get(key)
+    if res is None and create:
+        res = _kept_words[key] = torch.empty(32, dtype=torch.int32, device=dev)
+    return res
+
+
+def prep_words_done(dev) -> None:
+    res = _kept_result_words(dev, create=False)
+    if res is not None:
+        check(lib.tgnn_graph_prep_words_done(ptr(res), _lib.current_stream(dev)))
 
 
 def _read_back(res: Tensor):
@@ -301,7 +319,7 @@
     v = [buf[o:o + sz] for o, sz in zip(offs, sizes)]
     (a_rowptr, a_src, a_eid, adj_type, edge_type, rep, c_rowptr, c_src, c_eid, tile_col_ptr, col_meta, col_slot_src,
      mid_nb, mid_ent, tile_grp_ptr, grp) = v
-    res = torch.empty(32, dtype=torch.int32, device=dev)
+    res = _kept_result_words(dev) if want_eg and not want_cols else torch.empty(32, dtype=torch.int32, device=dev)
     tmp = torch.empty(ws_ints, dtype=torch.int32, device=dev)
     head = (ptr(adj), ea, ptr(attr), fe, ptr(col), ec, n_nodes) + (() if small else (n_src_nodes or n_nodes,)) + (ptr(a_rowptr), ptr(a_src), ptr(a_eid), ptr(adj_type), ptr(edge_type),
             ptr(rep), ptr(c_rowptr), ptr(c_src), ptr(c_eid),
```

After: 54.61 million nodes/s (median of 2 runs). No clear change (+0.4%).
